# Nextomics/NextPolish2

Hardware: AMD Instinct MI355X
Metric: polished reference Mbp/s (whole node) at 30x HiFi + k21/k31; FASTA identical to oracle (higher is better)
Workload: dtype u8

## Files before the change

### nextpolish2_amd/csrc/np2_ctx.hpp

```cpp
#pragma once
#include "../../include/np2.h"
#include "np2_abi.hpp"
#include "np2_common.hpp"
#include "np2_kernels.hpp"
#include "np2_hostcpu.hpp"

#include <algorithm>
#include <atomic>
#include <chrono>
#include <cstdio>
#include <cstdlib>
#include <cstring>
#include <map>
#include <memory>
#include <exception>
#include <mutex>
#include <stdexcept>
#include <string>
#include <vector>

namespace np2h {

using namespace np2;

// ... 418 lines not shown
    uint32_t tile_cap = TILE_CAP;
};

struct np2_ctx {
    int device = 0;
    hipStream_t stream = nullptr;
    hipStream_t stream_out = nullptr;
    hipEvent_t ev_out = nullptr;
    uint8_t *out_host[2] = {nullptr, nullptr};
    size_t out_host_cap[2] = {0, 0};
    int out_slot = 0;
    bool out_pending = false;
    uint64_t out_len = 0;
    std::vector<YakTable> yaks;
    std::string err;
    bool trace = false;
    std::map<std::string, std::vector<uint8_t>> trace_items;
    Timing timing;
    std::vector<std::pair<std::string, std::pair<hipEvent_t, hipEvent_t>>> pending_events;

    PinnedBuf pin_d2h, pin_h2d;
    uint32_t *mbox_host = nullptr, *mbox_dev = nullptr;
    uint32_t mbox_seq = 0;
    bool borrowed_state = false;
    uint8_t *sink_dst = nullptr;
    uint64_t sink_cap = 0;
    uint32_t last_first_pos = 0, last_last_pos = 0;
    const uint8_t *last_dbase = nullptr;
    const uint32_t *last_dpos = nullptr;
    DevBuf<uint32_t> shard_bounds;
    uint64_t last_len = 0;
    bool reuse_identical_pass = true;
    bool h2d_inflight = false;
    bool stage_timing = false;
    DevBuf<uint8_t> tmp;
    DevBuf<uint64_t> keys_raw, keys;
    DevBuf<uint32_t> vals_raw, vals;
    DevBuf<uint32_t> npos, ncount, nminr, nbesti, node_off, run_start, run_end, n0_besti, emit, eoff;
    DevBuf<uint16_t> nbases, ndelta;
    DevBuf<int64_t> nscore;
    DevBuf<int32_t> cov, mval, smin;
    DevBuf<uint8_t> alive, cns_base, cns_cls, lq_kind, lq_nothead;
    DevBuf<uint32_t> cns_pos, lq_next, rflag, rstart, rend, ridx, raw_start, raw_end, headflag, hidx, lq_start,
        lq_end;
    DevBuf<uint32_t> pj, pcount, reg_ncand, reg_bytes, reg_soff, reg_maxlen, blk_sum, blk_coff, blk_soff, kept_read, kept_len, kept_col, cand_off, cand_order, cand_seq_off, kill_ids;
    DevBuf<uint64_t> cand_kmer;
    DevBuf<uint8_t> cand_seq;
    DevBuf<uint16_t> kscore;
    DevBuf<uint32_t> scal;
    DevBuf<uint64_t> lb_status;
    DevBuf<uint32_t> lb_ticket;
    uint32_t lb_ticket_total = 0, lb_epoch = 0;
    bool lb_dirty = false;
    static constexpr size_t LB_MAX_BLOCKS = 1u << 20;
    DevBuf<uint32_t> mlen;
    DevBuf<uint8_t> reg_lable, grp, cns_base2, rech_groups, rech_groups_tmp;
    DevBuf<uint8_t> votepack;
    DevBuf<uint8_t> votepack2;
    DevBuf<uint32_t> rl_list, rl_blob_off, rl_glen;
    DevBuf<uint2> rl_job_ol;
    DevBuf<uint32_t> rech_headjobs;
    DevBuf<uint32_t> ecount, eval, eval_s, eflag, eidx, seed_cand, keep_n, keep_list, cns_pos2, sp_idx_s,
        sp_idx_e, ap_g, ap_s, ap_e, rech, rech_joboff, job_len,
        job_off32;
    DevBuf<int32_t> ew, ap_delta, ap_shift;
    DevBuf<uint64_t> ekey, ekey_s;
    DevBuf<uint16_t> keep_ks;
    DevBuf<uint32_t> long_list;
    DevBuf<uint64_t> bt_path;
    DevBuf<uint64_t> chunk_st;
    uint32_t chunk_epoch = 0;
    DevBuf<uint32_t> tile_cur, tile_n, tile_scan, tile_scanb, tile_nn, tile_nr, tile_noff, tile_roff;
    uint32_t tile_cap = TILE_CAP;
    uint32_t bucket_cap = 0;
    DevBuf<uint2> nrec;
    DevBuf<uint8_t> votebuf;
    DevBuf<uint32_t> band, band_n, band_off, row_cnt;
    DevBuf<int64_t> run_gain, tile_gain;
    DevBuf<uint8_t> out_snap;
    DevBuf<uint8_t> run_flag;
    uint32_t deep_min = 65536;
    DevBuf<uint32_t> lq_list, hbits;
    DevBuf<uint16_t> tile_pidx;
    bool pidx_valid = false;
    DevBuf<ReadInfo> rinfo;
    DevBuf<uint32_t> lqc, lqoff;
    DevBuf<uint8_t> pflag;
    DevBuf<uint32_t> dp_list;
    DevBuf<uint16_t> pf_slots;
    DevBuf<uint32_t> pf_bad, pf_bad2;
    DevBuf<uint64_t> pf_prof;
    bool front_fused = false;
    struct Hooks {
        bool front_unfused = false, pf_prof = false, edge_sort = false;
        bool test_misspeculate = false, shard_spec_log = false, phase_profile = false, exact_grow = false, no_speculate = false;
        bool has_grow_guess = false, rech_general = false, rech_log = false;
        uint32_t grow_guess = 0;
        uint32_t rech_cap_list = 0xFFFFFFFFu, rech_cap_jobs = 0xFFFFFFFFu, rech_cap_blob = 0xFFFFFFFFu;
        bool has_pf_cap = false, has_pf_cap_big = false, has_pf_halo = false, has_pf_cov_max = false;
        uint32_t pf_cap = 0, pf_cap_big = 0, pf_halo = 0, pf_cov_max = 0;
        void read() {
            auto on = [](const char *n) { return getenv(n) != nullptr; };
            auto u32 = [](const char *n, bool &has, uint32_t &v) {
                if (const char *e = getenv(n)) has = true, v = (uint32_t)atol(e);
            };
            front_unfused = on("NP2_FRONT_UNFUSED"), pf_prof = on("NP2_PF_PROF"), edge_sort = on("NP2_EDGE_SORT");
            test_misspeculate = on("NP2_TEST_MISSPECULATE");
            shard_spec_log = on("NP2_SHARD_SPEC_LOG"), phase_profile = on("NP2_PHASE_PROFILE"), exact_grow = on("NP2_EXACT_GROW");
            no_speculate = on("NP2_NO_SPECULATE");
            rech_general = on("NP2_RECH_GENERAL");
            rech_log = on("NP2_RECH_LOG");
            if (const char *e = getenv("NP2_TEST_RECH_CAP")) {
                char *end = nullptr;
                rech_cap_list = (uint32_t)strtoul(e, &end, 10);
                if (end && *end == ',') rech_cap_jobs = (uint32_t)strtoul(end + 1, &end, 10);
                if (end && *end == ',') rech_cap_blob = (uint32_t)strtoul(end + 1, &end, 10);
            }
            u32("NP2_TEST_GROW_GUESS", has_grow_guess, grow_guess);
            u32("NP2_PF_CAP", has_pf_cap, pf_cap), u32("NP2_PF_CAP_BIG", has_pf_cap_big, pf_cap_big);
            u32("NP2_PF_HALO", has_pf_halo, pf_halo), u32("NP2_PF_COV_MAX", has_pf_cov_max, pf_cov_max);
        }
    } hooks;
    bool pf_big = getenv("NP2_PF_BIG") != nullptr;
    uint32_t front_redos = 0;
    DevBuf<uint16_t> kscore_saved;
    DevBuf<uint8_t> sstr;
    DevBuf<uint64_t> soff;
    DevBuf<uint16_t> sscore;
};


namespace np2h {


enum Scal { S_ERR = 0, S_NNODES, S_NRUNS, S_BEST, S_PATHBEGIN, S_NRAW, S_NREG, S_DUP, S_LAST0, S_LAST1, S_GAIN0,
            S_GAIN1, S_DEEP, S_NDPLIST, S_NRECH, S_NGROUPS, S_NLONG, S_NLQ, S_PF, S_M0, S_M1, S_M2, S_M3, S_NC, S_SB, S_GROW,
            S_NBAD, S_PFOUT, S_PFGAIN0, S_PFGAIN1, S_PFEND0, S_PFEND1, S_NBAD2, S_NOKEY, S_COUNT = 34 };
static_assert(S_M1 % 2 == 0 && S_LAST0 % 2 == 0 && S_GAIN0 % 2 == 0 && S_PFGAIN0 % 2 == 0 && S_PFEND0 % 2 == 0,
              "64-bit device counters live in these slot pairs");

static constexpr int NP2_MAX_YAK = 15;
static constexpr uint32_t SCAL_TOTAL = 96;
static_assert(S_COUNT + 2 * (NP2_MAX_YAK + 2) <= SCAL_TOTAL && S_COUNT < 64, "round counters behind the posted block; the mailbox holds 64 words");
static constexpr uint32_t S_RL = S_COUNT + 2 * (NP2_MAX_YAK + 2);
static_assert(S_RL + 2 + np2::RL_STATE_WORDS <= SCAL_TOTAL, "the region lists' counters fit behind the round counters");

inline double thread_cpu_ms() {
    timespec ts;
    clock_gettime(CLOCK_THREAD_CPUTIME_ID, &ts);
    return ts.tv_sec * 1e3 + ts.tv_nsec * 1e-6;
}
struct WallTimer {
    np2_ctx *cx;
    const char *name;
    double t0, c0 = 0;
    WallTimer(np2_ctx *c, const char *n);
    ~WallTimer();
};

struct EventTimer {
    np2_ctx *cx;
    hipEvent_t a = nullptr, b = nullptr;
    bool on;
    EventTimer(np2_ctx *c, const char *name, bool always = false)
        : cx(c), on((always || c->stage_timing) && !tl_recorder()) {
        if (!on) return;
// ... 239 lines not shown
```

### nextpolish2_amd/csrc/np2_final.cpp

```cpp
#include "np2_polish.hpp"

#include <algorithm>
#include <cstdio>
#include <string>
#include <vector>

using namespace np2;

namespace {

static const uint8_t LB_SUCC = 0x80, LB_RECH = 0x20;

CnsDev splice_buffers(np2_ctx *cx, const CnsDev &in, uint32_t n_slots, uint32_t grow_bound, bool to_b, uint32_t version) {
    cx->sp_idx_s.ensure(n_slots + 2);
    cx->sp_idx_e.ensure(n_slots + 2);
    cx->ap_g.ensure(n_slots + 2);
    cx->ap_s.ensure(n_slots + 2);
    cx->ap_e.ensure(n_slots + 2);
    cx->ap_delta.ensure(n_slots + 2);
    cx->ap_shift.ensure(n_slots + 2);
    cx->mlen.ensure(16);
    const uint32_t out_cap = in.M_cap + grow_bound;
    const size_t cap = (size_t)out_cap + 64;
    uint32_t *opos = to_b ? cx->cns_pos2.ensure(cap) : cx->cns_pos.ensure(cap);
    uint8_t *obase = to_b ? cx->cns_base2.ensure(cap) : cx->cns_base.ensure(cap);
    return CnsDev{opos, obase, cx->mlen.p + version, out_cap};
}
CnsDev splice_gpu(np2_ctx *cx, const CnsDev &in, uint32_t n_reg, uint8_t lable, uint32_t grow_bound, bool to_b,
                  uint32_t version) {
    hipStream_t s = cx->stream;
    EventTimer t(cx, "splice");
    const CnsDev out = splice_buffers(cx, in, n_reg, grow_bound, to_b, version);
    uint32_t *const opos = out.pos;
    uint8_t *const obase = out.base;
    const uint32_t out_cap = out.M_cap;
    uint32_t *const stuck_p = cx->scal.p + S_COUNT + 2 * version, *const nap_p = stuck_p + 1;
    launch_splice_find(s, in.pos, in.M_p, cx->lq_start.p, cx->lq_end.p, cx->reg_lable.p, lable, n_reg, cx->sp_idx_s.p,
                       cx->sp_idx_e.p, stuck_p);
    launch_splice_plan(s, next_lookback(cx, region_lb_blocks(n_reg)), cx->reg_lable.p, lable, n_reg, stuck_p,
                       cx->sp_idx_s.p, cx->sp_idx_e.p, cx->seed_cand.p, cx->cand_seq_off.p, cx->ap_g.p, cx->ap_s.p,
                       cx->ap_e.p, cx->ap_delta.p, cx->ap_shift.p, nap_p, in.M_p, cx->mlen.p + version, out_cap,
                       cx->scal.p + S_ERR);
    launch_splice_write(s, in.pos, in.base, in.M_p, in.M_cap, cx->ap_g.p, cx->ap_s.p, cx->ap_e.p, cx->ap_delta.p,
                        cx->ap_shift.p, nap_p, n_reg, cx->lq_start.p, cx->seed_cand.p, cx->cand_seq_off.p,
                        cx->cand_seq.p, opos, obase);
    return out;
}

Cns fetch_cns_dev(np2_ctx *cx, const CnsDev &c) {
    Cns r;
    const uint32_t M = d2h(cx, c.M_p, 1)[0];
    r.pos = d2h(cx, c.pos, M);
    r.base = d2h(cx, c.base, M);
    return r;
}

bool rech_by_list(const np2_ctx *cx, uint32_t n_reg) {
    return !cx->trace && !cx->hooks.rech_general && n_reg <= RL_NREG_MAX;
}
uint32_t rech_list_cap(const np2_ctx *cx) { return std::min(cx->hooks.rech_cap_list, RL_CAP_LIST); }
uint32_t *rech_list_of(np2_ctx *cx, size_t y) { return cx->rl_list.p + (y & 1) * RL_CAP_LIST; }
uint32_t *rech_list_cnt(np2_ctx *cx, size_t y) { return cx->scal.p + S_RL + (y & 1); }

CnsDev recheck_list_gpu(np2_ctx *cx, const CnsDev &in, const PassCounts &pc, int yak_idx, uint16_t min_kmer_count,
                        bool first_yak, bool last_yak, bool to_b, uint32_t version) {
    hipStream_t s = cx->stream;
    EventTimer t(cx, "recheck");
    const uint32_t ksize = cx->yaks[yak_idx].k;
    const uint32_t cap_jobs = std::min(cx->hooks.rech_cap_jobs, RL_CAP_JOBS), cap_blob = std::min(cx->hooks.rech_cap_blob, RL_CAP_BLOB);
    cx->rech.ensure(RL_CAP_LIST + 2);
    cx->rech_groups.ensure((size_t)(RL_CAP_LIST + 2) * rech_group_bytes());
    cx->rech_groups_tmp.ensure((size_t)(RL_CAP_LIST + 2) * rech_group_bytes());
    cx->rech_joboff.ensure(RL_CAP_LIST + 2);
    cx->rl_blob_off.ensure(RL_CAP_LIST + 2);
    cx->rl_glen.ensure(RL_CAP_LIST + 2);
    cx->rl_job_ol.ensure(RL_CAP_JOBS + 2);
    cx->sstr.ensure((size_t)RL_CAP_BLOB + 64);
    cx->sscore.ensure(RL_CAP_JOBS + 2);
    const CnsDev out = splice_buffers(cx, in, std::max(pc.n_reg, RL_CAP_LIST), pc.grow, to_b, version);
    uint32_t *const st = cx->scal.p + S_RL + 2, *const nap_p = cx->scal.p + S_COUNT + 2 * version + 1;
    const RechList rl{rech_list_of(cx, (size_t)yak_idx), rech_list_cnt(cx, (size_t)yak_idx), rech_list_of(cx, (size_t)yak_idx + 1),
                      rech_list_cnt(cx, (size_t)yak_idx + 1), st, cx->rech.p, cx->sp_idx_s.p, cx->sp_idx_e.p, cx->rech_groups.p, cx->rech_groups_tmp.p,
                      cx->rech_joboff.p, cx->rl_blob_off.p, cx->rl_glen.p, cx->rl_job_ol.p, cx->sstr.p,
                      rech_list_cap(cx), cap_jobs, cap_blob};
    launch_rech_prepare(s, rl, in.pos, in.base, in.M_p, cx->lq_start.p, cx->lq_end.p, cx->keep_n.p, ksize, cx->reg_maxlen.p,
                        cx->cand_off.p, cx->keep_list.p, cx->cand_seq_off.p, cx->cand_seq.p, cx->scal.p + S_ERR);
    launch_score_jobs(s, cx->yaks[yak_idx].dev(), cx->sstr.p, cx->rl_job_ol.p, st + RL_NJOBS, min_kmer_count,
                      cx->sscore.p);
    launch_rech_finish(s, rl, cx->sscore.p, cx->keep_ks.p, cx->cand_off.p, cx->keep_n.p, cx->keep_list.p, cx->cand_order.p,
                       first_yak, last_yak, cx->reg_lable.p, cx->seed_cand.p, in.pos, in.M_p, cx->lq_start.p,
                       cx->cand_seq_off.p, cx->ap_g.p, cx->ap_s.p, cx->ap_e.p, cx->ap_delta.p, cx->ap_shift.p, nap_p, cx->mlen.p + version,
                       out.M_cap, cx->scal.p + S_ERR);
    launch_splice_write(s, in.pos, in.base, in.M_p, in.M_cap, cx->ap_g.p, cx->ap_s.p, cx->ap_e.p, cx->ap_delta.p,
                        cx->ap_shift.p, nap_p, RL_CAP_LIST, cx->lq_start.p, cx->seed_cand.p, cx->cand_seq_off.p,
                        cx->cand_seq.p, out.pos, out.base);
    cx->timing.host.push_back({"rech_list", 1.0f});
    return out;
}

CnsDev recheck_gpu(np2_ctx *cx, const CnsDev &in, const PassCounts &pc, int yak_idx, uint16_t min_kmer_count,
                   bool first_yak, bool to_b, uint32_t version) {
    hipStream_t s = cx->stream;
    const uint32_t n_reg = pc.n_reg, ksize = cx->yaks[yak_idx].k;
    uint32_t n_rech = 0, n_groups = 0, n_jobs = 0;
    uint64_t blob_bound = 0;
    {
        EventTimer t(cx, "recheck");
        cx->rech.ensure(n_reg + 2);
        cx->rech_groups.ensure((size_t)(n_reg + 2) * rech_group_bytes());
        cx->rech_joboff.ensure(n_reg + 2);
        cx->rech_groups_tmp.ensure((size_t)(n_reg + 2) * rech_group_bytes());
        cx->rech_headjobs.ensure(n_reg + 2);
        launch_rech_list(s, next_lookback(cx, region_lb_blocks(n_reg)), cx->reg_lable.p, n_reg, cx->rech.p, cx->scal.p + S_NRECH,
                         (unsigned long long *)(cx->scal.p + S_M1), cx->scal.p + S_ERR);
        launch_rech_groups(s, next_lookback(cx, region_lb_blocks(n_reg)), cx->rech.p, cx->scal.p + S_NRECH, n_reg, in.pos, in.M_p,
                           cx->lq_start.p, cx->lq_end.p, cx->keep_n.p, ksize, cx->reg_maxlen.p, cx->rech_groups_tmp.p,
                           cx->rech_headjobs.p, cx->rech_groups.p,
                           cx->rech_joboff.p, cx->scal.p + S_NGROUPS,
                           cx->scal.p + S_M0, (unsigned long long *)(cx->scal.p + S_M1), cx->scal.p + S_ERR);
        std::vector<uint32_t> sc = fetch_scal(cx);
        blob_bound = (uint64_t)sc[S_M1] | ((uint64_t)sc[S_M2] << 32);
        check_region_err(sc[S_ERR]);
        n_rech = sc[S_NRECH];
        n_groups = sc[S_NGROUPS];
        n_jobs = sc[S_M0];
        if (cx->hooks.rech_log)
            fprintf(stderr, "np2 recheck, table %d: %u regions, %u RECH, %u groups, %u jobs, %llu string bytes at most\n", yak_idx, n_reg,
                    n_rech, n_groups, n_jobs, (unsigned long long)blob_bound);
    }
    if (n_rech) {
        RechPtrs rp{cx->rech_groups.p, cx->rech_joboff.p, cx->rech.p, cx->cand_off.p, cx->keep_list.p,
                    cx->cand_seq_off.p, cx->cand_seq.p, in.base, n_groups};
        if (n_jobs) {
            EventTimer t(cx, "recheck");
            cx->job_len.ensure(n_jobs + 2);
            cx->job_off32.ensure(n_jobs + 2);
            cx->soff.ensure(n_jobs + 2);
            cx->sscore.ensure(n_jobs + 2);
            cx->tmp.ensure(prim_temp_bytes((size_t)n_jobs + 2));
            launch_rech_job_len(s, rp, n_jobs, cx->job_len.p);
            exclusive_total_n(cx, cx->job_len.p, cx->job_off32.p, n_jobs);
            if (blob_bound >= 0xFFFFFFF0ull)
                blob_bound = fetch_scal(cx, cx->scal.p + S_M0, cx->job_off32.p + n_jobs)[S_M0];
            cx->sstr.ensure((size_t)blob_bound + 64);
            launch_rech_job_build(s, rp, n_jobs, cx->job_off32.p, cx->soff.p, cx->sstr.p);
            launch_score_strings(s, cx->yaks[yak_idx].dev(), cx->sstr.p, cx->soff.p, n_jobs, min_kmer_count,
                                 cx->sscore.p, true);
            launch_rech_apply(s, rp, cx->sscore.p, cx->keep_ks.p);
        }
        EventTimer t(cx, "recheck");
        launch_rech_select(s, cx->rech.p, cx->scal.p + S_NRECH, n_rech, cx->cand_off.p, cx->keep_n.p, cx->keep_list.p,
                           cx->keep_ks.p, cx->cand_order.p, first_yak, cx->reg_lable.p, cx->seed_cand.p);
    }
    CnsDev out = splice_gpu(cx, in, n_reg, LB_RECH, pc.grow, to_b, version);
    launch_rech_relabel(s, cx->reg_lable.p, n_reg);
    return out;
}

void fetch_result(np2_ctx *cx, const uint32_t *dpos, const uint8_t *dbase, const uint32_t *M_p, uint32_t M_cap, ResultOut &r,
                  uint32_t M_likely = 0xFFFFFFFFu) {
    const double t0 = now_ms();
    std::vector<uint32_t> sc;
    if (cx->sink_dst && cx->sink_cap) launch_copy_len(cx->stream, cx->sink_dst, dbase, M_p, 1, cx->sink_cap);
    if (r.want_bases || r.want_pos) {
        const uint32_t seq = ++cx->mbox_seq;
        launch_post(cx->stream, cx->scal.p, S_COUNT, cx->mbox_dev, seq, cx->scal.p + S_M0, M_p, nullptr, nullptr, nullptr, nullptr,
                    nullptr, nullptr, dpos, cx->scal.p + S_M1);
        if (r.want_bases) r.bases = (uint8_t *)pinned_pool().get((size_t)M_cap + 1);
        if (r.want_pos) r.pos = (uint32_t *)pinned_pool().get(((size_t)M_cap + 1) * 4);
        if ((r.want_bases && !r.bases) || (r.want_pos && !r.pos)) throw Np2Error(NP2_E_NOMEM, "pinned result allocation failed");
        uint32_t first = std::min(M_cap, M_likely);
        const bool exact_b = r.want_bases && op_d2h_len(cx, r.bases, dbase, M_p, 1, M_cap);
        const bool exact_p = r.want_pos && op_d2h_len(cx, r.pos, dpos, M_p, 4, (size_t)M_cap * 4);
        if (r.want_bases && !exact_b) op_d2h(cx, r.bases, dbase, first);
        if (r.want_pos && !exact_p) op_d2h(cx, r.pos, dpos, (size_t)first * 4);
// ... 156 lines not shown
```

### nextpolish2_amd/csrc/np2_graph.hip

```cpp
#include "np2_common.hpp"
#include "np2_kernels.hpp"
#include "np2_blockscan.hpp"
#include "np2_lookback.hpp"

namespace np2 {

__device__ __forceinline__ uint32_t block_excl_scan_256(uint32_t v, uint32_t *sh, uint32_t &total) {
    return block_excl_scan<OpAdd, 4>(v, sh, total);
}

__device__ uint64_t make_node_key(const np2_read_t *__restrict__ reads, const uint8_t *__restrict__ nib, uint64_t rec,
                                  uint32_t r) {
    const uint32_t col = (uint32_t)rec, t3 = (uint32_t)(rec >> 32);
    const np2_read_t rd = reads[r];
    const uint8_t *base = nib + rd.nib_off;
    const uint32_t ts = rd.aln_t_s;
    auto mk = [&](int64_t c, uint32_t t) -> AlignBase {
        if (c == -2) return ab_head(ts - 1, 0);
        if (c == -1) return ab_head(ts - 1, 1);
        const uint8_t nb = nib_at(base, (uint32_t)c);
        AlignBase a;
        a.q = nb & 7;
        a.t_pos = t;
        a.delta = 0;
        if (c > 0 && (nb & 8)) {
            uint16_t dl = 1;
            int64_t x = c - 1;
            while (x > 0 && (nib_at(base, (uint32_t)x) & 8)) {
                dl = (uint16_t)(dl + 1);
                --x;
            }
            a.delta = dl;
        }
        return a;
    };
    auto is_ins = [&](int64_t c) -> bool { return c > 0 && (nib_at(base, (uint32_t)c) & 8); };
    const int64_t c3 = col;
    const AlignBase b3 = mk(c3, t3);
    const uint32_t t2 = is_ins(c3) ? t3 : t3 - 1;
    const AlignBase b2 = mk(c3 - 1, t2);
    const uint32_t t1 = is_ins(c3 - 1) ? t2 : t2 - 1;
    const AlignBase b1 = mk(c3 - 2, t1);
    return ((uint64_t)b3.t_pos << 32) | ((uint64_t)node_bases(b1, b2, b3) << 16) | b1.delta;
}

__device__ __forceinline__ void k_tile_layout(const uint32_t np2_bid, const uint32_t np2_nb, uint32_t *__restrict__ tile_cur, uint32_t n_tiles,
                                                      uint32_t bucket_cap, uint32_t *__restrict__ tile_n,
                                                      uint32_t *__restrict__ tile_scan, uint32_t *__restrict__ tile_scanb,
                                                      const uint32_t *__restrict__ ovf_cnt, uint32_t *__restrict__ out) {
    __shared__ uint32_t sh[16];
    const uint32_t ta = block_scan_array<OpAdd>(
        n_tiles, sh, [&](uint32_t i) { return tile_cur[i]; },
        [&](uint32_t i, uint32_t pre, uint32_t v) {
            tile_scan[i] = pre;
            tile_n[i] = v;
        });
    const uint32_t tb = block_scan_array<OpAdd>(
        n_tiles, sh, [&](uint32_t i) { return min(tile_n[i], bucket_cap); },
        [&](uint32_t i, uint32_t pre, uint32_t) { tile_scanb[i] = pre; });
    const uint32_t mx = block_scan_array<OpMaxU32>(
        n_tiles, sh, [&](uint32_t i) { return tile_n[i]; }, [&](uint32_t i, uint32_t, uint32_t) { tile_cur[i] = 0; });
    if (threadIdx.x == 0) {
        tile_scan[n_tiles] = ta;
        tile_scanb[n_tiles] = tb;
        out[0] = ta;
        out[1] = mx;
        out[2] = *ovf_cnt;
    }
}

static constexpr uint32_t TLB_ITEMS = 4;
__device__ __forceinline__ void k_tile_layout_lb(const uint32_t np2_bid, const uint32_t np2_nb, Lookback lb, uint32_t n_blocks, uint32_t *__restrict__ tile_cur,
                                                        uint32_t n_tiles, uint32_t bucket_cap, uint32_t *__restrict__ tile_n,
                                                        uint32_t *__restrict__ tile_scan, uint32_t *__restrict__ tile_scanb,
                                                        const uint32_t *__restrict__ ovf_cnt, uint32_t *__restrict__ out,
                                                        uint32_t *__restrict__ err) {
    __shared__ uint32_t sh[8];
    const uint32_t bid = lb_block_id(lb, sh);
    const uint32_t i0 = (bid * 256 + threadIdx.x) * TLB_ITEMS;
    uint32_t v[TLB_ITEMS], sa = 0, sb = 0, mx = 0;
#pragma unroll
    for (uint32_t k = 0; k < TLB_ITEMS; ++k) {
        v[k] = i0 + k < n_tiles ? tile_cur[i0 + k] : 0u;
        sa += v[k];
        sb += min(v[k], bucket_cap);
        mx = max(mx, v[k]);
    }
    for (int o = 32; o > 0; o >>= 1) mx = max(mx, __shfl_xor(mx, o));
    if ((threadIdx.x & 63) == 0 && mx) atomicMax(&out[1], mx);
    uint32_t ta, tb, pa, pb;
    uint32_t ra = block_excl_scan<OpAdd, 4>(sa, sh, ta);
    uint32_t rb = block_excl_scan<OpAdd, 4>(sb, sh, tb);
    lb_exclusive2(lb, bid, ta, tb, sh, err, pa, pb);
    ra += pa, rb += pb;
#pragma unroll
    for (uint32_t k = 0; k < TLB_ITEMS; ++k)
        if (i0 + k < n_tiles) {
            tile_scan[i0 + k] = ra;
            tile_scanb[i0 + k] = rb;
            tile_n[i0 + k] = v[k];
            tile_cur[i0 + k] = 0;
            ra += v[k];
            rb += min(v[k], bucket_cap);
        }
    if (bid == n_blocks - 1 && threadIdx.x == 255) {
        tile_scan[n_tiles] = ra;
        tile_scanb[n_tiles] = rb;
        out[0] = ra;
        out[2] = *ovf_cnt;
    }
}

template <uint32_t CAP>
__device__ __forceinline__ void k_tile_sort(const uint32_t np2_bid, const uint32_t np2_nb, uint16_t *__restrict__ pidx, const np2_read_t *__restrict__ reads,
                                                   const uint8_t *__restrict__ nib, const uint32_t *__restrict__ tile_n,
                                                   uint32_t bucket_cap, uint64_t *__restrict__ keys,
                                                   uint32_t *__restrict__ vals, uint32_t *__restrict__ err,
                                                   uint32_t n_above, uint32_t n_upto) {
    __shared__ uint32_t s_klo[CAP];
    __shared__ uint32_t s_v[CAP];
    __shared__ uint16_t s_q[CAP];
    __shared__ uint16_t s_idx[CAP];
    __shared__ uint32_t s_cnt[TILE];
    __shared__ uint16_t s_off[TILE];
    __shared__ uint32_t sh[8];
    const uint32_t n = tile_n[np2_bid], tid = threadIdx.x;
    const uint64_t a = (uint64_t)np2_bid * bucket_cap;
    if (n <= n_above || n > n_upto) return;
    if (n > CAP) {
        if (tid == 0) atomicOr(err, 8u);
        return;
    }
    const uint32_t start = np2_bid << TILE_SHIFT;
    for (uint32_t i = tid; i < TILE; i += 256) s_cnt[i] = 0;
    __syncthreads();
    for (uint32_t i = tid; i < n; i += 256) {
        const uint32_t r = vals[a + i];
        const uint64_t k = make_node_key(reads, nib, keys[a + i], r);
        uint32_t q = (uint32_t)(k >> 32) - start;
        if (q >= TILE) {
            atomicOr(err, 8u);
            q = TILE - 1;
        }
        s_klo[i] = (uint32_t)k;
        s_v[i] = r;
        s_q[i] = (uint16_t)q;
        atomicAdd(&s_cnt[q], 1u);
    }
    __syncthreads();
    {
        const uint32_t q0 = tid * 4;
        const uint32_t c0 = s_cnt[q0], c1 = s_cnt[q0 + 1], c2 = s_cnt[q0 + 2], c3 = s_cnt[q0 + 3];
        uint32_t tot;
        const uint32_t l0 = block_excl_scan_256(c0 + c1 + c2 + c3, sh, tot);
        s_off[q0] = (uint16_t)l0, s_off[q0 + 1] = (uint16_t)(l0 + c0), s_off[q0 + 2] = (uint16_t)(l0 + c0 + c1), s_off[q0 + 3] = (uint16_t)(l0 + c0 + c1 + c2);
        s_cnt[q0] = 0, s_cnt[q0 + 1] = 0, s_cnt[q0 + 2] = 0, s_cnt[q0 + 3] = 0;
    }
    __syncthreads();
    for (uint32_t i = tid; i < n; i += 256) {
        const uint32_t q = s_q[i];
        s_idx[s_off[q] + atomicAdd(&s_cnt[q], 1u)] = (uint16_t)i;
    }
    if (tid < TILE / 16) pidx[(size_t)np2_bid * (TILE / 16) + tid] = s_off[tid * 16];
    __syncthreads();
    for (uint32_t d = tid; d < n; d += 256) {
        const uint32_t i = s_idx[d], q = s_q[i], b = s_off[q], m = s_cnt[q];
        const uint32_t klo = s_klo[i], v = s_v[i];
        uint32_t rank = 0;
        for (uint32_t e = b; e < b + m; ++e) {
            const uint32_t j = s_idx[e];
            const uint32_t kj = s_klo[j], vj = s_v[j];
            rank += (kj < klo || (kj == klo && vj < v)) ? 1u : 0u;
        }
        keys[a + b + rank] = ((uint64_t)(start + q) << 32) | klo;
        vals[a + b + rank] = v;
    }
}

__device__ __forceinline__ void k_gather_buckets(const uint32_t np2_bid, const uint32_t np2_nb, const np2_read_t *__restrict__ reads,
                                                        const uint8_t *__restrict__ nib,
                                                        const uint32_t *__restrict__ tile_n,
                                                        const uint32_t *__restrict__ tile_scanb, uint32_t bucket_cap,
                                                        const uint64_t *__restrict__ bkeys,
                                                        const uint32_t *__restrict__ bvals, uint64_t *__restrict__ keys,
                                                        uint32_t *__restrict__ vals) {
    const uint32_t n = min(tile_n[np2_bid], bucket_cap);
    const uint64_t a = (uint64_t)np2_bid * bucket_cap;
    const uint32_t dst = tile_scanb[np2_bid];
    for (uint32_t i = threadIdx.x; i < n; i += 256) {
        const uint32_t r = bvals[a + i];
        keys[dst + i] = make_node_key(reads, nib, bkeys[a + i], r);
        vals[dst + i] = r;
    }
}
__device__ __forceinline__ void k_gather_spill(const uint32_t np2_bid, const uint32_t np2_nb, const np2_read_t *__restrict__ reads, const uint8_t *__restrict__ nib,
                               const uint64_t *__restrict__ okeys, const uint32_t *__restrict__ ovals, uint32_t n,
                               uint64_t *__restrict__ keys, uint32_t *__restrict__ vals) {
    const uint32_t i = np2_bid * blockDim.x + threadIdx.x;
    if (i >= n) return;
    const uint32_t r = ovals[i];
    keys[i] = make_node_key(reads, nib, okeys[i], r);
    vals[i] = r;
}

__device__ __forceinline__ bool group_head(const uint64_t *__restrict__ keys, const uint32_t *__restrict__ vals,
                                           const uint8_t *__restrict__ alive, uint64_t i, uint64_t a, uint64_t b,
                                           uint32_t &cnt, uint32_t &mn) {
    const uint64_t k = keys[i];
    if (i > a && keys[i - 1] == k) return false;
    cnt = 0;
    mn = 0xFFFFFFFFu;
// ... 396 lines not shown
                const uint16_t bb = nd.bases[i], d = nd.delta[i];
                const uint32_t c = nd.count[i], m = nd.minr[i];
                const uint32_t kd = node_delta3(bb, d);
                uint32_t x = i;
                while (x > o0) {
                    const uint32_t pd = node_delta3(nd.bases[x - 1], nd.delta[x - 1]);
                    if (pd < kd || (pd == kd && nd.minr[x - 1] < m)) break;
                    nd.bases[x] = nd.bases[x - 1];
                    nd.delta[x] = nd.delta[x - 1];
                    nd.count[x] = nd.count[x - 1];
                    nd.minr[x] = nd.minr[x - 1];
                    --x;
                }
                nd.bases[x] = bb;
                nd.delta[x] = d;
                nd.count[x] = c;
                nd.minr[x] = m;
            }
            for (uint32_t i = o0; i < o1; ++i)
                nrec[i] = make_uint2((uint32_t)nd.bases[i] | ((uint32_t)nd.delta[i] << 16), nd.count[i]);
        }
    }
    uint32_t pf = 0;
#pragma unroll
    for (uint32_t j = 0; j < 4; ++j) pf |= ((cj[j] ? 1u : 0u) | (cv[j] < 2 ? 2u : 0u)) << (8 * j);
    const bool pd0 = q0 ? cnt[q0 - 1] != 0 : prevd != 0;
    const uint32_t ref4 = q0 < npos ? *reinterpret_cast<const uint16_t *>(refnib + ((start + q0) >> 1)) : 0u;
    uint32_t em[4];
    {
        long long gain = 0;
        bool pdirty = pd0;
        for (uint32_t j = 0; j < 4; ++j) {
            const bool d = cj[j] != 0;
            em[j] = d ? 0u : (((ref4 >> (4 * j)) & 7) != 4 ? 1u : 0u);
            if (q0 + j < npos) {
                if (!d && !pdirty) gain += 6LL * cv[j];
            }
            pdirty = d;
        }
        for (int o = 32; o > 0; o >>= 1) gain += __shfl_down(gain, o);
        if ((tid & 63) == 0) s_gain[tid >> 6] = gain;
        __syncthreads();
    }
    const bool s0 = c0 && !pd0, s1 = c1 && !c0, s2 = c2 && !c1, s3 = c3 && !c2;
    uint32_t r = tile_roff[np2_bid] +
                 block_excl_scan_256((uint32_t)s0 + (uint32_t)s1 + (uint32_t)s2 + (uint32_t)s3, sh, tot);
    if (s0) run_start[r++] = start + q0;
    if (s1) run_start[r++] = start + q0 + 1;
    if (s2) run_start[r++] = start + q0 + 2;
    if (s3) run_start[r++] = start + q0 + 3;
    if (q0 < npos) {
        *reinterpret_cast<uint32_t *>(pflag + start + q0) = pf;
        if (q0 + 4 <= npos) {
            *reinterpret_cast<int4 *>(cov + start + q0) = make_int4(cv[0], cv[1], cv[2], cv[3]);
            *reinterpret_cast<uint4 *>(node_off + start + q0) = make_uint4(nbase + off[0], nbase + off[1], nbase + off[2], nbase + off[3]);
            *reinterpret_cast<uint4 *>(emit + start + q0) = make_uint4(em[0], em[1], em[2], em[3]);
        } else {
            for (uint32_t j = 0; j < 4; ++j)
                if (q0 + j < npos) {
                    cov[start + q0 + j] = cv[j];
                    node_off[start + q0 + j] = nbase + off[j];
                    emit[start + q0 + j] = em[j];
                }
        }
    }
    if (np2_bid == n_tiles - 1 && tid == 255) node_off[L] = nbase + off[4];
    if (max(max(cv[0], cv[1]), max(cv[2], cv[3])) >= deep_min) atomicOr(deep_flag, 1u);
    if (tid == 0) tile_gain[np2_bid] = s_gain[0] + s_gain[1] + s_gain[2] + s_gain[3];
    if (fast) {
        for (uint32_t i = tid; i < nn; i += 256) {
            const uint32_t kk = s_nkey[i], c = s_ncnt[i];
            const uint32_t o = nbase + i;
            nd.bases[o] = (uint16_t)(kk >> 16);
            nd.delta[o] = (uint16_t)kk;
            nd.count[o] = c;
            nrec[o] = make_uint2((kk >> 16) | (kk << 16), c);
        }
    }
}

uint32_t tile_scan_blocks(uint32_t n_tiles) { return (n_tiles + 256 * TLB_ITEMS - 1) / (256 * TLB_ITEMS); }
void launch_tile_layout(hipStream_t s, uint32_t *tile_cur, uint32_t n_tiles, uint32_t bucket_cap, uint32_t *tile_n,
                        uint32_t *tile_scan, uint32_t *tile_scanb, const uint32_t *ovf_cnt, uint32_t *out,
                        const Lookback *lb, uint32_t *err) {
    if (lb)
        NP2_LAUNCH(k_tile_layout_lb, dim3(tile_scan_blocks(n_tiles)), 256, s, *lb, tile_scan_blocks(n_tiles), tile_cur, n_tiles, bucket_cap, tile_n, tile_scan, tile_scanb, ovf_cnt, out, err);
    else
        NP2_LAUNCH(k_tile_layout, dim3(1), 1024, s, tile_cur, n_tiles, bucket_cap, tile_n, tile_scan, tile_scanb, ovf_cnt, out);
}
void launch_tile_sort(hipStream_t s, uint16_t *pidx, const np2_read_t *reads, const uint8_t *nib, const uint32_t *tile_n,
                      uint32_t n_tiles, uint32_t bucket_cap, uint32_t max_tile, uint64_t *keys, uint32_t *vals,
                      uint32_t *err) {
    const uint32_t ALL = 0xFFFFFFFFu;
    if (max_tile <= 1024) {
        NP2_LAUNCH(k_tile_sort<1024>, dim3(n_tiles), 256, s, pidx, reads, nib, tile_n, bucket_cap, keys, vals, err, 0u, ALL);
    } else {
        NP2_LAUNCH(k_tile_sort<1024>, dim3(n_tiles), 256, s, pidx, reads, nib, tile_n, bucket_cap, keys, vals, err, 0u, 1024u);
        if (max_tile <= 2048 && TILE_CAP > 2048)
            NP2_LAUNCH(k_tile_sort<2048>, dim3(n_tiles), 256, s, pidx, reads, nib, tile_n, bucket_cap, keys, vals, err, 1024u, ALL);
        else
            NP2_LAUNCH(k_tile_sort<TILE_CAP>, dim3(n_tiles), 256, s, pidx, reads, nib, tile_n, bucket_cap, keys, vals, err, 1024u, ALL);
    }
}
void launch_gather_buckets(hipStream_t s, const np2_read_t *reads, const uint8_t *nib, const uint32_t *tile_n,
                           const uint32_t *tile_scanb, uint32_t n_tiles, uint32_t bucket_cap, const uint64_t *bkeys,
                           const uint32_t *bvals, uint64_t *keys, uint32_t *vals) {
    NP2_LAUNCH(k_gather_buckets, dim3(n_tiles), 256, s, reads, nib, tile_n, tile_scanb, bucket_cap, bkeys, bvals, keys, vals);
}
void launch_gather_spill(hipStream_t s, const np2_read_t *reads, const uint8_t *nib, const uint64_t *okeys,
                         const uint32_t *ovals, uint32_t n, uint64_t *keys, uint32_t *vals) {
    if (n) NP2_LAUNCH(k_gather_spill, dim3((n + 255) / 256), 256, s, reads, nib, okeys, ovals, n, keys, vals);
}
void launch_tile_count(hipStream_t s, const uint64_t *keys, const uint32_t *vals, const uint32_t *tile_n,
                       const uint32_t *tile_scan, uint32_t bucket_cap, uint32_t n_tiles, const uint8_t *alive,
                       uint32_t *tile_nn, uint32_t *tile_nr) {
    NP2_LAUNCH(k_tile_count, dim3(n_tiles), 256, s, keys, vals, TileLayout{tile_n, tile_scan, bucket_cap}, alive, tile_nn, tile_nr);
}
void launch_tile_offsets(hipStream_t s, const uint32_t *tile_nn, const uint32_t *tile_nr, uint32_t n_tiles,
                         uint32_t *tile_noff, uint32_t *tile_roff, uint32_t *n_nodes, uint32_t *n_runs, uint32_t *reset,
                         uint32_t n_reset, const Lookback *lb, uint32_t *err, const long long *tile_gain,
                         unsigned long long *gain_total) {
    if (lb)
        NP2_LAUNCH(k_tile_offsets_lb, dim3(tile_scan_blocks(n_tiles)), 256, s, *lb, tile_scan_blocks(n_tiles), tile_nn, tile_nr, n_tiles, tile_noff, tile_roff, n_nodes, n_runs, reset, n_reset, err, tile_gain, gain_total);
    else
        NP2_LAUNCH(k_tile_offsets, dim3(1), 1024, s, tile_nn, tile_nr, n_tiles, tile_noff, tile_roff, n_nodes, n_runs, reset, n_reset, tile_gain, gain_total);
}
void launch_tile_write(hipStream_t s, const uint64_t *keys, const uint32_t *vals, const uint32_t *tile_n,
                       const uint32_t *tile_scan, uint32_t bucket_cap, const uint32_t *tile_noff, const uint32_t *tile_roff,
                       uint32_t n_tiles, const uint8_t *alive, uint32_t L, NodeArrays nd, uint2 *nrec, uint32_t *node_off,
                       uint32_t *run_start, const np2_read_t *reads, const uint32_t *tile_rd_off, const uint32_t *tile_rd,
                       int32_t *cov, const uint8_t *refnib, uint32_t *emit, long long *tile_gain, uint32_t *deep_flag, uint32_t deep_min,
                       uint8_t *pflag) {
    NP2_LAUNCH(k_tile_write, dim3(n_tiles), 256, s, keys, vals, TileLayout{tile_n, tile_scan, bucket_cap}, tile_noff, tile_roff, alive, L, n_tiles, nd, nrec, node_off, run_start, reads, tile_rd_off, tile_rd, cov, refnib, emit, tile_gain, deep_flag, (int32_t)deep_min, pflag);
}

}
```

### nextpolish2_amd/csrc/np2_kernels.hip

```cpp
#include "np2_common.hpp"
#include "np2_kernels.hpp"
#include "np2_blockscan.hpp"
#include "np2_nib128.hpp"
#include "../../include/np2.h"

namespace np2 {

__device__ __forceinline__ uint8_t ref_code(const uint8_t *__restrict__ refnib, uint32_t p) {
    return (refnib[p >> 1] >> (4 * (p & 1))) & 7;
}

__device__ __forceinline__ void k_encode_ref(const uint32_t np2_bid, const uint32_t np2_nb, const uint8_t *__restrict__ read0, uint32_t L, uint8_t *__restrict__ refnib,
                             uint32_t nbytes_total, uint32_t stride, uint32_t *__restrict__ err) {
    uint32_t i = np2_bid * blockDim.x + threadIdx.x;
    if (i >= nbytes_total) return;
    uint32_t c0 = 2 * i, c1 = 2 * i + 1;
    uint8_t b = c0 < L ? read0[i] : 0;
    uint8_t hi = c0 < L ? (b >> 4) : 0, lo = c1 < L ? (b & 15) : 0;
    if ((c0 < L && c0 != 0 && (hi & 8)) || (c1 < L && (lo & 8))) atomicOr(err, 1u);
    if (c0 < L && (hi & 7) == 7) atomicOr(err, 1u);
    if (c1 < L && (lo & 7) == 7) atomicOr(err, 1u);
    refnib[i] = (uint8_t)((hi & 7) | ((lo & 7) << 4));
    const uint8_t nx = c1 + 1 < L ? (uint8_t)((read0[i + 1] >> 4) & 7) : (uint8_t)0;
    refnib[stride + i] = (uint8_t)(((hi & 7) << 4) | (lo & 7));
// ... 1131 lines not shown
            cnt = s - j + 1;
        }
    }
    pj[r] = j;
    pcount[r] = cnt;
    rinfo[r] = ReadInfo{rd.aln_t_s, rd.n_cols, (uint32_t)(rd.nib_off >> 4), (uint32_t)ck_off[r], rd.aln_t_e, j, cnt, 0u};
}


__global__ void k_yak_insert(const uint64_t *__restrict__ words, const uint64_t *__restrict__ bucket_off,
                             uint32_t n_buckets, uint64_t *__restrict__ table, uint32_t cap_log2,
                             uint32_t *__restrict__ dup_flag, uint32_t gap) {
    const uint32_t b = blockIdx.y;
    if (b >= n_buckets) return;
    const uint64_t n = bucket_off[b + 1] - bucket_off[b] - gap;
    const uint64_t capm = (1ULL << cap_log2) - 1;
    uint64_t *tb = table + ((uint64_t)b << cap_log2);
    for (uint64_t i = (uint64_t)blockIdx.x * blockDim.x + threadIdx.x; i < n; i += (uint64_t)gridDim.x * blockDim.x) {
        const uint64_t w = words[bucket_off[b] + i];
        const uint64_t key = w >> 10;
        uint64_t s = key & capm;
        for (;;) {
            const unsigned long long old = atomicCAS((unsigned long long *)&tb[s], (unsigned long long)YAK_EMPTY,
                                                     (unsigned long long)w);
            if (old == YAK_EMPTY) break;
            if ((old >> 10) == key) {
                atomicOr(dup_flag, 1u);
                break;
            }
            s = (s + 1) & capm;
        }
    }
}

__global__ void k_yak_insert_dup(const uint64_t *__restrict__ words, const uint64_t *__restrict__ bucket_off,
                                 uint32_t n_buckets, uint64_t *__restrict__ table, uint32_t cap_log2,
                                 uint32_t *__restrict__ ord, uint32_t gap) {
    const uint32_t b = blockIdx.y;
    if (b >= n_buckets) return;
    const uint64_t n = bucket_off[b + 1] - bucket_off[b] - gap;
    const uint64_t capm = (1ULL << cap_log2) - 1;
    uint64_t *tb = table + ((uint64_t)b << cap_log2);
    uint32_t *ob = ord + ((uint64_t)b << cap_log2);
    for (uint64_t i = (uint64_t)blockIdx.x * blockDim.x + threadIdx.x; i < n; i += (uint64_t)gridDim.x * blockDim.x) {
        const uint64_t w = words[bucket_off[b] + i];
        uint64_t s = (w >> 10) & capm;
        while (atomicCAS((unsigned long long *)&tb[s], (unsigned long long)YAK_EMPTY, (unsigned long long)w) != YAK_EMPTY)
            s = (s + 1) & capm;
        ob[s] = (uint32_t)i;
    }
}

__device__ __forceinline__ void k_lookup(const uint32_t np2_bid, const uint32_t np2_nb, YakDev y, const uint64_t *__restrict__ hashes, uint64_t n, uint16_t min_count,
                         uint16_t *__restrict__ out) {
    uint64_t i = (uint64_t)np2_bid * blockDim.x + threadIdx.x;
    if (i < n) out[i] = yak_get(y, hashes[i], min_count);
}

__device__ __forceinline__ uint16_t wave_score_string_any(const YakDev &y, const uint8_t *__restrict__ s, uint32_t len,
                                                          uint16_t min_count) {
    const uint32_t lane = threadIdx.x & 63;
    const uint32_t k = y.k;
    const uint64_t mask = (1ULL << (2 * (uint64_t)k)) - 1, shift = 2 * ((uint64_t)k - 1);
    uint32_t mn = 0xFFFFFFFFu;
    if (len >= k) {
        for (uint32_t st = lane; st + k <= len; st += 64) {
            uint64_t fw = 0, rv = 0;
            bool ok = true;
            for (uint32_t j = 0; j < k; ++j) {
                const uint64_t c = ascii_to_code(s[st + j]);
                if (c >= 4) {
                    ok = false;
                    break;
                }
                fw = ((fw << 2) | c) & mask;
                rv = (rv >> 2) | ((3ULL ^ c) << shift);
            }
            if (ok) mn = min(mn, (uint32_t)yak_get(y, yak_hash64(fw < rv ? fw : rv, mask), min_count));
        }
    }
    for (int o = 32; o > 0; o >>= 1) mn = min(mn, (uint32_t)__shfl_xor(mn, o));
    return mn == 0xFFFFFFFFu ? (uint16_t)0 : (uint16_t)mn;
}
__device__ __forceinline__ uint16_t wave_score_string(const YakDev &y, const uint8_t *__restrict__ s, uint32_t len,
                                                      uint16_t min_count) {
    const uint32_t lane = threadIdx.x & 63;
    const uint32_t k = y.k;
    const uint64_t mask = (1ULL << (2 * (uint64_t)k)) - 1;
    uint32_t mn = 0xFFFFFFFFu;
    if (len >= k) {
        for (uint32_t st = lane; st + k <= len; st += 64) {
            uint64_t codes = 0, bad = 0;
#pragma unroll
            for (uint32_t wd = 0; wd < 4; ++wd) {
                uint64_t x;
                __builtin_memcpy(&x, s + st + 8 * wd, 8);
                uint64_t c = ((x >> 1) ^ (x >> 2)) & 0x0303030303030303ULL;
                c = (c | (c >> 6)) & 0x000F000F000F000FULL;
                c = (c | (c >> 12)) & 0x000000FF000000FFULL;
                c = (c | (c >> 24)) & 0xFFFFULL;
                codes |= c << (16 * wd);
                uint64_t b = (x >> 3) & 0x0101010101010101ULL;
                b = (b | (b >> 7)) & 0x0003000300030003ULL;
                b = (b | (b >> 14)) & 0x0000000F0000000FULL;
                b = (b | (b >> 28)) & 0xFFULL;
                bad |= b << (8 * wd);
            }
            if ((bad & ((1ULL << k) - 1ULL)) == 0) {
                codes &= mask;
                uint64_t rb = __builtin_bitreverse64(codes);
                rb = ((rb >> 1) & 0x5555555555555555ULL) | ((rb & 0x5555555555555555ULL) << 1);
                const uint64_t fw = rb >> (64 - 2 * k), rv = ~codes & mask;
                mn = min(mn, (uint32_t)yak_get(y, yak_hash64(fw < rv ? fw : rv, mask), min_count));
            }
        }
    }
    for (int o = 32; o > 0; o >>= 1) mn = min(mn, (uint32_t)__shfl_xor(mn, o));
    return mn == 0xFFFFFFFFu ? (uint16_t)0 : (uint16_t)mn;
}

__device__ __forceinline__ void k_score_strings(const uint32_t np2_bid, const uint32_t np2_nb, YakDev y, const uint8_t *__restrict__ strs, const uint64_t *__restrict__ off,
                                uint64_t n, uint16_t min_count, uint16_t *__restrict__ out, uint32_t own_strings) {
    const uint64_t w = ((uint64_t)np2_bid * (blockDim.x >> 6)) + (uint32_t)__builtin_amdgcn_readfirstlane((int)(threadIdx.x >> 6));
    if (w >= n) return;
    const uint16_t sc = own_strings ? wave_score_string(y, strs + off[w], (uint32_t)(off[w + 1] - off[w]), min_count)
                                    : wave_score_string_any(y, strs + off[w], (uint32_t)(off[w + 1] - off[w]), min_count);
    if ((threadIdx.x & 63) == 0) out[w] = sc;
}

__device__ __forceinline__ void k_score_jobs(const uint32_t np2_bid, const uint32_t np2_nb, YakDev y, const uint8_t *__restrict__ strs, const uint2 *__restrict__ job_ol,
                                             const uint32_t *__restrict__ n_jobs_p, uint16_t min_count, uint16_t *__restrict__ out) {
    const uint32_t n = *n_jobs_p, n_waves = np2_nb * (blockDim.x >> 6);
    for (uint32_t w = np2_bid * (blockDim.x >> 6) + (uint32_t)__builtin_amdgcn_readfirstlane((int)(threadIdx.x >> 6)); w < n; w += n_waves) {
        const uint2 ol = job_ol[w];
        const uint16_t sc = wave_score_string(y, strs + ol.x, ol.y, min_count);
        if ((threadIdx.x & 63) == 0) out[w] = sc;
    }
}

__device__ __forceinline__ void k_cand_score(const uint32_t np2_bid, const uint32_t np2_nb, YakDev y, const uint32_t *__restrict__ cand_seq_off, const uint64_t *__restrict__ cand_kmer,
                             const uint32_t *__restrict__ n_cand_p, uint16_t min_count,
                             uint16_t *__restrict__ kscore, uint32_t *__restrict__ long_list,
                             uint32_t *__restrict__ n_long) {
    const uint32_t c = np2_bid * blockDim.x + threadIdx.x;
    const bool live = c < *n_cand_p;
    const uint32_t len = live ? cand_seq_off[c + 1] - cand_seq_off[c] : 0u;
    const bool is_long = live && len > y.k;
    const uint64_t m = __ballot(is_long);
    if (m) {
        const uint32_t lane = threadIdx.x & 63, lead = (uint32_t)__builtin_ctzll(m);
        uint32_t base = 0;
        if (lane == lead) base = atomicAdd(n_long, (uint32_t)__builtin_popcountll(m));
        base = __shfl(base, lead);
        if (is_long) long_list[base + (uint32_t)__builtin_popcountll(m & ((1ULL << lane) - 1ULL))] = c;
    }
    if (!live) return;
    uint16_t sc = 0;
    if (!is_long) {
        const uint64_t km = cand_kmer[c];
        if (km != INVALID_KMER) sc = yak_get(y, km, min_count);
    }
    kscore[c] = sc;
}
__device__ __forceinline__ void k_cand_score_long(const uint32_t np2_bid, const uint32_t np2_nb, YakDev y, const uint32_t *__restrict__ cand_seq_off,
                                  const uint8_t *__restrict__ cand_seq, const uint32_t *__restrict__ long_list,
                                  const uint32_t *__restrict__ n_long, uint16_t min_count,
                                  uint16_t *__restrict__ kscore) {
    const uint32_t nl = *n_long;
    for (uint32_t w = (uint32_t)__builtin_amdgcn_readfirstlane((int)((np2_bid * blockDim.x + threadIdx.x) >> 6)); w < nl; w += (np2_nb * blockDim.x) >> 6) {
        const uint32_t c = long_list[w];
        const uint16_t sc = wave_score_string(y, cand_seq + cand_seq_off[c], cand_seq_off[c + 1] - cand_seq_off[c],
                                              min_count);
        if ((threadIdx.x & 63) == 0) kscore[c] = sc;
    }
}

}

namespace np2 {
static inline dim3 grid1(uint64_t n, uint32_t bs = 256) { return dim3((unsigned)((n + bs - 1) / bs)); }

void launch_encode_ref(hipStream_t s, const uint8_t *read0, uint32_t L, uint8_t *refnib, uint32_t nbytes,
                       uint32_t stride, uint32_t *err) {
    NP2_LAUNCH(k_encode_ref, grid1(nbytes), 256, s, read0, L, refnib, nbytes, stride, err);
}
void launch_post(hipStream_t s, uint32_t *scal, uint32_t n_scal, uint32_t *mbox, uint32_t seq, uint32_t *d0,
                 const uint32_t *s0, uint32_t *d1, const uint32_t *s1, uint32_t *d2, const uint32_t *s2, uint32_t *d3,
                 const uint32_t *s3, const uint32_t *ends_of, uint32_t *ends_dst) {
    NP2_LAUNCH(k_post, dim3(1), 64, s, scal, n_scal, mbox, seq, d0, s0, d1, s1, d2, s2, d3, s3, ends_of, ends_dst);
}
void launch_fill(hipStream_t s, uint8_t *p, uint64_t bytes, uint8_t byte) {
    if (bytes) NP2_LAUNCH(k_fill, grid1((bytes + 15) / 16), 256, s, p, bytes, 0x01010101u * byte);
}
void launch_copy(hipStream_t s, uint8_t *dst, const uint8_t *src, uint64_t bytes) {
    if (bytes) NP2_LAUNCH(k_copy, grid1((bytes + 15) / 16), 256, s, dst, src, bytes);
}
void launch_copy_len(hipStream_t s, uint8_t *dst, const uint8_t *src, const uint32_t *n_dev, uint32_t elem, uint64_t cap_bytes) {
    if (cap_bytes) NP2_LAUNCH(k_copy_len, grid1((cap_bytes + 15) / 16), 256, s, dst, src, n_dev, elem, cap_bytes);
}
void launch_copy_counted(hipStream_t s, uint32_t *dst, const uint32_t *src, const uint32_t *n_dev, uint32_t cap, uint32_t words_per) {
    if (cap) NP2_LAUNCH(k_copy_counted, dim3(std::max<uint32_t>(1, std::min<uint32_t>((cap + 1023) / 1024, 2048))), 256, s, dst, src, n_dev, cap, words_per);
}
void launch_init_alive(hipStream_t s, const np2_read_t *reads, uint32_t R, uint8_t *alive) {
    NP2_LAUNCH(k_init_alive, grid1(R), 256, s, reads, R, alive);
}
void launch_kill_flagged(hipStream_t s, const uint8_t *flag, uint32_t n, uint8_t *alive) {
    if (n) NP2_LAUNCH(k_kill_flagged, grid1(n), 256, s, flag, n, alive);
}
void launch_kill_reads(hipStream_t s, const uint32_t *ids, uint32_t n, uint8_t *alive) {
    if (n) NP2_LAUNCH(k_kill_reads, grid1(n), 256, s, ids, n, alive);
}
void launch_revive_reads(hipStream_t s, const uint32_t *ids, uint32_t n, uint8_t *alive) {
    if (n) NP2_LAUNCH(k_revive_reads, grid1(n), 256, s, ids, n, alive);
}
static Graph mk_graph(const GraphPtrs &gp) { return Graph{gp.refnib, gp.node_off, gp.nd, gp.cov, gp.L, gp.nrec, gp.deep}; }

void launch_dp_short(hipStream_t s, const GraphPtrs &gp, const void *refw, const uint32_t *run_start,
                     const uint32_t *n_runs, uint32_t max_runs, uint32_t *run_end, int64_t *run_gain, uint32_t *emit,
                     uint32_t *path_begin, uint64_t *path, uint32_t *dp_list, uint32_t *n_dp_list) {
    if (max_runs)
// ... 5 lines not shown
                    const uint32_t *dp_list, const uint32_t *n_dp_list) {
    if (!max_runs) return;
    NP2_LAUNCH(k_dp_bt_oct, dim3(std::min<uint32_t>((max_runs + 7) / 8, 2048u)), 64, s, run_start, mk_graph(gp), nrec, nscore, nbesti, n0_besti, run_end, last_n0_score, run_gain, emit, path_begin, path, run_flag, dp_list, n_dp_list);
    NP2_LAUNCH(k_dp_bt_long, dim3(std::min<uint32_t>((max_runs + DP_BLOCK - 1) / DP_BLOCK, 512u)), DP_BLOCK, s, run_start, mk_graph(gp), nrec, nscore, nbesti, n0_besti, run_end, last_n0_score, run_gain, emit, path_begin, path, run_flag, dp_list, n_dp_list);
}
void launch_dp_finish(hipStream_t s, const GraphPtrs &gp, const uint32_t *run_start, const uint32_t *n_runs,
                      const int64_t *nscore, const uint32_t *nbesti, const uint32_t *n0_besti, const int64_t *last_n0_score,
                      unsigned long long *total_gain, uint32_t *blocks_done, uint32_t *best_idx, const int64_t *run_gain,
                      const long long *tile_gain, uint32_t n_tiles, uint32_t *emit, uint32_t *path_begin, uint64_t *path) {
    NP2_LAUNCH(k_dp_finish, dim3(64), 256, s, run_gain, n_runs, tile_gain, n_tiles, total_gain, blocks_done, mk_graph(gp), nscore, last_n0_score, run_start, nbesti, n0_besti, best_idx, emit, path_begin, path);
}
static inline dim3 run_grid(uint32_t bound) { return dim3(std::max<uint32_t>(1, std::min<uint32_t>((bound + 256) / 256, 4096))); }
void launch_bt_write(hipStream_t s, const GraphPtrs &gp, const uint32_t *run_start, const uint32_t *n_runs,
                     uint32_t run_bound, const uint32_t *emit, const uint32_t *eoff, const uint64_t *path,
                     uint32_t *cns_pos, uint8_t *cns_base, uint8_t *cns_cls, uint8_t *lq_nothead, uint32_t *lqc) {
    NP2_LAUNCH(k_cns_write, grid1(gp.L), 256, s, gp.refnib, gp.pflag, emit, eoff, gp.L, cns_pos, cns_base, cns_cls, lq_nothead);
    NP2_LAUNCH(k_cns_runs, run_grid(4 * (uint64_t)run_bound > 0xFFFFFFF0ull ? 0xFFFFFFF0u : 4 * run_bound), 256, s, run_start, n_runs, run_bound, gp.node_off, emit, eoff, path, cns_pos, cns_base, cns_cls, lq_nothead, lqc);
}
void launch_lq_list(hipStream_t s, const GraphPtrs &gp, const uint32_t *run_start, const uint32_t *n_runs,
                    uint32_t run_bound, const uint32_t *emit, const uint32_t *eoff, const uint64_t *path,
                    const uint32_t *lqoff, uint32_t cap, uint32_t *lq_list, uint32_t *err) {
    NP2_LAUNCH(k_lq_list, run_grid(run_bound), 256, s, run_start, n_runs, run_bound, gp.node_off, emit, eoff, path, lqoff, cap, lq_list, err);
}
void launch_default_tail(hipStream_t s, const GraphPtrs &gp, const uint32_t *best_idx, const uint32_t *M_p, uint8_t *cns_base,
                         uint8_t *cns_cls, uint32_t *lq_list, uint32_t *n_lq, uint32_t cap, uint32_t *err) {
    NP2_LAUNCH(k_default_tail, 1, 64, s, best_idx, gp.node_off, gp.pflag, gp.L, M_p, cns_base, cns_cls, lq_list, n_lq, cap, err);
}
static inline dim3 lq_grid(uint32_t cap) { return dim3(std::max<uint32_t>(1, std::min<uint32_t>((cap + 2047) / 2048, 2048))); }
void launch_lq_scan(hipStream_t s, const uint32_t *cns_pos, const uint8_t *cns_base, const uint8_t *cns_cls,
                    const uint32_t *M_p, const uint32_t *lq_list, const uint32_t *n_lq, uint32_t lq_cap, uint8_t *lq_kind,
                    uint32_t *lq_next, uint8_t *lq_nothead, uint32_t *hbits, uint32_t n_hwords, uint32_t *rstart, uint32_t *rend) {
    NP2_LAUNCH(k_lq_scan, lq_grid(std::max(lq_cap, n_hwords / 4)), 256, s, cns_pos, cns_base, cns_cls, M_p, lq_list, n_lq, lq_cap, lq_kind, lq_next, lq_nothead, hbits, n_hwords);
    NP2_LAUNCH(k_lq_region, lq_grid(lq_cap), 256, s, cns_pos, cns_base, M_p, lq_list, n_lq, lq_cap, lq_kind, lq_next, lq_nothead, hbits, rstart, rend);
}
void launch_lq_bits_count(hipStream_t s, const uint32_t *hbits, uint32_t n_words, uint32_t *wcnt) {
    NP2_LAUNCH(k_lq_bits_count, grid1((uint64_t)n_words + 1), 256, s, hbits, n_words, wcnt);
}
void launch_scatter_regions(hipStream_t s, const uint32_t *hbits, uint32_t n_words, const uint32_t *woff,
                            const uint32_t *rstart, const uint32_t *rend, uint32_t *raw_start, uint32_t *raw_end,
                            uint32_t *n_raw) {
    NP2_LAUNCH(k_scatter_regions, grid1(std::max<uint32_t>(n_words, 1)), 256, s, hbits, n_words, woff, rstart, rend, raw_start, raw_end, n_raw);
}
void launch_lq_merge_flag(hipStream_t s, const uint32_t *raw_start, const uint32_t *raw_end, const uint32_t *n_raw,
                          uint32_t *headflag) {
    NP2_LAUNCH(k_lq_merge_flag, dim3(256), 256, s, raw_start, raw_end, n_raw, headflag);
}
void launch_lq_merge_scan(hipStream_t s, const uint32_t *raw_start, const uint32_t *raw_end, const uint32_t *n_raw, uint32_t n_host,
                          uint32_t *headflag, uint32_t *hidx) {
    NP2_LAUNCH(k_lq_merge_scan, dim3(1), 1024, s, raw_start, raw_end, n_raw, n_host, headflag, hidx);
}
void launch_lq_merge_write(hipStream_t s, const uint32_t *raw_start, const uint32_t *raw_end, const uint32_t *n_raw,
                           const uint32_t *headflag, const uint32_t *hidx, uint32_t *lq_start, uint32_t *lq_end,
                           uint32_t *n_reg) {
    NP2_LAUNCH(k_lq_merge_write, dim3(256), 256, s, raw_start, raw_end, n_raw, headflag, hidx, lq_start, lq_end, n_reg);
}
void launch_read_m(hipStream_t s, const np2_read_t *reads, uint32_t R, const uint8_t *alive, const uint32_t *lq_start,
                   uint32_t n_reg, int32_t *mval) {
    NP2_LAUNCH(k_read_m, grid1(R), 256, s, reads, R, alive, lq_start, n_reg, mval);
}
void launch_pair_count(hipStream_t s, const np2_read_t *reads, uint32_t R, const uint8_t *alive,
                       const uint32_t *lq_start, const uint32_t *lq_end, uint32_t n_reg, const int32_t *smin,
                       uint32_t *pj, uint32_t *pcount, const uint64_t *ck_off, ReadInfo *rinfo) {
    NP2_LAUNCH(k_pair_count, grid1(R), 256, s, reads, R, alive, lq_start, lq_end, n_reg, smin, pj, pcount, ck_off, rinfo);
}
void launch_yak_insert(hipStream_t s, const uint64_t *words, const uint64_t *bucket_off, uint32_t n_buckets,
                       uint64_t max_bucket, uint64_t *table, uint32_t cap_log2, uint32_t *dup_flag, uint32_t gap) {
    uint32_t gx = (uint32_t)((max_bucket + 255) / 256);
    if (gx == 0) gx = 1;
    if (gx > 64) gx = 64;
    hipLaunchKernelGGL(k_yak_insert, dim3(gx, n_buckets), dim3(256), 0, s, words, bucket_off, n_buckets, table,
                       cap_log2, dup_flag, gap);
}
void launch_yak_insert_dup(hipStream_t s, const uint64_t *words, const uint64_t *bucket_off, uint32_t n_buckets,
                           uint64_t max_bucket, uint64_t *table, uint32_t cap_log2, uint32_t *ord, uint32_t gap) {
    uint32_t gx = (uint32_t)((max_bucket + 255) / 256);
    gx = std::min<uint32_t>(64, std::max<uint32_t>(1, gx));
    hipLaunchKernelGGL(k_yak_insert_dup, dim3(gx, n_buckets), dim3(256), 0, s, words, bucket_off, n_buckets, table,
                       cap_log2, ord, gap);
}
void launch_lookup(hipStream_t s, const YakDev &y, const uint64_t *hashes, uint64_t n, uint16_t min_count,
                   uint16_t *out) {
    if (n) NP2_LAUNCH(k_lookup, grid1(n), 256, s, y, hashes, n, min_count, out);
}
void launch_score_jobs(hipStream_t s, const YakDev &y, const uint8_t *strs, const uint2 *job_ol, const uint32_t *n_jobs_p,
                       uint16_t min_count, uint16_t *out) {
    NP2_LAUNCH(k_score_jobs, dim3(16), 256, s, y, strs, job_ol, n_jobs_p, min_count, out);
}
void launch_score_strings(hipStream_t s, const YakDev &y, const uint8_t *strs, const uint64_t *off, uint64_t n,
                          uint16_t min_count, uint16_t *out, bool own_strings) {
    if (n) NP2_LAUNCH(k_score_strings, grid1(n * 64), 256, s, y, strs, off, n, min_count, out, own_strings ? 1u : 0u);
}
void launch_cand_score(hipStream_t s, const YakDev &y, const uint32_t *cand_seq_off, const uint8_t *cand_seq,
                       const uint64_t *cand_kmer, const uint32_t *n_cand_p, uint32_t cand_cap, uint16_t min_count,
                       uint16_t *kscore, uint32_t *long_list, uint32_t *n_long) {
    if (!cand_cap) return;
    NP2_LAUNCH(k_cand_score, grid1(cand_cap), 256, s, y, cand_seq_off, cand_kmer, n_cand_p, min_count, kscore, long_list, n_long);
    NP2_LAUNCH(k_cand_score_long, dim3(std::max<uint32_t>(16, std::min<uint32_t>(1024, cand_cap / 4096))), 256, s, y, cand_seq_off, cand_seq, long_list, n_long, min_count, kscore);
}
}
```

### nextpolish2_amd/csrc/np2_kernels.hpp

```cpp
#pragma once
#include <cstddef>
#include <cstdint>
#include <hip/hip_runtime.h>
#include "../../include/np2.h"
#include "np2_lookback.hpp"
#include "np2_launch.hpp"
#include "np2_vote_band.hpp"

namespace np2 {

static constexpr uint32_t TILE_SHIFT = 10;
static constexpr uint32_t TILE = 1u << TILE_SHIFT;
static constexpr uint32_t TILE_CAP = 4096;

static constexpr uint32_t DENSE_COLS = 4096;
struct ChunkDesc {
    uint64_t nib_off;
    uint64_t ckbase;
    uint32_t read, ts;
    uint32_t c0, ncols;
    uint32_t first_chunk;
    uint32_t aln_t_e, nck;
    uint32_t pad0;
    uint32_t pad[4];
};

struct NodeArrays {
    uint32_t *pos;
    uint16_t *bases;
    uint16_t *delta;
    uint32_t *count;
    uint32_t *minr;
};
struct GraphPtrs {
    const uint8_t *refnib;
    const uint32_t *node_off;
    NodeArrays nd;
    const int32_t *cov;
    uint32_t L;
    const uint2 *nrec;
    const uint32_t *deep;
    const uint8_t *pflag;
};
struct __attribute__((aligned(16))) ReadInfo {
    uint32_t aln_t_s, n_cols;
    uint32_t nib16;
    uint32_t ck_off;
    uint32_t aln_t_e;
    uint32_t pj, pcount;
    uint32_t pad;
};
struct CandPtrs {
    const np2_read_t *reads;
    const uint8_t *nib;
    const uint64_t *ck_off;
    const uint32_t *ckpt;
    const uint32_t *lq_start;
    const uint32_t *lq_end;
    const uint32_t *pj;
    const uint32_t *pcount;
    const uint8_t *alive;
    const ReadInfo *rinfo;
    const uint32_t *tile_rd_off;
    const uint32_t *tile_rd;
    uint32_t n_tiles;
    uint32_t ksize;
    const uint64_t *rec_key;
    const uint32_t *rec_read;
    const uint32_t *tile_n;
    const uint16_t *rec_pidx;
    uint32_t bucket_cap;
    const uint32_t *refnib;
    uint32_t L;
};
struct YakDev {
    const uint64_t *table;
    uint32_t cap_log2;
    uint32_t k;
    const uint32_t *ord;
};
static constexpr uint64_t YAK_EMPTY = ~0ULL;
#if defined(__HIPCC__)
__device__ __forceinline__ uint16_t yak_get(const YakDev &y, uint64_t x, uint16_t min_count) {
    const uint64_t capm = (1ULL << y.cap_log2) - 1;
    const uint64_t *tb = y.table + ((x & 1023) << y.cap_log2);
    const uint64_t key = x >> 10;
    uint64_t s = key & capm;
    if (y.ord) {
        const uint32_t *ob = y.ord + ((x & 1023) << y.cap_log2);
        uint16_t c = 0;
        int64_t at = -1;
        for (;;) {
            const uint64_t w = tb[s];
            if (w == YAK_EMPTY) return c;
            if ((w >> 10) == key && (uint16_t)(w & 1023) >= min_count && (int64_t)ob[s] > at) at = ob[s], c = (uint16_t)(w & 1023);
            s = (s + 1) & capm;
        }
    }
    for (;;) {
        const uint64_t w = tb[s];
        if (w == YAK_EMPTY) return 0;
        if ((w >> 10) == key) {
            const uint16_t c = (uint16_t)(w & 1023);
            return c >= min_count ? c : 0;
        }
        s = (s + 1) & capm;
    }
}
#endif

void launch_encode_ref(hipStream_t s, const uint8_t *read0, uint32_t L, uint8_t *refnib, uint32_t nbytes, uint32_t stride, uint32_t *err);
void launch_chunk_counts(hipStream_t s, const ChunkDesc *descs, uint32_t n_chunks, const uint8_t *nib, uint64_t *chunk_st, uint32_t epoch);
void launch_diff_reads(hipStream_t s, const ChunkDesc *descs, uint32_t n_chunks, const uint8_t *nib, const uint64_t *refw,
                       const uint8_t *refnib, const uint8_t *refeo, uint32_t eo_stride, uint32_t L, uint64_t *keys, uint32_t *vals, uint32_t *tile_cur,
                       uint32_t n_tiles, uint32_t bucket_cap, uint64_t ovf_base, uint32_t ovf_cap, uint32_t *ovf_cnt,
                       uint32_t *ckpt, uint64_t *chunk_st, uint32_t epoch, uint32_t *err);
void launch_post(hipStream_t s, uint32_t *scal, uint32_t n_scal, uint32_t *mbox, uint32_t seq, uint32_t *d0 = nullptr,
                 const uint32_t *s0 = nullptr, uint32_t *d1 = nullptr, const uint32_t *s1 = nullptr, uint32_t *d2 = nullptr,
                 const uint32_t *s2 = nullptr, uint32_t *d3 = nullptr, const uint32_t *s3 = nullptr,
                 const uint32_t *ends_of = nullptr, uint32_t *ends_dst = nullptr);
void launch_fill(hipStream_t s, uint8_t *p, uint64_t bytes, uint8_t byte);
void launch_copy(hipStream_t s, uint8_t *dst, const uint8_t *src, uint64_t bytes);
void launch_copy_len(hipStream_t s, uint8_t *dst, const uint8_t *src, const uint32_t *n_dev, uint32_t elem, uint64_t cap_bytes);
void launch_copy_counted(hipStream_t s, uint32_t *dst, const uint32_t *src, const uint32_t *n_dev, uint32_t cap, uint32_t words_per = 1);
void launch_init_alive(hipStream_t s, const np2_read_t *reads, uint32_t R, uint8_t *alive);
void launch_kill_reads(hipStream_t s, const uint32_t *ids, uint32_t n, uint8_t *alive);
void launch_revive_reads(hipStream_t s, const uint32_t *ids, uint32_t n, uint8_t *alive);
void launch_kill_flagged(hipStream_t s, const uint8_t *flag, uint32_t n, uint8_t *alive);
void launch_dp_short(hipStream_t s, const GraphPtrs &gp, const void *refw, const uint32_t *run_start,
                     const uint32_t *n_runs, uint32_t max_runs, uint32_t *run_end, int64_t *run_gain, uint32_t *emit,
                     uint32_t *path_begin, uint64_t *path, uint32_t *dp_list, uint32_t *n_dp_list);
void launch_dp_long(hipStream_t s, const GraphPtrs &gp, const uint32_t *run_start, uint32_t max_runs, const uint2 *nrec,
                    int64_t *nscore, uint32_t *nbesti, uint32_t *n0_besti, uint32_t *run_end, int64_t *last_n0_score,
                    int64_t *run_gain, uint32_t *emit, uint32_t *path_begin, uint64_t *path, uint8_t *run_flag,
                    const uint32_t *dp_list, const uint32_t *n_dp_list);
void launch_dp_finish(hipStream_t s, const GraphPtrs &gp, const uint32_t *run_start, const uint32_t *n_runs,
                      const int64_t *nscore, const uint32_t *nbesti, const uint32_t *n0_besti, const int64_t *last_n0_score,
                      unsigned long long *total_gain, uint32_t *blocks_done, uint32_t *best_idx, const int64_t *run_gain,
                      const long long *tile_gain, uint32_t n_tiles, uint32_t *emit, uint32_t *path_begin, uint64_t *path);
void launch_bt_write(hipStream_t s, const GraphPtrs &gp, const uint32_t *run_start, const uint32_t *n_runs,
                     uint32_t run_bound, const uint32_t *emit, const uint32_t *eoff, const uint64_t *path,
                     uint32_t *cns_pos, uint8_t *cns_base, uint8_t *cns_cls, uint8_t *lq_nothead, uint32_t *lqc);
void launch_lq_list(hipStream_t s, const GraphPtrs &gp, const uint32_t *run_start, const uint32_t *n_runs,
                    uint32_t run_bound, const uint32_t *emit, const uint32_t *eoff, const uint64_t *path,
                    const uint32_t *lqoff, uint32_t cap, uint32_t *lq_list, uint32_t *err);
void launch_default_tail(hipStream_t s, const GraphPtrs &gp, const uint32_t *best_idx, const uint32_t *M_p, uint8_t *cns_base,
                         uint8_t *cns_cls, uint32_t *lq_list, uint32_t *n_lq, uint32_t cap, uint32_t *err);
void launch_lq_scan(hipStream_t s, const uint32_t *cns_pos, const uint8_t *cns_base, const uint8_t *cns_cls,
                    const uint32_t *M_p, const uint32_t *lq_list, const uint32_t *n_lq, uint32_t lq_cap, uint8_t *lq_kind,
                    uint32_t *lq_next, uint8_t *lq_nothead, uint32_t *hbits, uint32_t n_hwords, uint32_t *rstart, uint32_t *rend);
void launch_lq_merge_scan_lb(hipStream_t s, const Lookback &lb, const uint32_t *raw_start, const uint32_t *raw_end, const uint32_t *n_raw,
                             uint32_t n_host, uint32_t *headflag, uint32_t *hidx, uint32_t *err);
uint32_t lq_merge_lb_blocks();
void launch_lq_merge_scan(hipStream_t s, const uint32_t *raw_start, const uint32_t *raw_end, const uint32_t *n_raw, uint32_t n_host,
                          uint32_t *headflag, uint32_t *hidx);
void launch_scan_lb_popc(hipStream_t s, const Lookback &lb, const uint32_t *bits, uint32_t *out, uint32_t n_words, uint32_t *err);
void launch_lq_bits_count(hipStream_t s, const uint32_t *hbits, uint32_t n_words, uint32_t *wcnt);
void launch_scatter_regions(hipStream_t s, const uint32_t *hbits, uint32_t n_words, const uint32_t *woff,
                            const uint32_t *rstart, const uint32_t *rend, uint32_t *raw_start, uint32_t *raw_end,
                            uint32_t *n_raw);
void launch_lq_merge_flag(hipStream_t s, const uint32_t *raw_start, const uint32_t *raw_end, const uint32_t *n_raw,
                          uint32_t *headflag);
void launch_lq_merge_write(hipStream_t s, const uint32_t *raw_start, const uint32_t *raw_end, const uint32_t *n_raw,
                           const uint32_t *headflag, const uint32_t *hidx, uint32_t *lq_start, uint32_t *lq_end,
                           uint32_t *n_reg);
void launch_read_m(hipStream_t s, const np2_read_t *reads, uint32_t R, const uint8_t *alive, const uint32_t *lq_start,
                   uint32_t n_reg, int32_t *mval);
void launch_yak_insert(hipStream_t s, const uint64_t *words, const uint64_t *bucket_off, uint32_t n_buckets,
                       uint64_t max_bucket, uint64_t *table, uint32_t cap_log2, uint32_t *dup_flag, uint32_t gap = 0);
void launch_yak_insert_dup(hipStream_t s, const uint64_t *words, const uint64_t *bucket_off, uint32_t n_buckets,
                           uint64_t max_bucket, uint64_t *table, uint32_t cap_log2, uint32_t *ord, uint32_t gap = 0);
void launch_lookup(hipStream_t s, const YakDev &y, const uint64_t *hashes, uint64_t n, uint16_t min_count, uint16_t *out);
void launch_score_strings(hipStream_t s, const YakDev &y, const uint8_t *strs, const uint64_t *off, uint64_t n,
                          uint16_t min_count, uint16_t *out, bool own_strings);
void launch_score_jobs(hipStream_t s, const YakDev &y, const uint8_t *strs, const uint2 *job_ol, const uint32_t *n_jobs_p,
                       uint16_t min_count, uint16_t *out);
void launch_cand_score(hipStream_t s, const YakDev &y, const uint32_t *cand_seq_off, const uint8_t *cand_seq,
                       const uint64_t *cand_kmer, const uint32_t *n_cand_p, uint32_t cand_cap, uint16_t min_count,
                       uint16_t *kscore, uint32_t *long_list, uint32_t *n_long);


void launch_pair_count(hipStream_t s, const np2_read_t *reads, uint32_t R, const uint8_t *alive,
                       const uint32_t *lq_start, const uint32_t *lq_end, uint32_t n_reg, const int32_t *smin,
                       uint32_t *pj, uint32_t *pcount, const uint64_t *ck_off, ReadInfo *rinfo);
void launch_scan_lb_excl(hipStream_t s, const Lookback &lb, const uint32_t *in, uint32_t *out, uint32_t n, bool write_end,
                          uint32_t *err);
uint32_t scan_lb_blocks(uint64_t n);
void launch_scan_small_excl(hipStream_t s, const uint32_t *in, uint32_t *out, uint32_t n, const uint32_t *n_dev,
                            uint32_t *total_out, bool write_end);
void launch_scan_small_incl(hipStream_t s, const int32_t *in, int32_t *out, uint32_t n, const uint32_t *n_dev);
void launch_scan_small_min(hipStream_t s, const int32_t *in, int32_t *out, uint32_t n, const uint32_t *n_dev);
void launch_region_measure(hipStream_t s, const CandPtrs &c, uint32_t n_reg, uint32_t *kept_read, uint32_t *kept_len,
                           uint32_t *kept_col, uint32_t *reg_ncand, uint32_t *reg_bytes, uint32_t *reg_maxlen,
                           uint32_t *blk_sum);
uint32_t cand_offsets_blocks(uint32_t n_reg);
void launch_cand_offsets(hipStream_t s, const uint32_t *blk_sum, uint32_t n_reg, uint32_t *blk_coff, uint32_t *blk_soff,
                         uint32_t *cand_off, uint32_t *reg_soff, uint32_t *n_cand, uint32_t *n_bytes, uint32_t *grow,
                         const Lookback *lb = nullptr, uint32_t *err = nullptr);
void launch_region_write(hipStream_t s, const CandPtrs &c, uint32_t n_reg, const uint32_t *kept_read,
                         const uint32_t *kept_len, const uint32_t *kept_col, const uint32_t *reg_ncand,
                         const uint32_t *reg_bytes, const uint32_t *blk_coff, const uint32_t *blk_soff, uint32_t *cand_off,
                         uint32_t *reg_soff, uint32_t cand_cap, uint32_t seq_cap, uint32_t *cand_order, uint64_t *cand_kmer,
                         uint32_t *cand_seq_off, uint8_t *cand_seq);

uint32_t tile_scan_blocks(uint32_t n_tiles);
void launch_tile_layout(hipStream_t s, uint32_t *tile_cur, uint32_t n_tiles, uint32_t bucket_cap, uint32_t *tile_n,
                        uint32_t *tile_scan, uint32_t *tile_scanb, const uint32_t *ovf_cnt, uint32_t *out,
                        const Lookback *lb = nullptr, uint32_t *err = nullptr);
void launch_tile_sort(hipStream_t s, uint16_t *pidx, const np2_read_t *reads, const uint8_t *nib, const uint32_t *tile_n,
                      uint32_t n_tiles, uint32_t bucket_cap, uint32_t max_tile, uint64_t *keys, uint32_t *vals,
                      uint32_t *err);
void launch_gather_buckets(hipStream_t s, const np2_read_t *reads, const uint8_t *nib, const uint32_t *tile_n,
                           const uint32_t *tile_scanb, uint32_t n_tiles, uint32_t bucket_cap, const uint64_t *bkeys,
                           const uint32_t *bvals, uint64_t *keys, uint32_t *vals);
void launch_gather_spill(hipStream_t s, const np2_read_t *reads, const uint8_t *nib, const uint64_t *okeys,
                         const uint32_t *ovals, uint32_t n, uint64_t *keys, uint32_t *vals);
void launch_tile_count(hipStream_t s, const uint64_t *keys, const uint32_t *vals, const uint32_t *tile_n,
                       const uint32_t *tile_scan, uint32_t bucket_cap, uint32_t n_tiles, const uint8_t *alive,
                       uint32_t *tile_nn, uint32_t *tile_nr);
void launch_tile_offsets(hipStream_t s, const uint32_t *tile_nn, const uint32_t *tile_nr, uint32_t n_tiles,
                         uint32_t *tile_noff, uint32_t *tile_roff, uint32_t *n_nodes, uint32_t *n_runs, uint32_t *reset,
                         uint32_t n_reset, const Lookback *lb = nullptr, uint32_t *err = nullptr,
                         const long long *tile_gain = nullptr, unsigned long long *gain_total = nullptr);
void launch_tile_write(hipStream_t s, const uint64_t *keys, const uint32_t *vals, const uint32_t *tile_n,
                       const uint32_t *tile_scan, uint32_t bucket_cap, const uint32_t *tile_noff, const uint32_t *tile_roff,
                       uint32_t n_tiles, const uint8_t *alive, uint32_t L, NodeArrays nd, uint2 *nrec, uint32_t *node_off,
                       uint32_t *run_start, const np2_read_t *reads, const uint32_t *tile_rd_off, const uint32_t *tile_rd,
                       int32_t *cov, const uint8_t *refnib, uint32_t *emit, long long *tile_gain, uint32_t *deep_flag, uint32_t deep_min,
                       uint8_t *pflag);

static constexpr uint32_t PF_CAP = 960;
static constexpr uint32_t PF_HALO = 64;
static constexpr uint32_t PF_CAP_MID = 2048;
static constexpr uint32_t PF_CAP_BIG = 3584;
static constexpr uint32_t PF_COV_MAX = 8192;
static constexpr uint32_t PF_REDO = 1u;
static constexpr uint32_t PF_NEED_BIG = 2u;
struct PfTile {
    const uint64_t *keys;
    const uint32_t *vals;
    const uint32_t *tile_n, *tile_scan;
    const uint16_t *pidx;
    const uint8_t *alive;
    const np2_read_t *reads;
    const uint32_t *tile_rd_off, *tile_rd;
    const uint8_t *refnib;
    uint16_t *slots;
    uint32_t *tile_cnt, *tile_lq;
    long long *tile_gain;
    uint32_t *flags, *n_bad, *bad_list, *n_bad2, *bad_list2;
    long long *end_rel;
    unsigned long long *gain_total;
    unsigned long long *prof;
    uint32_t L, n_tiles, bucket_cap;
    uint32_t cap_lim, cap_lim_big, halo_lim, cov_max;
    uint32_t big_enabled;
};
uint64_t pf_slot_entries(uint32_t n_tiles, uint64_t T);
void launch_pf_tile(hipStream_t s, const PfTile &a);
void launch_pf_compact(hipStream_t s, uint32_t n_tiles, const uint16_t *slots, const uint32_t *tile_scan, const uint32_t *tile_cnt,
                       const uint32_t *tile_coff, const uint32_t *tile_lqoff, uint32_t *cns_pos, uint8_t *cns_base,
                       uint8_t *cns_cls, uint8_t *lq_nothead, uint32_t *lq_list, uint32_t lq_cap, uint32_t *err, uint32_t *flags,
                       uint32_t *flags_out, uint32_t *n_bad, uint32_t *n_bad2);

struct RegionTables {
    const uint32_t *cand_off;
    const uint32_t *order;
    uint16_t *kscore;
    const uint32_t *seq_off;
    const uint8_t *seq;
    uint32_t n_reg;
};
struct RechPtrs {
    const void *groups;
    const uint32_t *job_off;
    const uint32_t *rech;
    const uint32_t *cand_off;
    const uint32_t *keep_list;
    const uint32_t *seq_off;
    const uint8_t *seq;
    const uint8_t *cns_base;
    uint32_t n_groups;
};
void launch_vote_phase(hipStream_t s, const RegionTables &rt, bool asref, bool use_all, const uint32_t *lq_start,
                       uint32_t own_lo, uint32_t own_hi, uint8_t *reg_lable, uint8_t *grp, uint32_t *ecount, int32_t *ref_w,
                       uint8_t *ref_seen, uint8_t *bad, uint32_t *first_reg, uint32_t *err);
void launch_vote_counts(hipStream_t s, const uint32_t *first_reg, const uint8_t *bad, uint32_t R, uint32_t *out);
void launch_edges_write(hipStream_t s, const RegionTables &rt, const uint8_t *reg_lable, const uint8_t *grp,
                        const uint32_t *ecount, const uint32_t *eoff, uint64_t *ekey, uint32_t *eval);
static_assert(EDGE_BAND == 4 * 64, "the band kernels move a read's row as one uint4 per lane of a wavefront");
void launch_edges_row(hipStream_t s, const RegionTables &rt, const uint8_t *grp, const uint32_t *ecount, const uint32_t *pj,
                      const uint32_t *pcount, const uint8_t *alive, uint32_t R, uint32_t *band, uint32_t *row_n, uint32_t *ovf);
void launch_band_emit(hipStream_t s, const uint32_t *band, uint32_t R, const uint32_t *row_off, uint64_t *ukey, uint32_t *uw,
                      uint32_t *n_out, uint64_t key_add = 0);
void launch_vote_rows_count(hipStream_t s, const uint32_t *band, const uint32_t *row_n, const uint8_t *bad, bool use_all, uint32_t R,
                            uint32_t *cnt, uint32_t *nokey);
void launch_vote_rows_emit(hipStream_t s, const uint32_t *band, const uint32_t *row_n, const uint8_t *bad, bool use_all,
                           const uint32_t *first_reg, uint32_t R, const uint32_t *off, void *edges, uint32_t *n_out, uint32_t *nokey);
void launch_edge_reduce(hipStream_t s, const uint64_t *ekey, const uint32_t *eval, uint32_t n, uint32_t *flag, uint32_t *wout);
void launch_edge_compact(hipStream_t s, const uint64_t *ekey, const uint32_t *flag, const uint32_t *idx, const uint32_t *wout,
                         uint32_t n, uint64_t *ukey, uint32_t *uw, uint32_t *n_out);
void launch_seed(hipStream_t s, const RegionTables &rt, int32_t max_indel_len, uint8_t *reg_lable, uint32_t *seed_cand,
                 uint32_t *keep_n, uint32_t *keep_list, uint16_t *keep_ks, uint32_t *err, uint32_t *rl_list = nullptr,
                 uint32_t *rl_cnt = nullptr, uint32_t rl_cap = 0);
uint32_t region_lb_blocks(uint32_t n_reg);
void launch_splice_find(hipStream_t s, const uint32_t *cns_pos, const uint32_t *M_p, const uint32_t *lq_start,
                        const uint32_t *lq_end, const uint8_t *reg_lable, uint8_t lable, uint32_t n_reg, uint32_t *idx_s,
                        uint32_t *idx_e, uint32_t *stuck);
void launch_splice_plan(hipStream_t s, const Lookback &lb, const uint8_t *reg_lable, uint8_t lable, uint32_t n_reg,
                        const uint32_t *stuck, const uint32_t *idx_s, const uint32_t *idx_e, const uint32_t *seed_cand,
                        const uint32_t *seq_off, uint32_t *ap_g, uint32_t *ap_s, uint32_t *ap_e, int32_t *ap_delta,
                        int32_t *ap_shift_incl, uint32_t *n_ap, const uint32_t *M_in, uint32_t *M_out, uint32_t out_cap , uint32_t *err);
void launch_splice_write(hipStream_t s, const uint32_t *in_pos, const uint8_t *in_base, const uint32_t *M_p, uint32_t M_cap,
                         const uint32_t *ap_g, const uint32_t *ap_s, const uint32_t *ap_e, const int32_t *ap_delta,
                         const int32_t *ap_shift_incl, const uint32_t *n_ap, uint32_t max_ap, const uint32_t *lq_start,
                         const uint32_t *seed_cand, const uint32_t *seq_off, const uint8_t *seq, uint32_t *out_pos,
                         uint8_t *out_base);
void launch_shard_bounds(hipStream_t s, const uint32_t *cns_pos, const uint32_t *M_p, const uint32_t *t, uint32_t *out);
void launch_rech_list(hipStream_t s, const Lookback &lb, const uint8_t *reg_lable, uint32_t n_reg, uint32_t *rech,
                      uint32_t *n_rech, unsigned long long *blob_bound, uint32_t *err);
void launch_rech_groups(hipStream_t s, const Lookback &lb, const uint32_t *rech, const uint32_t *n_rech_p, uint32_t max_rech,
                        const uint32_t *cns_pos, const uint32_t *M_p, const uint32_t *lq_start, const uint32_t *lq_end,
                        const uint32_t *keep_n, uint32_t ksize, const uint32_t *reg_maxlen, void *tmp_groups,
                        uint32_t *head_jobs, void *groups, uint32_t *job_off, uint32_t *n_groups, uint32_t *n_jobs,
                        unsigned long long *blob_bound, uint32_t *err);
size_t rech_group_bytes();
void launch_rech_job_len(hipStream_t s, const RechPtrs &p, uint32_t n_jobs, uint32_t *len);
void launch_rech_job_build(hipStream_t s, const RechPtrs &p, uint32_t n_jobs, const uint32_t *soff32, uint64_t *soff64,
                           uint8_t *blob);
void launch_rech_apply(hipStream_t s, const RechPtrs &p, const uint16_t *score, uint16_t *keep_ks);
void launch_rech_select(hipStream_t s, const uint32_t *rech, const uint32_t *n_rech_p, uint32_t max_rech,
                        const uint32_t *cand_off, const uint32_t *keep_n, const uint32_t *keep_list, const uint16_t *keep_ks,
                        const uint32_t *order, bool first_yak, uint8_t *reg_lable, uint32_t *seed_cand);
void launch_rech_relabel(hipStream_t s, uint8_t *reg_lable, uint32_t n_reg);
static constexpr uint32_t RL_CAP_LIST = 1024;
static constexpr uint32_t RL_CAP_JOBS = 2048;
static constexpr uint32_t RL_CAP_BLOB = 1u << 20;
static constexpr uint32_t RL_NREG_MAX = 400000;
enum : uint32_t { RL_N = 0, RL_NGROUPS, RL_NJOBS, RL_OFF, RL_STATE_WORDS };
struct RechList {
    const uint32_t *list_in;
    uint32_t *cnt_in;
    uint32_t *list_out, *cnt_out;
    uint32_t *st;
    uint32_t *rech;
    uint32_t *pos_lo, *pos_ub;
    void *groups, *tmp_groups;
    uint32_t *job_off, *blob_off, *glen;
    uint2 *job_ol;
    uint8_t *blob;
    uint32_t cap_list, cap_jobs, cap_blob;
};
void launch_rech_prepare(hipStream_t s, const RechList &a, const uint32_t *cns_pos, const uint8_t *cns_base, const uint32_t *M_p,
                         const uint32_t *lq_start, const uint32_t *lq_end, const uint32_t *keep_n, uint32_t ksize,
                         const uint32_t *reg_maxlen, const uint32_t *cand_off, const uint32_t *keep_list,
                         const uint32_t *seq_off, const uint8_t *seq, uint32_t *err);
void launch_rech_finish(hipStream_t s, const RechList &a, const uint16_t *score, uint16_t *keep_ks, const uint32_t *cand_off,
                        const uint32_t *keep_n, const uint32_t *keep_list, const uint32_t *order, bool first_yak,
                        bool last_round, uint8_t *reg_lable, uint32_t *seed_cand, const uint32_t *cns_pos,
                        const uint32_t *M_in, const uint32_t *lq_start, const uint32_t *seq_off,
                        uint32_t *ap_g, uint32_t *ap_s, uint32_t *ap_e, int32_t *ap_delta, int32_t *ap_shift_incl,
                        uint32_t *n_ap, uint32_t *M_out, uint32_t out_cap, uint32_t *err);

struct FrontOp {
    uint32_t col0, q0, t0;
    uint32_t len_type;
};
struct FrontRec {
    uint32_t pos, n_ops;
    uint64_t op_off;
    uint64_t seq_off;
    uint64_t out_off;
    uint32_t n_cols;
    uint32_t pad;
};
struct FrontOut {
    uint32_t aln_t_s, aln_t_e, n_cols, pad;
};
void launch_columnarise(hipStream_t s, const FrontRec *recs, uint32_t n_recs, const FrontOp *ops, const uint8_t *ref,
                        const uint8_t *seq4, uint8_t *nib, FrontOut *out);
void launch_pack_ref(hipStream_t s, const uint8_t *ref, uint32_t L, uint8_t *dst);

size_t prim_temp_bytes(size_t n);
int prim_sort_pairs_u64_u32(hipStream_t s, void *tmp, size_t tmp_bytes, const uint64_t *kin, uint64_t *kout,
                            const uint32_t *vin, uint32_t *vout, size_t n, unsigned end_bit);
int prim_exclusive_sum_u32(hipStream_t s, void *tmp, size_t tmp_bytes, const uint32_t *in, uint32_t *out, size_t n);
int prim_exclusive_sum_u32_u64(hipStream_t s, void *tmp, size_t tmp_bytes, const uint32_t *in, uint64_t *out, size_t n);
int prim_inclusive_sum_i32(hipStream_t s, void *tmp, size_t tmp_bytes, const int32_t *in, int32_t *out, size_t n);
int prim_inclusive_min_i32(hipStream_t s, void *tmp, size_t tmp_bytes, const int32_t *in, int32_t *out, size_t n);

}
```

### nextpolish2_amd/csrc/np2_polish.cpp

```cpp
#include "np2_polish.hpp"

#include <algorithm>
#include <cstdio>
#include <cstdlib>
#include <cstring>
#include <functional>
#include <future>
#include <memory>
#include <string>
#include <vector>

using namespace np2;

namespace np2h {
void check_region_err(uint32_t e) {
    if (e & 4u) throw Np2Error(NP2_E_REFPANIC, "reference would panic: seq2 order is equal to 0");
    if (e & 8u) throw Np2Error(NP2_E_REFPANIC, "reference would panic: index out of bounds: lqseq.seqs[max1_p]");
    if (e & 16u) throw Np2Error(NP2_E_REFPANIC, "reference would panic: the first lqseq is not ref.");
    if (e & 32u) throw Np2Error(NP2_E_REFPANIC, "reference would panic: lqseq.seqs[0] after retain_sort_seqs");
    if (e & 64u) throw Np2Error(NP2_E_REFPANIC, "reference would panic: consensus index out of bounds in reupdate");
    if (e & 128u) throw Np2Error(NP2_E_NOMEM, "cartesian product of chained LQ regions is too large");
    if (e & LB_ERR) throw Np2Error(NP2_E_DEVICE, "device-wide scan timed out waiting for a predecessor block");
    if (e & (GROW_ERR | RECH_CAP_ERR)) throw GrowRetry((e & GROW_ERR) != 0, (e & RECH_CAP_ERR) != 0);
    if (e & LQ_LIST_ERR) throw Np2Error(NP2_E_DEVICE, "internal: more low-quality bases than their list was sized for");
}

void trace_cns(np2_ctx *cx, int pass, const std::string &tag, const Cns &c) {
    trace_put(cx, pass, tag + ".pos", c.pos);
    trace_put(cx, pass, tag + ".base", c.base);
}

void trace_region_tables(np2_ctx *cx, int pass, const std::string &tag, const PassCounts &pc, bool kept_view) {
    if (!cx->trace) return;
    const uint32_t n_reg = pc.n_reg;
    auto start = d2h(cx, cx->lq_start.p, n_reg), end = d2h(cx, cx->lq_end.p, n_reg);
    auto coff = d2h(cx, cx->cand_off.p, (size_t)n_reg + 1);
    auto order = d2h(cx, cx->cand_order.p, pc.NC);
    auto ks = d2h(cx, cx->kscore.p, pc.NC);
    auto soff = d2h(cx, cx->cand_seq_off.p, (size_t)pc.NC + 1);
    auto pool = d2h(cx, cx->cand_seq.p, pc.SB);
    std::vector<uint8_t> lable(n_reg, 0);
    std::vector<uint32_t> seedc, keepn, keepl;
    std::vector<uint16_t> keepks;
    if (tag != "cand") lable = d2h(cx, cx->reg_lable.p, n_reg);
    if (kept_view) {
        seedc = d2h(cx, cx->seed_cand.p, n_reg);
        keepn = d2h(cx, cx->keep_n.p, n_reg);
        keepl = d2h(cx, cx->keep_list.p, pc.NC);
        keepks = d2h(cx, cx->keep_ks.p, pc.NC);
    }
    std::vector<uint32_t> o_coff(1, 0), o_order, o_soff(1, 0), sudo_off(1, 0);
    std::vector<uint16_t> o_ks;
    std::vector<uint8_t> o_seq, sudo;
    for (uint32_t g = 0; g < n_reg; ++g) {
        if (kept_view) {
            const uint32_t c = seedc[g];
            if (c != 0xFFFFFFFFu) sudo.insert(sudo.end(), pool.begin() + soff[c], pool.begin() + soff[c + 1]);
            for (uint32_t t = 0; t < keepn[g]; ++t) {
                const uint32_t ci = keepl[coff[g] + t];
                o_order.push_back(order[ci]);
                o_ks.push_back(keepks[coff[g] + t]);
                o_seq.insert(o_seq.end(), pool.begin() + soff[ci], pool.begin() + soff[ci + 1]);
                o_soff.push_back((uint32_t)o_seq.size());
            }
        } else {
            for (uint32_t ci = coff[g]; ci < coff[g + 1]; ++ci) {
                o_order.push_back(order[ci]);
                o_ks.push_back(ks[ci]);
                o_seq.insert(o_seq.end(), pool.begin() + soff[ci], pool.begin() + soff[ci + 1]);
                o_soff.push_back((uint32_t)o_seq.size());
            }
        }
        sudo_off.push_back((uint32_t)sudo.size());
        o_coff.push_back((uint32_t)o_order.size());
    }
    trace_put(cx, pass, tag + ".start", start);
    trace_put(cx, pass, tag + ".end", end);
    trace_put(cx, pass, tag + ".lable", lable);
    trace_put(cx, pass, tag + ".sudo_off", sudo_off);
    trace_put(cx, pass, tag + ".sudo", sudo);
    trace_put(cx, pass, tag + ".cand_off", o_coff);
    trace_put(cx, pass, tag + ".order", o_order);
    trace_put(cx, pass, tag + ".kscore", o_ks);
    trace_put(cx, pass, tag + ".seq_off", o_soff);
    trace_put(cx, pass, tag + ".seq", o_seq);
    if (tag == "cand") trace_put(cx, pass, "cand.kmer", d2h(cx, cx->cand_kmer.p, pc.NC));
}

}

namespace {

void run_diff(np2_ctx *cx, np2_contig *c, uint32_t &T) {
    hipStream_t s = cx->stream;
    const uint32_t L = c->L, R = c->R, NCH = c->n_chunks;
    const uint32_t n_tiles = (L + TILE - 1) >> TILE_SHIFT;
    const uint32_t bcap = std::min(cx->tile_cap, c->tile_cap);
    const uint64_t buckets = (uint64_t)n_tiles * bcap;
    uint64_t ovf_cap = std::max<uint64_t>(c->n_cols / 256 + 65536, 1u << 18);
    cx->tmp.ensure(prim_temp_bytes(std::max<size_t>((size_t)NCH + 2, (size_t)L + 2)));
    cx->tile_n.ensure(n_tiles + 2);
    cx->tile_scan.ensure(n_tiles + 2);
    cx->tile_scanb.ensure(n_tiles + 2);
    cx->tile_nn.ensure(n_tiles + 2);
    cx->tile_nr.ensure(n_tiles + 2);
    cx->tile_noff.ensure(n_tiles + 2);
    cx->tile_roff.ensure(n_tiles + 2);
    cx->tile_gain.ensure(n_tiles + 2);
    if (cx->tile_cur.cap < (size_t)n_tiles + 2) {
        cx->tile_cur.ensure(n_tiles + 2);
        zero32(cx, cx->tile_cur.p, cx->tile_cur.cap);
    }
    if (cx->chunk_st.cap < (size_t)NCH + 2) {
        cx->chunk_st.ensure(NCH + 2);
        zero32(cx, cx->chunk_st.p, cx->chunk_st.cap, 8);
    }
    static const bool precount_env = getenv("NP2_DENSE_PRECOUNT") != nullptr;
    bool precount = precount_env;
    for (int attempt = 0; attempt < 4; ++attempt) {
        if (ovf_cap >= 0xFFFFFFF0ull) throw Np2Error(NP2_E_NOMEM, "too many exception nodes");
        cx->keys_raw.ensure(buckets + ovf_cap + 1);
        cx->vals_raw.ensure(buckets + ovf_cap + 1);
        zero32(cx, cx->scal.p, SCAL_TOTAL);
        if (++cx->chunk_epoch == 0) ++cx->chunk_epoch;
        if (precount) launch_chunk_counts(s, c->descs.p, NCH, c->nib.p, cx->chunk_st.p, cx->chunk_epoch);
        {
            EventTimer t(cx, "diff_reads", true);
            launch_diff_reads(s, c->descs.p, NCH, c->nib.p, (const uint64_t *)c->refnib.p, c->refnib.p, c->refnib.p + c->ref_stride, c->ref_stride, L,
                              cx->keys_raw.p, cx->vals_raw.p, cx->tile_cur.p, n_tiles, bcap, buckets, (uint32_t)ovf_cap,
                              cx->scal.p + S_M3, c->ckpt.p, cx->chunk_st.p, cx->chunk_epoch, cx->scal.p + S_ERR);
        }
        {
            EventTimer t(cx, "sort_exceptions");
            const bool wide = n_tiles >= 2048;
            Lookback lb{};
            if (wide) lb = next_lookback(cx, tile_scan_blocks(n_tiles));
            launch_tile_layout(s, cx->tile_cur.p, n_tiles, bcap, cx->tile_n.p, cx->tile_scan.p, cx->tile_scanb.p,
                               cx->scal.p + S_M3, cx->scal.p + S_M0, wide ? &lb : nullptr, cx->scal.p + S_ERR);
        }
        std::vector<uint32_t> sc = fetch_scal(cx);
        static const bool test_fail = getenv("NP2_TEST_DENSE_LB_FAIL") != nullptr;
        if (test_fail && attempt == 0 && !precount) sc[S_ERR] |= LB_ERR;
        if ((sc[S_ERR] & LB_ERR) && !precount) {
            precount = true;
            continue;
        }
        if (sc[S_ERR] & ~2u) check_region_err(sc[S_ERR] & ~2u);
        if (sc[S_ERR] & 2u)
            throw Np2Error(NP2_E_ARG, "packed read inconsistent with its descriptor (n_cols / aln_t_e / terminator)");
        if (sc[S_M2] > ovf_cap) {
            ovf_cap = (uint64_t)sc[S_M2] * 5 / 4 + 65536;
            continue;
        }
        T = sc[S_M0];
        if (T >= 0xFFFFFFF0u) throw Np2Error(NP2_E_NOMEM, "too many exception nodes");
        cx->tmp.ensure(prim_temp_bytes(std::max<size_t>({(size_t)T + 1, (size_t)L + 2, (size_t)R + 1})));
        EventTimer t(cx, "sort_exceptions");
        if (sc[S_M2] == 0) {
            cx->tile_pidx.ensure((size_t)n_tiles * (TILE / 16) + 64);
            launch_tile_sort(s, cx->tile_pidx.p, c->reads.p, c->nib.p, cx->tile_n.p, n_tiles, bcap, sc[S_M1], cx->keys_raw.p,
                             cx->vals_raw.p, cx->scal.p + S_ERR);
            cx->bucket_cap = bcap;
            cx->pidx_valid = true;
        } else {
            cx->keys.ensure((size_t)T + 1);
            cx->vals.ensure((size_t)T + 1);
            const uint32_t nb = T - sc[S_M2];
            launch_gather_buckets(s, c->reads.p, c->nib.p, cx->tile_n.p, cx->tile_scanb.p, n_tiles, bcap, cx->keys_raw.p,
                                  cx->vals_raw.p, cx->keys.p, cx->vals.p);
            launch_gather_spill(s, c->reads.p, c->nib.p, cx->keys_raw.p + buckets, cx->vals_raw.p + buckets, sc[S_M2],
                                cx->keys.p + nb, cx->vals.p + nb);
            unsigned pos_bits = 1;
            while ((1ull << pos_bits) < (uint64_t)L + 1) ++pos_bits;
            prim_op(cx, [=](hipStream_t st) {
                if (prim_sort_pairs_u64_u32(st, cx->tmp.p, cx->tmp.cap, cx->keys.p, cx->keys_raw.p, cx->vals.p, cx->vals_raw.p,
                                            T, 32 + pos_bits))
                    throw Np2Error(NP2_E_DEVICE, "rocprim radix_sort_pairs failed");
            });
            cx->bucket_cap = 0;
            cx->pidx_valid = false;
        }
        return;
    }
    throw Np2Error(NP2_E_NOMEM, "exception buffer kept overflowing");
}

void build_graph(np2_ctx *cx, np2_contig *c, uint32_t T, uint32_t &n_nodes, uint32_t &n_runs) {
    hipStream_t s = cx->stream;
    const uint32_t L = c->L;
    const uint32_t n_tiles = (L + TILE - 1) >> TILE_SHIFT;
    EventTimer t(cx, "build_graph");
    cx->npos.ensure(T + 1);
    cx->nbases.ensure(T + 1);
    cx->ndelta.ensure(T + 1);
    cx->ncount.ensure(T + 1);
    cx->nminr.ensure(T + 1);
    cx->nscore.ensure(T + 1);
    cx->nbesti.ensure(T + 1);
    cx->nrec.ensure((size_t)T + 32);
    cx->node_off.ensure(L + 16);
    cx->cov.ensure(L + 16);
    cx->pflag.ensure((size_t)L + TILE + 16);
    cx->run_start.ensure(L + 2);
    cx->run_end.ensure(L + 2);
    cx->emit.ensure(L + 2);
    NodeArrays nd{cx->npos.p, cx->nbases.p, cx->ndelta.p, cx->ncount.p, cx->nminr.p};
    launch_tile_count(s, cx->keys_raw.p, cx->vals_raw.p, cx->tile_n.p, cx->tile_scan.p, cx->bucket_cap, n_tiles,
                      cx->alive.p, cx->tile_nn.p, cx->tile_nr.p);
    {
        const bool wide = n_tiles >= 2048;
        Lookback lb{};
        if (wide) lb = next_lookback(cx, tile_scan_blocks(n_tiles));
        launch_tile_offsets(s, cx->tile_nn.p, cx->tile_nr.p, n_tiles, cx->tile_noff.p, cx->tile_roff.p,
                            cx->scal.p + S_NNODES, cx->scal.p + S_NRUNS, cx->scal.p + S_BEST, S_NLQ + 1 - S_BEST,
                            wide ? &lb : nullptr, cx->scal.p + S_ERR);
    }
    launch_tile_write(s, cx->keys_raw.p, cx->vals_raw.p, cx->tile_n.p, cx->tile_scan.p, cx->bucket_cap, cx->tile_noff.p,
                      cx->tile_roff.p, n_tiles, cx->alive.p, L, nd, cx->nrec.p, cx->node_off.p, cx->run_start.p,
                      c->reads.p, c->tile_rd_off.p, c->tile_rd.p, cx->cov.p, c->refnib.p, cx->emit.p,
                      (long long *)cx->tile_gain.p, cx->scal.p + S_DEEP , cx->deep_min,
                      cx->pflag.p);
    n_runs = std::min<uint32_t>(T, L);
    n_nodes = T;
    if (cx->trace) n_nodes = d2h(cx, cx->scal.p + S_NNODES, 1)[0];
}

GraphPtrs graph_ptrs(np2_ctx *cx, np2_contig *c) {
    NodeArrays nd{cx->npos.p, cx->nbases.p, cx->ndelta.p, cx->ncount.p, cx->nminr.p};
    return GraphPtrs{c->refnib.p, cx->node_off.p, nd, cx->cov.p, c->L, cx->nrec.p, cx->scal.p + S_DEEP, cx->pflag.p};
}

void trace_graph(np2_ctx *cx, np2_contig *c, int pass, uint32_t n_nodes) {
    if (!cx->trace) return;
    const uint32_t L = c->L;
    auto off = d2h(cx, cx->node_off.p, (size_t)L + 1);
    auto nb = d2h(cx, cx->nbases.p, n_nodes);
    auto ndl = d2h(cx, cx->ndelta.p, n_nodes);
    auto nc = d2h(cx, cx->ncount.p, n_nodes);
    auto cov = d2h(cx, cx->cov.p, (size_t)L);
    auto rn = d2h(cx, c->refnib.p, (size_t)(L + 1) / 2);
    auto code = [&](uint32_t p) -> unsigned { return (rn[p >> 1] >> (4 * (p & 1))) & 7; };
    std::vector<uint32_t> goff(L + 1, 0), gcount;
    std::vector<uint16_t> gbases, gdelta;
    for (uint32_t p = 0; p < L; ++p) {
// ... 554 lines not shown
```

### nextpolish2_amd/csrc/np2_regions.hip

```cpp
#include "np2_common.hpp"
#include "np2_kernels.hpp"
#include "np2_blockscan.hpp"
#include "np2_lookback.hpp"

namespace np2 {

static constexpr uint8_t LB_TEMP = 0x01, LB_SUCC = 0x80, LB_HETE = 0x40, LB_RECH = 0x20;

__device__ __forceinline__ uint32_t min_support(uint32_t n) { return n >= 9 ? 3u : (n >= 6 ? 2u : 1u); }

struct SubWave {
    uint32_t base;
    bool half;
    __device__ __forceinline__ uint64_t ballot(bool p) const {
        const uint64_t b = __ballot(p);
        return half ? (b >> base) & 0xFFFFFFFFull : b;
    }
    template <class T> __device__ __forceinline__ T shfl(T v, uint32_t j) const { return __shfl(v, (int)(base + j)); }
};

struct WaveStats {
    uint64_t eqmask;
    uint32_t stat;
    uint32_t c;
// ... 586 lines not shown
    cns_span(cns_pos, M, st, en, lo, ub);
    return splice_range(cns_pos, M, st, lo, ub, s, e);
}
__device__ __forceinline__ void splice_plan_total(uint32_t m_in, uint32_t dsum, uint32_t cnt, uint32_t out_cap,
                                                  uint32_t *__restrict__ n_ap, uint32_t *__restrict__ M_out,
                                                  uint32_t *__restrict__ err) {
    const uint32_t m_out = m_in + dsum;
    if (m_out > out_cap) {
        atomicOr(err, GROW_ERR);
        *n_ap = 0;
        *M_out = m_in;
    } else {
        *n_ap = cnt;
        *M_out = m_out;
    }
}
__device__ __forceinline__ void k_splice_find(const uint32_t np2_bid, const uint32_t np2_nb, const uint32_t *__restrict__ cns_pos, const uint32_t *__restrict__ M_p,
                              const uint32_t *__restrict__ lq_start,
                              const uint32_t *__restrict__ lq_end, const uint8_t *__restrict__ reg_lable,
                              uint8_t lable, uint32_t n_reg, uint32_t *__restrict__ idx_s, uint32_t *__restrict__ idx_e,
                              uint32_t *__restrict__ stuck) {
    uint32_t g = np2_bid * blockDim.x + threadIdx.x;
    if (g >= n_reg || !(reg_lable[g] & lable)) return;
    uint32_t s, e;
    const bool found = splice_find_region(cns_pos, *M_p, lq_start[g], lq_end[g], s, e);
    idx_s[g] = s;
    idx_e[g] = e;
    if (!found) atomicMax(stuck, g + 1);
}
static constexpr uint32_t LB_REG_ITEMS = 4;
__device__ __forceinline__ void k_splice_plan(const uint32_t np2_bid, const uint32_t np2_nb, Lookback lb, uint32_t n_blocks, const uint8_t *__restrict__ reg_lable,
                                                     uint8_t lable, uint32_t n_reg, const uint32_t *__restrict__ stuck,
                                                     const uint32_t *__restrict__ idx_s, const uint32_t *__restrict__ idx_e,
                                                     const uint32_t *__restrict__ seed_cand,
                                                     const uint32_t *__restrict__ seq_off, uint32_t *__restrict__ ap_g,
                                                     uint32_t *__restrict__ ap_s, uint32_t *__restrict__ ap_e,
                                                     int32_t *__restrict__ ap_delta, int32_t *__restrict__ ap_shift_incl,
                                                     uint32_t *__restrict__ n_ap, const uint32_t *__restrict__ M_in,
                                                     uint32_t *__restrict__ M_out, uint32_t out_cap, uint32_t *__restrict__ err) {
    __shared__ uint32_t sh[8];
    const uint32_t bid = lb_block_id(lb, sh);
    uint32_t flag[LB_REG_ITEMS], g[LB_REG_ITEMS], s[LB_REG_ITEMS], e[LB_REG_ITEMS];
    int32_t delta[LB_REG_ITEMS];
    uint32_t fsum = 0;
    int32_t dsum_t = 0;
#pragma unroll
    for (uint32_t k = 0; k < LB_REG_ITEMS; ++k) {
        const uint32_t rr = (bid * 256 + threadIdx.x) * LB_REG_ITEMS + k;
        flag[k] = 0, g[k] = 0, s[k] = 0, e[k] = 0, delta[k] = 0;
        if (rr < n_reg) {
            g[k] = n_reg - 1 - rr;
            flag[k] = ((reg_lable[g[k]] & lable) && g[k] + 1 > *stuck) ? 1u : 0u;
            if (flag[k]) {
                const uint32_t c = seed_cand[g[k]];
                s[k] = idx_s[g[k]], e[k] = idx_e[g[k]];
                delta[k] = (int32_t)(seq_off[c + 1] - seq_off[c]) - (int32_t)(e[k] - s[k]);
            }
        }
        fsum += flag[k];
        dsum_t += delta[k];
    }
    uint32_t cnt, dsum;
    uint32_t lo = block_excl_scan<OpAdd, 4>(fsum, sh, cnt);
    uint32_t ld = block_excl_scan<OpAdd, 4>((uint32_t)dsum_t, sh, dsum);
    uint32_t pre_c, pre_d;
    lb_exclusive2(lb, bid, cnt, dsum, sh, err, pre_c, pre_d);
#pragma unroll
    for (uint32_t k = 0; k < LB_REG_ITEMS; ++k) {
        if (flag[k]) {
            const uint32_t o = pre_c + lo;
            ap_g[o] = g[k];
            ap_s[o] = s[k];
            ap_e[o] = e[k];
            ap_delta[o] = delta[k];
            ap_shift_incl[o] = (int32_t)(pre_d + ld) + delta[k];
        }
        lo += flag[k];
        ld += (uint32_t)delta[k];
    }
    if (bid == n_blocks - 1 && threadIdx.x == 0) splice_plan_total(*M_in, pre_d + dsum, pre_c + cnt, out_cap, n_ap, M_out, err);
}
static constexpr uint32_t SPLICE_SPAN = 2048;
static constexpr uint32_t SPLICE_LDS_SLOTS = 256;
__device__ __forceinline__ void k_splice_bases(const uint32_t np2_bid, const uint32_t np2_nb, const uint32_t *__restrict__ in_pos,
                                                      const uint8_t *__restrict__ in_base,
                                                      const uint32_t *__restrict__ M_p,
                                                      const uint32_t *__restrict__ ap_s, const uint32_t *__restrict__ ap_e,
                                                      const int32_t *__restrict__ ap_shift_incl,
                                                      const uint32_t *__restrict__ n_ap_p, uint32_t *__restrict__ out_pos,
                                                      uint8_t *__restrict__ out_base) {
    __shared__ uint32_t s_lo[2];
    __shared__ uint32_t s_s[SPLICE_LDS_SLOTS], s_e[SPLICE_LDS_SLOTS];
    __shared__ int32_t s_sh[SPLICE_LDS_SLOTS];
    const uint32_t i0 = np2_bid * SPLICE_SPAN;
    const uint32_t n_ap = *n_ap_p, M = *M_p;
    if (i0 >= M) return;
    uint32_t pv[SPLICE_SPAN / 256];
    uint8_t bv[SPLICE_SPAN / 256];
#pragma unroll
    for (uint32_t k = 0; k < SPLICE_SPAN / 256; ++k) {
        const uint32_t i = min(i0 + k * 256 + threadIdx.x, M - 1);
        pv[k] = in_pos[i], bv[k] = in_base[i];
    }
    if (threadIdx.x < 2)
        s_lo[threadIdx.x] = upper_bound_u32(ap_s, n_ap, threadIdx.x == 0 ? i0 : min(M - 1, i0 + SPLICE_SPAN - 1));
    __syncthreads();
    const uint32_t blo = s_lo[0], bhi = s_lo[1], b0 = blo ? blo - 1 : 0u;
    const bool staged = bhi - b0 <= SPLICE_LDS_SLOTS;
    if (staged && b0 + threadIdx.x < bhi) {
        s_s[threadIdx.x] = ap_s[b0 + threadIdx.x];
        s_e[threadIdx.x] = ap_e[b0 + threadIdx.x];
        s_sh[threadIdx.x] = ap_shift_incl[b0 + threadIdx.x];
    }
    __syncthreads();
#pragma unroll
    for (uint32_t k = 0; k < SPLICE_SPAN / 256; ++k) {
        const uint32_t i = i0 + k * 256 + threadIdx.x;
        if (i >= M) break;
        uint32_t lo = blo, hi = bhi;
        int64_t o = i;
        if (staged) {
            while (lo < hi) {
                const uint32_t mid = (lo + hi) >> 1;
                if (s_s[mid - b0] <= i) lo = mid + 1; else hi = mid;
            }
            if (lo > 0) {
                if (i < s_e[lo - 1 - b0]) continue;
                o += s_sh[lo - 1 - b0];
            }
        } else {
            while (lo < hi) {
                const uint32_t mid = (lo + hi) >> 1;
                if (ap_s[mid] <= i) lo = mid + 1; else hi = mid;
            }
            if (lo > 0) {
                const uint32_t sl = lo - 1;
                if (i < ap_e[sl]) continue;
                o += ap_shift_incl[sl];
            }
        }
        out_pos[o] = pv[k];
        out_base[o] = bv[k];
    }
}
__device__ __forceinline__ void k_splice_seeds(const uint32_t np2_bid, const uint32_t np2_nb, const uint32_t *__restrict__ ap_g, const uint32_t *__restrict__ ap_s,
                               const int32_t *__restrict__ ap_delta, const int32_t *__restrict__ ap_shift_incl,
                               const uint32_t *__restrict__ n_ap_p, const uint32_t *__restrict__ lq_start,
                               const uint32_t *__restrict__ seed_cand, const uint32_t *__restrict__ seq_off,
                               const uint8_t *__restrict__ seq, uint32_t *__restrict__ out_pos,
                               uint8_t *__restrict__ out_base) {
    const uint32_t sl = (np2_bid * blockDim.x + threadIdx.x) >> 3, q = threadIdx.x & 7u;
    if (sl >= *n_ap_p) return;
    const uint32_t g = ap_g[sl], c = seed_cand[g];
    const uint32_t so = seq_off[c], len = seq_off[c + 1] - so;
    const int64_t o = (int64_t)ap_s[sl] + (ap_shift_incl[sl] - ap_delta[sl]);
    const uint32_t p = lq_start[g];
    for (uint32_t t = q; t < len; t += 8) {
        out_pos[o + t] = p;
        out_base[o + t] = seq[so + t];
    }
}

__device__ __forceinline__ void k_shard_bounds(const uint32_t np2_bid, const uint32_t np2_nb, const uint32_t *__restrict__ cns_pos, const uint32_t *__restrict__ M_p,
                                               uint32_t t0, uint32_t t1, uint32_t t2, uint32_t t3, uint32_t t4, uint32_t t5,
                                               uint32_t *__restrict__ out) {
    __shared__ uint32_t s_i[6];
    const uint32_t M = *M_p;
    const uint32_t t[6] = {t0, t1, t2, t3, t4, t5};
    if (threadIdx.x < 6) {
        uint32_t tv = t[0];
#pragma unroll
        for (uint32_t k = 1; k < 6; ++k) tv = threadIdx.x == k ? t[k] : tv;
        const uint32_t i = lower_bound_u32(cns_pos, M, tv);
        out[threadIdx.x] = i;
        s_i[threadIdx.x] = i;
    }
    __syncthreads();
    if (threadIdx.x == 0) {
        const uint32_t a = s_i[1], b = s_i[4];
        out[6] = b > a ? cns_pos[a] : 0u;
        out[7] = b > a ? cns_pos[b - 1] : 0u;
    }
}

__device__ __forceinline__ void k_rech_list(const uint32_t np2_bid, const uint32_t np2_nb, Lookback lb, uint32_t n_blocks, const uint8_t *__restrict__ reg_lable,
                                                   uint32_t n_reg, uint32_t *__restrict__ rech, uint32_t *__restrict__ n_rech,
                                                   unsigned long long *__restrict__ blob_bound, uint32_t *__restrict__ err) {
    __shared__ uint32_t sh[8];
    if (np2_bid == 0 && threadIdx.x == 0) *blob_bound = 0;
    const uint32_t bid = lb_block_id(lb, sh);
    uint32_t flag[LB_REG_ITEMS], fsum = 0;
#pragma unroll
    for (uint32_t k = 0; k < LB_REG_ITEMS; ++k) {
        const uint32_t rr = (bid * 256 + threadIdx.x) * LB_REG_ITEMS + k;
        flag[k] = (rr < n_reg && (reg_lable[n_reg - 1 - rr] & LB_RECH)) ? 1u : 0u;
        fsum += flag[k];
    }
    uint32_t cnt, pre, dummy;
    uint32_t lo = block_excl_scan<OpAdd, 4>(fsum, sh, cnt);
    lb_exclusive2(lb, bid, cnt, 0u, sh, err, pre, dummy);
#pragma unroll
    for (uint32_t k = 0; k < LB_REG_ITEMS; ++k) {
        if (flag[k]) rech[pre + lo] = n_reg - 1 - ((bid * 256 + threadIdx.x) * LB_REG_ITEMS + k);
        lo += flag[k];
    }
    if (bid == n_blocks - 1 && threadIdx.x == 0) *n_rech = pre + cnt;
}

struct RechGroup {
    uint32_t first, n;
    uint32_t sl, el, sr, er;
    uint32_t bs[5], be[5];
    uint32_t lens[6];
    uint32_t njobs;
};

__device__ __forceinline__ bool rech_chained(const uint32_t *rech, const uint32_t *__restrict__ lq_start,
                                             const uint32_t *__restrict__ lq_end, uint32_t ksize, uint32_t x) {
    return lq_start[rech[x]] < lq_end[rech[x - 1]] + ksize;
}
__device__ __forceinline__ bool rech_is_head(const uint32_t *rech, const uint32_t *__restrict__ lq_start,
                                             const uint32_t *__restrict__ lq_end, uint32_t ksize, uint32_t e) {
    uint32_t back = 0, x = e;
    while (x > 0 && rech_chained(rech, lq_start, lq_end, ksize, x)) {
        --x;
        ++back;
    }
    return back % 6 == 0;
}
struct RechSearch {
    const uint32_t *rech, *cns_pos, *lq_start, *lq_end;
    uint32_t M;
    __device__ __forceinline__ uint32_t lo(uint32_t x) const { return lower_bound_u32(cns_pos, M, lq_start[rech[x]]); }
    __device__ __forceinline__ uint32_t ub(uint32_t x) const { return upper_bound_u32(cns_pos, M, lq_end[rech[x]]); }
};
struct RechFound {
    const uint32_t *s_lo, *s_ub;
    __device__ __forceinline__ uint32_t lo(uint32_t x) const { return s_lo[x]; }
    __device__ __forceinline__ uint32_t ub(uint32_t x) const { return s_ub[x]; }
};
template <class Where>
__device__ __forceinline__ RechGroup rech_group_build(uint32_t e, uint32_t n_rech, const uint32_t *rech, const Where &where,
                                                      uint32_t M, const uint32_t *__restrict__ lq_start,
// ... 177 lines not shown
                                 uint8_t *__restrict__ blob) {
    uint32_t j = np2_bid * blockDim.x + threadIdx.x;
    if (j < n_jobs) rech_string<true>(cx, j, blob + soff[j]);
}
__device__ __forceinline__ void k_u32_to_u64_off(const uint32_t np2_bid, const uint32_t np2_nb, const uint32_t *__restrict__ in, uint32_t n, uint64_t *__restrict__ out) {
    uint32_t i = np2_bid * blockDim.x + threadIdx.x;
    if (i < n) out[i] = in[i];
}

__device__ __forceinline__ void rech_apply_group(const RechCtx &cx, uint32_t gi, const uint16_t *__restrict__ score,
                                                 uint16_t *__restrict__ keep_ks) {
    const RechGroup &G = cx.groups[gi];
    const uint32_t j0 = cx.job_off[gi];
    if (G.n == 1) {
        const uint32_t g = cx.rech[G.first];
        for (uint32_t t = 0; t < G.lens[0]; ++t) keep_ks[cx.cand_off[g] + t] = score[j0 + t];
        return;
    }
    for (uint32_t x = 0; x < G.n; ++x) {
        const uint32_t g = cx.rech[G.first + x];
        for (uint32_t t = 0; t < G.lens[x]; ++t) keep_ks[cx.cand_off[g] + t] = 0;
    }
    for (uint32_t j = 0; j < G.njobs; ++j) {
        const uint16_t ks = score[j0 + j];
        if (!ks) continue;
        uint32_t rem = j;
        for (uint32_t x = G.n; x-- > 0;) {
            const uint32_t p = rem % G.lens[x];
            rem /= G.lens[x];
            keep_ks[cx.cand_off[cx.rech[G.first + x]] + p] = ks;
        }
    }
}
__device__ __forceinline__ void k_rech_apply(const uint32_t np2_bid, const uint32_t np2_nb, RechCtx cx, const uint16_t *__restrict__ score, uint16_t *__restrict__ keep_ks) {
    uint32_t gi = np2_bid * blockDim.x + threadIdx.x;
    if (gi < cx.n_groups) rech_apply_group(cx, gi, score, keep_ks);
}

__device__ __forceinline__ void rech_select_region(uint32_t g, const uint32_t *__restrict__ cand_off,
                                                   const uint32_t *__restrict__ keep_n, const uint32_t *__restrict__ keep_list,
                                                   const uint16_t *__restrict__ keep_ks, const uint32_t *__restrict__ order,
                                                   uint32_t first_yak, uint8_t *__restrict__ reg_lable,
                                                   uint32_t *__restrict__ seed_cand) {
    const uint32_t c0 = cand_off[g], n = keep_n[g];
    uint32_t c = 0, valid = 0;
    for (uint32_t p = 0; p < n; ++p)
        if (keep_ks[c0 + p] != 0) {
            if (c == 0 || order[keep_list[c0 + p]] == 0) c = p + 1;
            ++valid;
        }
    if (valid > 1) reg_lable[g] |= LB_TEMP;
    if (c != 0) {
        seed_cand[g] = keep_list[c0 + c - 1];
    } else if (first_yak) {
        uint32_t i = 0;
        for (uint32_t p = 0; p < n; ++p)
            if (order[keep_list[c0 + p]] == 0) {
                i = p;
                break;
            }
        seed_cand[g] = keep_list[c0 + i];
    }
}
__device__ __forceinline__ void k_rech_select(const uint32_t np2_bid, const uint32_t np2_nb, const uint32_t *__restrict__ rech, const uint32_t *__restrict__ n_rech_p,
                              const uint32_t *__restrict__ cand_off, const uint32_t *__restrict__ keep_n,
                              const uint32_t *__restrict__ keep_list, const uint16_t *__restrict__ keep_ks,
                              const uint32_t *__restrict__ order, uint32_t first_yak, uint8_t *__restrict__ reg_lable,
                              uint32_t *__restrict__ seed_cand) {
    uint32_t e = np2_bid * blockDim.x + threadIdx.x;
    if (e >= *n_rech_p) return;
    rech_select_region(rech[e], cand_off, keep_n, keep_list, keep_ks, order, first_yak, reg_lable, seed_cand);
}
__device__ __forceinline__ uint8_t rech_relabel(uint8_t l) {
    return (l & LB_TEMP) ? (uint8_t)(l ^ LB_TEMP) : (uint8_t)(l ^ LB_RECH);
}
__device__ __forceinline__ void k_rech_relabel(const uint32_t np2_bid, const uint32_t np2_nb, uint8_t *__restrict__ reg_lable, uint32_t n_reg) {
    uint32_t g = np2_bid * blockDim.x + threadIdx.x;
    if (g >= n_reg) return;
    const uint8_t l = reg_lable[g];
    if (l & LB_RECH) reg_lable[g] = rech_relabel(l);
}

static constexpr uint32_t RL_ITEMS = 4;
static_assert(RL_CAP_LIST == 256 * RL_ITEMS, "a thread of the list kernels owns RL_ITEMS consecutive entries");
static_assert((uint64_t)RL_CAP_LIST * (RL_CAP_JOBS + 1) < (1ull << 32) && (uint64_t)RL_CAP_LIST * (RL_CAP_BLOB + 1) < (1ull << 32),
              "clamped per-group sums stay inside 32 bits");

__device__ __forceinline__ RechCtx rl_ctx(const RechList &a, const uint32_t *rech, const uint32_t *__restrict__ cand_off,
                                          const uint32_t *__restrict__ keep_list, const uint32_t *__restrict__ seq_off,
                                          const uint8_t *__restrict__ seq, const uint8_t *__restrict__ cns_base, uint32_t n_groups) {
    return RechCtx{(const RechGroup *)a.groups, a.job_off, rech, cand_off, keep_list, seq_off, seq, cns_base, n_groups};
}
__device__ __forceinline__ void rl_round_off(const RechList &a, uint32_t cap_err, uint32_t *__restrict__ err) {
    a.st[RL_N] = 0, a.st[RL_NGROUPS] = 0, a.st[RL_NJOBS] = 0, a.st[RL_OFF] = 1;
    if (cap_err) atomicOr(err, RECH_CAP_ERR);
}

__device__ __forceinline__ void k_rech_prepare(const uint32_t np2_bid, const uint32_t np2_nb, RechList a,
                                               const uint32_t *__restrict__ cns_pos, const uint8_t *__restrict__ cns_base,
                                               const uint32_t *__restrict__ M_p, const uint32_t *__restrict__ lq_start,
                                               const uint32_t *__restrict__ lq_end, const uint32_t *__restrict__ keep_n,
                                               uint32_t ksize, const uint32_t *__restrict__ reg_maxlen,
                                               const uint32_t *__restrict__ cand_off, const uint32_t *__restrict__ keep_list,
                                               const uint32_t *__restrict__ seq_off, const uint8_t *__restrict__ seq,
                                               uint32_t *__restrict__ err) {
    __shared__ uint32_t s_raw[RL_CAP_LIST], s_rech[RL_CAP_LIST], s_lo[RL_CAP_LIST], s_ub[RL_CAP_LIST], sh[8], s_hdr[2];
    const uint32_t tid = threadIdx.x;
    if (tid == 0) s_hdr[0] = *err, s_hdr[1] = *a.cnt_in;
    __syncthreads();
    const uint32_t n = s_hdr[1], cap_list = min(a.cap_list, RL_CAP_LIST);
    if (s_hdr[0] != 0 || n > cap_list) {
        if (tid == 0) rl_round_off(a, s_hdr[0] == 0, err);
        return;
    }
    for (uint32_t i = tid; i < n; i += 256) s_raw[i] = a.list_in[i];
    __syncthreads();
    for (uint32_t i = tid; i < n; i += 256) {
        const uint32_t v = s_raw[i];
        uint32_t rank = 0;
        for (uint32_t j = 0; j < n; ++j) rank += s_raw[j] > v ? 1u : 0u;
        s_rech[rank] = v;
        a.rech[rank] = v;
    }
    __syncthreads();
    const uint32_t M = *M_p;
    for (uint32_t i = tid; i < n; i += 256) {
        const uint32_t g = s_rech[i];
        uint32_t lo, ub;
        cns_span(cns_pos, M, lq_start[g], lq_end[g], lo, ub);
        s_lo[i] = lo, s_ub[i] = ub;
        a.pos_lo[i] = lo, a.pos_ub[i] = ub;
    }
    __syncthreads();
    RechGroup *const groups = (RechGroup *)a.groups, *const tmp_groups = (RechGroup *)a.tmp_groups;
    uint32_t head[RL_ITEMS], jobs[RL_ITEMS], bytes[RL_ITEMS], glen[RL_ITEMS], hs = 0, js = 0, bsum = 0;
#pragma unroll
    for (uint32_t k = 0; k < RL_ITEMS; ++k) {
        const uint32_t e = tid * RL_ITEMS + k;
        head[k] = (e < n && rech_is_head(s_rech, lq_start, lq_end, ksize, e)) ? 1u : 0u;
        jobs[k] = 0, bytes[k] = 0, glen[k] = 0;
        if (head[k]) {
            uint64_t len;
            const RechGroup G = rech_group_build(e, n, s_rech, RechFound{s_lo, s_ub}, M, lq_start, lq_end, keep_n, ksize, reg_maxlen, err, len);
            tmp_groups[e] = G;
            jobs[k] = min(G.njobs, a.cap_jobs + 1u);
            glen[k] = (uint32_t)min(len, (uint64_t)a.cap_blob + 1u);
            bytes[k] = (uint32_t)min((uint64_t)G.njobs * len, (uint64_t)a.cap_blob + 1u);
        }
        hs += head[k], js += jobs[k], bsum += bytes[k];
    }
    uint32_t nh, nj, nb;
    uint32_t lh = block_excl_scan<OpAdd, 4>(hs, sh, nh);
    uint32_t lj = block_excl_scan<OpAdd, 4>(js, sh, nj);
    uint32_t lbt = block_excl_scan<OpAdd, 4>(bsum, sh, nb);
    if (nj > min(a.cap_jobs, RL_CAP_JOBS) || nb > min(a.cap_blob, RL_CAP_BLOB)) {
        if (tid == 0) rl_round_off(a, 1u, err);
        return;
    }
#pragma unroll
    for (uint32_t k = 0; k < RL_ITEMS; ++k) {
        if (!head[k]) continue;
        groups[lh] = tmp_groups[tid * RL_ITEMS + k];
        a.job_off[lh] = lj;
        a.blob_off[lh] = lbt;
        a.glen[lh] = glen[k];
        ++lh, lj += jobs[k], lbt += bytes[k];
    }
    if (tid == 0) {
        a.job_off[nh] = nj;
        a.st[RL_N] = n, a.st[RL_NGROUPS] = nh, a.st[RL_NJOBS] = nj, a.st[RL_OFF] = 0;
    }
    __threadfence_block();
    __syncthreads();
    const RechCtx cx = rl_ctx(a, s_rech, cand_off, keep_list, seq_off, seq, cns_base, nh);
    for (uint32_t j = tid >> 4; j < nj; j += 16) {
        const uint32_t gi = job_group(cx, j), rem = j - a.job_off[gi];
        const uint32_t off = a.blob_off[gi] + rem * a.glen[gi];
        uint32_t len = rech_group_string<false>(cx, gi, rem, nullptr);
        if (len <= a.glen[gi]) {
            rech_group_string<true>(cx, gi, rem, a.blob + off, tid & 15u, 16u);
        } else {
            if ((tid & 15u) == 0) atomicOr(err, RECH_CAP_ERR);
            len = 0;
        }
        if ((tid & 15u) == 0) a.job_ol[j] = make_uint2(off, len);
    }
}

__device__ __forceinline__ void k_rech_finish(const uint32_t np2_bid, const uint32_t np2_nb, RechList a,
                                              const uint16_t *__restrict__ score, uint16_t *__restrict__ keep_ks,
                                              const uint32_t *__restrict__ cand_off, const uint32_t *__restrict__ keep_n,
                                              const uint32_t *__restrict__ keep_list, const uint32_t *__restrict__ order,
                                              uint32_t first_yak, uint32_t last_round, uint8_t *__restrict__ reg_lable,
                                              uint32_t *__restrict__ seed_cand, const uint32_t *__restrict__ cns_pos,
                                              const uint32_t *__restrict__ M_in, const uint32_t *__restrict__ lq_start,
                                              const uint32_t *__restrict__ seq_off,
                                              uint32_t *__restrict__ ap_g, uint32_t *__restrict__ ap_s,
                                              uint32_t *__restrict__ ap_e, int32_t *__restrict__ ap_delta,
                                              int32_t *__restrict__ ap_shift_incl, uint32_t *__restrict__ n_ap,
                                              uint32_t *__restrict__ M_out, uint32_t out_cap, uint32_t *__restrict__ err) {
    __shared__ uint32_t sh[8], s_hdr[4], s_stuck;
    const uint32_t tid = threadIdx.x;
    if (tid == 0) s_hdr[0] = *err, s_hdr[1] = a.st[RL_N], s_hdr[2] = a.st[RL_NGROUPS], s_hdr[3] = a.st[RL_OFF], s_stuck = 0;
    __syncthreads();
    if (s_hdr[0] != 0 || s_hdr[3] != 0) {
        if (tid == 0) *n_ap = 0, *M_out = *M_in, *a.cnt_in = 0, *a.cnt_out = 0;
        return;
    }
    const uint32_t n = s_hdr[1], n_groups = s_hdr[2], M = *M_in;
    const RechCtx cx = rl_ctx(a, a.rech, cand_off, keep_list, seq_off, nullptr, nullptr, n_groups);
    for (uint32_t gi = tid; gi < n_groups; gi += 256) rech_apply_group(cx, gi, score, keep_ks);
    __threadfence_block();
    __syncthreads();
    uint32_t g[RL_ITEMS], s[RL_ITEMS], e[RL_ITEMS];
#pragma unroll
    for (uint32_t k = 0; k < RL_ITEMS; ++k) {
        const uint32_t x = tid * RL_ITEMS + k;
        g[k] = 0, s[k] = 0, e[k] = 0;
        if (x >= n) continue;
        g[k] = a.rech[x];
        rech_select_region(g[k], cand_off, keep_n, keep_list, keep_ks, order, first_yak, reg_lable, seed_cand);
        if (!splice_range(cns_pos, M, lq_start[g[k]], a.pos_lo[x], a.pos_ub[x], s[k], e[k])) atomicMax(&s_stuck, g[k] + 1);
    }
    __syncthreads();
    const uint32_t stuck = s_stuck;
    uint32_t flag[RL_ITEMS], fsum = 0;
    int32_t delta[RL_ITEMS], dsum_t = 0;
#pragma unroll
    for (uint32_t k = 0; k < RL_ITEMS; ++k) {
        flag[k] = (tid * RL_ITEMS + k < n && g[k] + 1 > stuck) ? 1u : 0u;
        delta[k] = 0;
        if (flag[k]) {
            const uint32_t c = seed_cand[g[k]];
            delta[k] = (int32_t)(seq_off[c + 1] - seq_off[c]) - (int32_t)(e[k] - s[k]);
        }
        fsum += flag[k], dsum_t += delta[k];
    }
    uint32_t cnt, dsum;
    uint32_t lo = block_excl_scan<OpAdd, 4>(fsum, sh, cnt);
    uint32_t ld = block_excl_scan<OpAdd, 4>((uint32_t)dsum_t, sh, dsum);
#pragma unroll
    for (uint32_t k = 0; k < RL_ITEMS; ++k) {
        if (flag[k]) {
            ap_g[lo] = g[k];
            ap_s[lo] = s[k];
            ap_e[lo] = e[k];
            ap_delta[lo] = delta[k];
            ap_shift_incl[lo] = (int32_t)ld + delta[k];
        }
        lo += flag[k];
        ld += (uint32_t)delta[k];
    }
    if (tid == 0) splice_plan_total(M, dsum, cnt, out_cap, n_ap, M_out, err);
    uint32_t keep[RL_ITEMS], ksum = 0;
#pragma unroll
    for (uint32_t k = 0; k < RL_ITEMS; ++k) {
        keep[k] = 0;
        if (tid * RL_ITEMS + k < n) {
            const uint8_t l = rech_relabel(reg_lable[g[k]]);
            reg_lable[g[k]] = l;
            keep[k] = (l & LB_RECH) ? 1u : 0u;
        }
        ksum += keep[k];
    }
    uint32_t n_keep;
    uint32_t lk = block_excl_scan<OpAdd, 4>(ksum, sh, n_keep);
#pragma unroll
    for (uint32_t k = 0; k < RL_ITEMS; ++k) {
        if (keep[k]) a.list_out[lk] = g[k];
        lk += keep[k];
    }
    if (tid == 0) *a.cnt_in = 0, *a.cnt_out = last_round ? 0u : n_keep;
}

__device__ __forceinline__ void k_vote_counts(const uint32_t np2_bid, const uint32_t np2_nb, const uint32_t *__restrict__ first_reg, const uint8_t *__restrict__ bad,
                                                      uint32_t R, uint32_t *__restrict__ out) {
    __shared__ uint32_t sk[16], sb[16];
    uint32_t nk = 0, nb = 0;
    for (uint32_t r = threadIdx.x; r < R; r += 1024) {
        nk += first_reg[r] != 0xFFFFFFFFu ? 1u : 0u;
        nb += bad[r] ? 1u : 0u;
    }
    for (int o = 32; o > 0; o >>= 1) {
        nk += __shfl_xor(nk, o);
        nb += __shfl_xor(nb, o);
    }
    if ((threadIdx.x & 63) == 0) {
        sk[threadIdx.x >> 6] = nk;
        sb[threadIdx.x >> 6] = nb;
    }
    __syncthreads();
    if (threadIdx.x == 0) {
        uint32_t a = 0, b = 0;
        for (int i = 0; i < 16; ++i) {
            a += sk[i];
            b += sb[i];
        }
        out[0] = a;
        out[1] = b;
    }
}

static inline dim3 g1(uint64_t n, uint32_t bs = 256) { return dim3((unsigned)((n + bs - 1) / bs)); }

void launch_vote_phase(hipStream_t s, const RegionTables &rt, bool asref, bool use_all, const uint32_t *lq_start,
                       uint32_t own_lo, uint32_t own_hi, uint8_t *reg_lable, uint8_t *grp, uint32_t *ecount, int32_t *ref_w,
                       uint8_t *ref_seen, uint8_t *bad, uint32_t *first_reg, uint32_t *err) {
    if (rt.n_reg)
        NP2_LAUNCH(k_vote_phase, g1((uint64_t)((rt.n_reg + 1) / 2) * 64), 256, s, rt, asref ? 1u : 0u, use_all ? 1u : 0u, lq_start, own_lo, own_hi, reg_lable, grp, ecount, ref_w, ref_seen, bad, first_reg, err);
}
void launch_vote_counts(hipStream_t s, const uint32_t *first_reg, const uint8_t *bad, uint32_t R, uint32_t *out) {
    NP2_LAUNCH(k_vote_counts, dim3(1), 1024, s, first_reg, bad, R, out);
}
void launch_edges_write(hipStream_t s, const RegionTables &rt, const uint8_t *reg_lable, const uint8_t *grp,
                        const uint32_t *ecount, const uint32_t *eoff, uint64_t *ekey, uint32_t *eval) {
    if (rt.n_reg)
        NP2_LAUNCH(k_edges_write, g1((uint64_t)rt.n_reg * 64), 256, s, rt, reg_lable, grp, ecount, eoff, ekey, eval);
}
void launch_edges_row(hipStream_t s, const RegionTables &rt, const uint8_t *grp, const uint32_t *ecount, const uint32_t *pj,
                      const uint32_t *pcount, const uint8_t *alive, uint32_t R, uint32_t *band, uint32_t *row_n, uint32_t *ovf) {
    if (R) NP2_LAUNCH(k_edges_row, g1((uint64_t)R * 64), 256, s, rt, grp, ecount, pj, pcount, alive, R, band, row_n, ovf);
}
void launch_vote_rows_count(hipStream_t s, const uint32_t *band, const uint32_t *row_n, const uint8_t *bad, bool use_all, uint32_t R,
                            uint32_t *cnt, uint32_t *nokey) {
    if (R) NP2_LAUNCH(k_vote_rows_count, g1((uint64_t)R * 64), 256, s, band, row_n, bad, use_all ? 1u : 0u, R, cnt, nokey);
}
void launch_vote_rows_emit(hipStream_t s, const uint32_t *band, const uint32_t *row_n, const uint8_t *bad, bool use_all,
                           const uint32_t *first_reg, uint32_t R, const uint32_t *off, void *edges, uint32_t *n_out, uint32_t *nokey) {
    if (R) NP2_LAUNCH(k_vote_rows_emit, g1((uint64_t)R * 64), 256, s, band, row_n, bad, use_all ? 1u : 0u, first_reg, R, off, (uint2 *)edges, n_out, nokey);
}
void launch_band_emit(hipStream_t s, const uint32_t *band, uint32_t R, const uint32_t *row_off, uint64_t *ukey, uint32_t *uw,
                      uint32_t *n_out, uint64_t key_add) {
    if (R) NP2_LAUNCH(k_band_emit, g1((uint64_t)R * 64), 256, s, band, R, row_off, ukey, uw, n_out, key_add);
}
void launch_edge_reduce(hipStream_t s, const uint64_t *ekey, const uint32_t *eval, uint32_t n, uint32_t *flag,
                        uint32_t *wout) {
    if (n) NP2_LAUNCH(k_edge_reduce, g1(n), 256, s, ekey, eval, n, flag, wout);
}
void launch_edge_compact(hipStream_t s, const uint64_t *ekey, const uint32_t *flag, const uint32_t *idx,
                         const uint32_t *wout, uint32_t n, uint64_t *ukey, uint32_t *uw, uint32_t *n_out) {
    if (n) NP2_LAUNCH(k_edge_compact, g1(n), 256, s, ekey, flag, idx, wout, n, ukey, uw, n_out);
}
void launch_seed(hipStream_t s, const RegionTables &rt, int32_t max_indel_len, uint8_t *reg_lable, uint32_t *seed_cand,
                 uint32_t *keep_n, uint32_t *keep_list, uint16_t *keep_ks, uint32_t *err, uint32_t *rl_list, uint32_t *rl_cnt,
                 uint32_t rl_cap) {
    if (rt.n_reg)
        NP2_LAUNCH(k_seed, g1((uint64_t)((rt.n_reg + 1) / 2) * 64), 256, s, rt, max_indel_len, reg_lable, seed_cand, keep_n, keep_list, keep_ks, err, rl_list, rl_cnt, rl_cap);
}
uint32_t region_lb_blocks(uint32_t n_reg) { return (n_reg + 256 * LB_REG_ITEMS - 1) / (256 * LB_REG_ITEMS); }
void launch_splice_find(hipStream_t s, const uint32_t *cns_pos, const uint32_t *M_p, const uint32_t *lq_start,
                        const uint32_t *lq_end, const uint8_t *reg_lable, uint8_t lable, uint32_t n_reg,
                        uint32_t *idx_s, uint32_t *idx_e, uint32_t *stuck) {
    NP2_LAUNCH(k_splice_find, g1(n_reg), 256, s, cns_pos, M_p, lq_start, lq_end, reg_lable, lable, n_reg, idx_s, idx_e, stuck);
}
void launch_splice_plan(hipStream_t s, const Lookback &lb, const uint8_t *reg_lable, uint8_t lable, uint32_t n_reg,
                        const uint32_t *stuck, const uint32_t *idx_s, const uint32_t *idx_e, const uint32_t *seed_cand,
                        const uint32_t *seq_off, uint32_t *ap_g, uint32_t *ap_s, uint32_t *ap_e, int32_t *ap_delta,
                        int32_t *ap_shift_incl, uint32_t *n_ap, const uint32_t *M_in, uint32_t *M_out, uint32_t out_cap, uint32_t *err) {
    const uint32_t nb = region_lb_blocks(n_reg);
    NP2_LAUNCH(k_splice_plan, dim3(nb), 256, s, lb, nb, reg_lable, lable, n_reg, stuck, idx_s, idx_e, seed_cand, seq_off, ap_g, ap_s, ap_e, ap_delta, ap_shift_incl, n_ap, M_in, M_out, out_cap, err);
}
void launch_splice_write(hipStream_t s, const uint32_t *in_pos, const uint8_t *in_base, const uint32_t *M_p, uint32_t M_cap,
                         const uint32_t *ap_g, const uint32_t *ap_s, const uint32_t *ap_e, const int32_t *ap_delta,
                         const int32_t *ap_shift_incl, const uint32_t *n_ap, uint32_t max_ap, const uint32_t *lq_start,
                         const uint32_t *seed_cand, const uint32_t *seq_off, const uint8_t *seq, uint32_t *out_pos,
                         uint8_t *out_base) {
    NP2_LAUNCH(k_splice_bases, dim3((M_cap + SPLICE_SPAN - 1) / SPLICE_SPAN), 256, s, in_pos, in_base, M_p, ap_s, ap_e, ap_shift_incl, n_ap, out_pos, out_base);
    if (max_ap)
        NP2_LAUNCH(k_splice_seeds, g1((uint64_t)max_ap * 8, 256), 256, s, ap_g, ap_s, ap_delta, ap_shift_incl, n_ap, lq_start, seed_cand, seq_off, seq, out_pos, out_base);
}
void launch_shard_bounds(hipStream_t s, const uint32_t *cns_pos, const uint32_t *M_p, const uint32_t *t, uint32_t *out) {
    NP2_LAUNCH(k_shard_bounds, dim3(1), 64, s, cns_pos, M_p, t[0], t[1], t[2], t[3], t[4], t[5], out);
}
void launch_rech_list(hipStream_t s, const Lookback &lb, const uint8_t *reg_lable, uint32_t n_reg, uint32_t *rech,
                      uint32_t *n_rech, unsigned long long *blob_bound, uint32_t *err) {
    const uint32_t nb = region_lb_blocks(n_reg);
    NP2_LAUNCH(k_rech_list, dim3(nb), 256, s, lb, nb, reg_lable, n_reg, rech, n_rech, blob_bound, err);
}
void launch_rech_groups(hipStream_t s, const Lookback &lb, const uint32_t *rech, const uint32_t *n_rech_p, uint32_t max_rech,
                        const uint32_t *cns_pos, const uint32_t *M_p, const uint32_t *lq_start, const uint32_t *lq_end,
                        const uint32_t *keep_n, uint32_t ksize, const uint32_t *reg_maxlen, void *tmp_groups,
                        uint32_t *head_jobs, void *groups, uint32_t *job_off, uint32_t *n_groups, uint32_t *n_jobs,
                        unsigned long long *blob_bound, uint32_t *err) {
    NP2_LAUNCH(k_rech_groups, dim3((max_rech + 255) / 256), 256, s, rech, n_rech_p, cns_pos, M_p, lq_start, lq_end, keep_n, ksize, reg_maxlen, (RechGroup *)tmp_groups, head_jobs, blob_bound, err);
    const uint32_t nb = region_lb_blocks(max_rech);
    NP2_LAUNCH(k_rech_compact, dim3(nb), 256, s, lb, nb, n_rech_p, head_jobs, (const RechGroup *)tmp_groups, (RechGroup *)groups, job_off, n_groups, n_jobs, err);
}
size_t rech_group_bytes() { return sizeof(RechGroup); }
static RechCtx mk_rech(const RechPtrs &p) {
    return RechCtx{(const RechGroup *)p.groups, p.job_off, p.rech, p.cand_off, p.keep_list, p.seq_off, p.seq,
                   p.cns_base, p.n_groups};
}
void launch_rech_job_len(hipStream_t s, const RechPtrs &p, uint32_t n_jobs, uint32_t *len) {
    if (n_jobs) NP2_LAUNCH(k_rech_job_len, g1(n_jobs, 64), 64, s, mk_rech(p), n_jobs, len);
}
void launch_rech_job_build(hipStream_t s, const RechPtrs &p, uint32_t n_jobs, const uint32_t *soff32, uint64_t *soff64,
                           uint8_t *blob) {
    if (!n_jobs) return;
    NP2_LAUNCH(k_u32_to_u64_off, g1(n_jobs + 1), 256, s, soff32, n_jobs + 1, soff64);
    NP2_LAUNCH(k_rech_job_build, g1(n_jobs, 64), 64, s, mk_rech(p), n_jobs, soff64, blob);
}
void launch_rech_apply(hipStream_t s, const RechPtrs &p, const uint16_t *score, uint16_t *keep_ks) {
    if (p.n_groups) NP2_LAUNCH(k_rech_apply, g1(p.n_groups, 64), 64, s, mk_rech(p), score, keep_ks);
}
void launch_rech_select(hipStream_t s, const uint32_t *rech, const uint32_t *n_rech_p, uint32_t max_rech,
                        const uint32_t *cand_off, const uint32_t *keep_n, const uint32_t *keep_list,
                        const uint16_t *keep_ks, const uint32_t *order, bool first_yak, uint8_t *reg_lable,
                        uint32_t *seed_cand) {
    if (max_rech)
        NP2_LAUNCH(k_rech_select, g1(max_rech, 64), 64, s, rech, n_rech_p, cand_off, keep_n, keep_list, keep_ks, order, first_yak ? 1u : 0u, reg_lable, seed_cand);
}
void launch_rech_relabel(hipStream_t s, uint8_t *reg_lable, uint32_t n_reg) {
    NP2_LAUNCH(k_rech_relabel, g1(n_reg), 256, s, reg_lable, n_reg);
}
void launch_rech_prepare(hipStream_t s, const RechList &a, const uint32_t *cns_pos, const uint8_t *cns_base, const uint32_t *M_p,
                         const uint32_t *lq_start, const uint32_t *lq_end, const uint32_t *keep_n, uint32_t ksize,
                         const uint32_t *reg_maxlen, const uint32_t *cand_off, const uint32_t *keep_list,
                         const uint32_t *seq_off, const uint8_t *seq, uint32_t *err) {
    NP2_LAUNCH(k_rech_prepare, dim3(1), 256, s, a, cns_pos, cns_base, M_p, lq_start, lq_end, keep_n, ksize, reg_maxlen, cand_off, keep_list, seq_off, seq, err);
}
void launch_rech_finish(hipStream_t s, const RechList &a, const uint16_t *score, uint16_t *keep_ks, const uint32_t *cand_off,
                        const uint32_t *keep_n, const uint32_t *keep_list, const uint32_t *order, bool first_yak,
                        bool last_round, uint8_t *reg_lable, uint32_t *seed_cand, const uint32_t *cns_pos,
                        const uint32_t *M_in, const uint32_t *lq_start, const uint32_t *seq_off,
                        uint32_t *ap_g, uint32_t *ap_s, uint32_t *ap_e, int32_t *ap_delta, int32_t *ap_shift_incl,
                        uint32_t *n_ap, uint32_t *M_out, uint32_t out_cap, uint32_t *err) {
    NP2_LAUNCH(k_rech_finish, dim3(1), 256, s, a, score, keep_ks, cand_off, keep_n, keep_list, order, first_yak ? 1u : 0u, last_round ? 1u : 0u, reg_lable, seed_cand, cns_pos, M_in, lq_start, seq_off, ap_g, ap_s, ap_e, ap_delta, ap_shift_incl, n_ap, M_out, out_cap, err);
}

}
```

Baseline: 4488.

## Fuse recheck round kernels, merge splice launches, and add register-resident tile sort

The list-based recheck's prepare, k-mer scoring and finish kernels become one single-block kernel that keeps per-round state in shared memory. The two splice-write kernels become one launch, and tile sort gains a register-staged fast path for tiles up to 2048 entries, flagging overfull tiles as heavy for the larger-capacity kernel. The goal is fewer launches and less global-memory round-tripping, at the cost of scoring all jobs inside a single workgroup, which can serialise large job counts.

```diff
diff --git a/nextpolish2_amd/csrc/np2_ctx.hpp b/nextpolish2_amd/csrc/np2_ctx.hpp
--- a/nextpolish2_amd/csrc/np2_ctx.hpp
+++ b/nextpolish2_amd/csrc/np2_ctx.hpp
@@ -524,6 +524,7 @@
     uint32_t deep_min = 65536;
     DevBuf<uint32_t> lq_list, hbits;
     DevBuf<uint16_t> tile_pidx;
+    DevBuf<uint8_t> tile_heavy;
     bool pidx_valid = false;
     DevBuf<ReadInfo> rinfo;
     DevBuf<uint32_t> lqc, lqoff;
diff --git a/nextpolish2_amd/csrc/np2_final.cpp b/nextpolish2_amd/csrc/np2_final.cpp
--- a/nextpolish2_amd/csrc/np2_final.cpp
+++ b/nextpolish2_amd/csrc/np2_final.cpp
@@ -68,10 +68,8 @@
     EventTimer t(cx, "recheck");
     const uint32_t ksize = cx->yaks[yak_idx].k;
     const uint32_t cap_jobs = std::min(cx->hooks.rech_cap_jobs, RL_CAP_JOBS), cap_blob = std::min(cx->hooks.rech_cap_blob, RL_CAP_BLOB);
-    cx->rech.ensure(RL_CAP_LIST + 2);
     cx->rech_groups.ensure((size_t)(RL_CAP_LIST + 2) * rech_group_bytes());
     cx->rech_groups_tmp.ensure((size_t)(RL_CAP_LIST + 2) * rech_group_bytes());
-    cx->rech_joboff.ensure(RL_CAP_LIST + 2);
     cx->rl_blob_off.ensure(RL_CAP_LIST + 2);
     cx->rl_glen.ensure(RL_CAP_LIST + 2);
     cx->rl_job_ol.ensure(RL_CAP_JOBS + 2);
@@ -80,17 +78,14 @@
     const CnsDev out = splice_buffers(cx, in, std::max(pc.n_reg, RL_CAP_LIST), pc.grow, to_b, version);
     uint32_t *const st = cx->scal.p + S_RL + 2, *const nap_p = cx->scal.p + S_COUNT + 2 * version + 1;
     const RechList rl{rech_list_of(cx, (size_t)yak_idx), rech_list_cnt(cx, (size_t)yak_idx), rech_list_of(cx, (size_t)yak_idx + 1),
-                      rech_list_cnt(cx, (size_t)yak_idx + 1), st, cx->rech.p, cx->sp_idx_s.p, cx->sp_idx_e.p, cx->rech_groups.p, cx->rech_groups_tmp.p,
-                      cx->rech_joboff.p, cx->rl_blob_off.p, cx->rl_glen.p, cx->rl_job_ol.p, cx->sstr.p,
+                      rech_list_cnt(cx, (size_t)yak_idx + 1), st, cx->rech_groups.p, cx->rech_groups_tmp.p,
+                      cx->rl_blob_off.p, cx->rl_glen.p, cx->rl_job_ol.p, cx->sstr.p,
                       rech_list_cap(cx), cap_jobs, cap_blob};
-    launch_rech_prepare(s, rl, in.pos, in.base, in.M_p, cx->lq_start.p, cx->lq_end.p, cx->keep_n.p, ksize, cx->reg_maxlen.p,
-                        cx->cand_off.p, cx->keep_list.p, cx->cand_seq_off.p, cx->cand_seq.p, cx->scal.p + S_ERR);
-    launch_score_jobs(s, cx->yaks[yak_idx].dev(), cx->sstr.p, cx->rl_job_ol.p, st + RL_NJOBS, min_kmer_count,
-                      cx->sscore.p);
-    launch_rech_finish(s, rl, cx->sscore.p, cx->keep_ks.p, cx->cand_off.p, cx->keep_n.p, cx->keep_list.p, cx->cand_order.p,
-                       first_yak, last_yak, cx->reg_lable.p, cx->seed_cand.p, in.pos, in.M_p, cx->lq_start.p,
-                       cx->cand_seq_off.p, cx->ap_g.p, cx->ap_s.p, cx->ap_e.p, cx->ap_delta.p, cx->ap_shift.p, nap_p, cx->mlen.p + version,
-                       out.M_cap, cx->scal.p + S_ERR);
+    launch_rech_round(s, rl, cx->yaks[yak_idx].dev(), min_kmer_count, cx->sscore.p, in.pos, in.base, in.M_p, cx->lq_start.p,
+                      cx->lq_end.p, cx->keep_n.p, ksize, cx->reg_maxlen.p, cx->cand_off.p, cx->keep_list.p, cx->cand_seq_off.p,
+                      cx->cand_seq.p, cx->keep_ks.p, cx->cand_order.p, first_yak, last_yak, cx->reg_lable.p, cx->seed_cand.p,
+                      cx->ap_g.p, cx->ap_s.p, cx->ap_e.p, cx->ap_delta.p, cx->ap_shift.p, nap_p, cx->mlen.p + version,
+                      out.M_cap, cx->scal.p + S_ERR);
     launch_splice_write(s, in.pos, in.base, in.M_p, in.M_cap, cx->ap_g.p, cx->ap_s.p, cx->ap_e.p, cx->ap_delta.p,
                         cx->ap_shift.p, nap_p, RL_CAP_LIST, cx->lq_start.p, cx->seed_cand.p, cx->cand_seq_off.p,
                         cx->cand_seq.p, out.pos, out.base);
diff --git a/nextpolish2_amd/csrc/np2_graph.hip b/nextpolish2_amd/csrc/np2_graph.hip
--- a/nextpolish2_amd/csrc/np2_graph.hip
+++ b/nextpolish2_amd/csrc/np2_graph.hip
@@ -47,7 +47,8 @@
 __device__ __forceinline__ void k_tile_layout(const uint32_t np2_bid, const uint32_t np2_nb, uint32_t *__restrict__ tile_cur, uint32_t n_tiles,
                                                       uint32_t bucket_cap, uint32_t *__restrict__ tile_n,
                                                       uint32_t *__restrict__ tile_scan, uint32_t *__restrict__ tile_scanb,
-                                                      const uint32_t *__restrict__ ovf_cnt, uint32_t *__restrict__ out) {
+                                                      const uint32_t *__restrict__ ovf_cnt, uint32_t *__restrict__ out,
+                                                      uint8_t *__restrict__ heavy) {
     __shared__ uint32_t sh[16];
     const uint32_t ta = block_scan_array<OpAdd>(
         n_tiles, sh, [&](uint32_t i) { return tile_cur[i]; },
@@ -59,7 +60,11 @@
         n_tiles, sh, [&](uint32_t i) { return min(tile_n[i], bucket_cap); },
         [&](uint32_t i, uint32_t pre, uint32_t) { tile_scanb[i] = pre; });
     const uint32_t mx = block_scan_array<OpMaxU32>(
-        n_tiles, sh, [&](uint32_t i) { return tile_n[i]; }, [&](uint32_t i, uint32_t, uint32_t) { tile_cur[i] = 0; });
+        n_tiles, sh, [&](uint32_t i) { return tile_n[i]; },
+        [&](uint32_t i, uint32_t, uint32_t) {
+            tile_cur[i] = 0;
+            if (heavy) heavy[i] = 0;
+        });
     if (threadIdx.x == 0) {
         tile_scan[n_tiles] = ta;
         tile_scanb[n_tiles] = tb;
@@ -74,7 +79,7 @@
                                                         uint32_t n_tiles, uint32_t bucket_cap, uint32_t *__restrict__ tile_n,
                                                         uint32_t *__restrict__ tile_scan, uint32_t *__restrict__ tile_scanb,
                                                         const uint32_t *__restrict__ ovf_cnt, uint32_t *__restrict__ out,
-                                                        uint32_t *__restrict__ err) {
+                                                        uint32_t *__restrict__ err, uint8_t *__restrict__ heavy) {
     __shared__ uint32_t sh[8];
     const uint32_t bid = lb_block_id(lb, sh);
     const uint32_t i0 = (bid * 256 + threadIdx.x) * TLB_ITEMS;
@@ -100,6 +105,7 @@
             tile_scanb[i0 + k] = rb;
             tile_n[i0 + k] = v[k];
             tile_cur[i0 + k] = 0;
+            if (heavy) heavy[i0 + k] = 0;
             ra += v[k];
             rb += min(v[k], bucket_cap);
         }
@@ -111,12 +117,108 @@
     }
 }
 
+static constexpr uint32_t TS_REGS = 8;
 template <uint32_t CAP>
 __device__ __forceinline__ void k_tile_sort(const uint32_t np2_bid, const uint32_t np2_nb, uint16_t *__restrict__ pidx, const np2_read_t *__restrict__ reads,
                                                    const uint8_t *__restrict__ nib, const uint32_t *__restrict__ tile_n,
                                                    uint32_t bucket_cap, uint64_t *__restrict__ keys,
                                                    uint32_t *__restrict__ vals, uint32_t *__restrict__ err,
-                                                   uint32_t n_above, uint32_t n_upto) {
+                                                   uint8_t *__restrict__ heavy);
+template <>
+__device__ __forceinline__ void k_tile_sort<1024>(const uint32_t np2_bid, const uint32_t np2_nb, uint16_t *__restrict__ pidx, const np2_read_t *__restrict__ reads,
+                                                         const uint8_t *__restrict__ nib, const uint32_t *__restrict__ tile_n,
+                                                         uint32_t bucket_cap, uint64_t *__restrict__ keys,
+                                                         uint32_t *__restrict__ vals, uint32_t *__restrict__ err,
+                                                         uint8_t *__restrict__ heavy) {
+    constexpr uint32_t CAP = 1024;
+    __shared__ uint32_t s_klo[CAP];
+    __shared__ uint32_t s_v[CAP];
+    __shared__ uint16_t s_q[CAP];
+    __shared__ uint32_t s_cnt[TILE];
+    __shared__ uint16_t s_off[TILE + 2];
+    __shared__ uint32_t sh[8];
+    const uint32_t n = tile_n[np2_bid], tid = threadIdx.x;
+    const uint64_t a = (uint64_t)np2_bid * bucket_cap;
+    if (n == 0 || n > TS_REGS * 256) return;
+    const uint32_t start = np2_bid << TILE_SHIFT;
+    for (uint32_t i = tid; i < TILE; i += 256) s_cnt[i] = 0;
+    __syncthreads();
+    uint32_t r_klo[TS_REGS], r_v[TS_REGS], r_q[TS_REGS];
+#pragma unroll
+    for (uint32_t k = 0; k < TS_REGS; ++k) {
+        const uint32_t i = tid + k * 256;
+        r_klo[k] = 0, r_v[k] = 0, r_q[k] = 0xFFFFFFFFu;
+        if (i < n) {
+            const uint32_t r = vals[a + i];
+            const uint64_t key = make_node_key(reads, nib, keys[a + i], r);
+            uint32_t q = (uint32_t)(key >> 32) - start;
+            if (q >= TILE) {
+                atomicOr(err, 8u);
+                q = TILE - 1;
+            }
+            r_klo[k] = (uint32_t)key, r_v[k] = r, r_q[k] = q;
+            atomicAdd(&s_cnt[q], 1u);
+        }
+    }
+    __syncthreads();
+    uint32_t one_pos_too_many;
+    {
+        const uint32_t q0 = tid * 4;
+        const uint32_t c0 = s_cnt[q0], c1 = s_cnt[q0 + 1], c2 = s_cnt[q0 + 2], c3 = s_cnt[q0 + 3];
+        uint32_t tot;
+        const uint32_t l0 = block_excl_scan_256(c0 + c1 + c2 + c3, sh, tot);
+        s_off[q0] = (uint16_t)l0, s_off[q0 + 1] = (uint16_t)(l0 + c0), s_off[q0 + 2] = (uint16_t)(l0 + c0 + c1), s_off[q0 + 3] = (uint16_t)(l0 + c0 + c1 + c2);
+        if (tid == 0) s_off[TILE] = (uint16_t)n;
+        s_cnt[q0] = 0, s_cnt[q0 + 1] = 0, s_cnt[q0 + 2] = 0, s_cnt[q0 + 3] = 0;
+        one_pos_too_many = __syncthreads_or((c0 > CAP || c1 > CAP || c2 > CAP || c3 > CAP) ? 1 : 0);
+    }
+    if (one_pos_too_many) {
+        if (tid == 0) heavy[np2_bid] = 1;
+        return;
+    }
+    if (tid < TILE / 16) pidx[(size_t)np2_bid * (TILE / 16) + tid] = s_off[tid * 16];
+    for (uint32_t qa = 0, qb; qa < TILE; qa = qb) {
+        const uint32_t base = s_off[qa];
+        if (base >= n) break;
+        qb = TILE;
+        if (n - base > CAP) {
+            uint32_t lo = qa + 1, hi = TILE - 1;
+            while (lo < hi) {
+                const uint32_t mid = (lo + hi + 1) >> 1;
+                if (s_off[mid] - base <= CAP) lo = mid; else hi = mid - 1;
+            }
+            qb = lo;
+        }
+        const uint32_t m = s_off[qb] - base;
+#pragma unroll
+        for (uint32_t k = 0; k < TS_REGS; ++k) {
+            const uint32_t q = r_q[k];
+            if (q >= qa && q < qb) {
+                const uint32_t d = s_off[q] - base + atomicAdd(&s_cnt[q], 1u);
+                s_klo[d] = r_klo[k], s_v[d] = r_v[k], s_q[d] = (uint16_t)q;
+            }
+        }
+        __syncthreads();
+        for (uint32_t d = tid; d < m; d += 256) {
+            const uint32_t q = s_q[d], b = s_off[q] - base, c = s_cnt[q];
+            const uint32_t klo = s_klo[d], v = s_v[d];
+            uint32_t rank = 0;
+            for (uint32_t e = b; e < b + c; ++e) {
+                const uint32_t kj = s_klo[e], vj = s_v[e];
+                rank += (kj < klo || (kj == klo && vj < v)) ? 1u : 0u;
+            }
+            keys[a + base + b + rank] = ((uint64_t)(start + q) << 32) | klo;
+            vals[a + base + b + rank] = v;
+        }
+        __syncthreads();
+    }
+}
+template <uint32_t CAP>
+__device__ __forceinline__ void k_tile_sort(const uint32_t np2_bid, const uint32_t np2_nb, uint16_t *__restrict__ pidx, const np2_read_t *__restrict__ reads,
+                                                   const uint8_t *__restrict__ nib, const uint32_t *__restrict__ tile_n,
+                                                   uint32_t bucket_cap, uint64_t *__restrict__ keys,
+                                                   uint32_t *__restrict__ vals, uint32_t *__restrict__ err,
+                                                   uint8_t *__restrict__ heavy) {
     __shared__ uint32_t s_klo[CAP];
     __shared__ uint32_t s_v[CAP];
     __shared__ uint16_t s_q[CAP];
@@ -126,7 +228,7 @@
     __shared__ uint32_t sh[8];
     const uint32_t n = tile_n[np2_bid], tid = threadIdx.x;
     const uint64_t a = (uint64_t)np2_bid * bucket_cap;
-    if (n <= n_above || n > n_upto) return;
+    if (n <= TS_REGS * 256 && !heavy[np2_bid]) return;
     if (n > CAP) {
         if (tid == 0) atomicOr(err, 8u);
         return;
@@ -689,25 +791,21 @@
 uint32_t tile_scan_blocks(uint32_t n_tiles) { return (n_tiles + 256 * TLB_ITEMS - 1) / (256 * TLB_ITEMS); }
 void launch_tile_layout(hipStream_t s, uint32_t *tile_cur, uint32_t n_tiles, uint32_t bucket_cap, uint32_t *tile_n,
                         uint32_t *tile_scan, uint32_t *tile_scanb, const uint32_t *ovf_cnt, uint32_t *out,
-                        const Lookback *lb, uint32_t *err) {
+                        const Lookback *lb, uint32_t *err, uint8_t *heavy) {
     if (lb)
-        NP2_LAUNCH(k_tile_layout_lb, dim3(tile_scan_blocks(n_tiles)), 256, s, *lb, tile_scan_blocks(n_tiles), tile_cur, n_tiles, bucket_cap, tile_n, tile_scan, tile_scanb, ovf_cnt, out, err);
+        NP2_LAUNCH(k_tile_layout_lb, dim3(tile_scan_blocks(n_tiles)), 256, s, *lb, tile_scan_blocks(n_tiles), tile_cur, n_tiles, bucket_cap, tile_n, tile_scan, tile_scanb, ovf_cnt, out, err, heavy);
     else
-        NP2_LAUNCH(k_tile_layout, dim3(1), 1024, s, tile_cur, n_tiles, bucket_cap, tile_n, tile_scan, tile_scanb, ovf_cnt, out);
+        NP2_LAUNCH(k_tile_layout, dim3(1), 1024, s, tile_cur, n_tiles, bucket_cap, tile_n, tile_scan, tile_scanb, ovf_cnt, out, heavy);
 }
 void launch_tile_sort(hipStream_t s, uint16_t *pidx, const np2_read_t *reads, const uint8_t *nib, const uint32_t *tile_n,
                       uint32_t n_tiles, uint32_t bucket_cap, uint32_t max_tile, uint64_t *keys, uint32_t *vals,
-                      uint32_t *err) {
-    const uint32_t ALL = 0xFFFFFFFFu;
-    if (max_tile <= 1024) {
-        NP2_LAUNCH(k_tile_sort<1024>, dim3(n_tiles), 256, s, pidx, reads, nib, tile_n, bucket_cap, keys, vals, err, 0u, ALL);
-    } else {
-        NP2_LAUNCH(k_tile_sort<1024>, dim3(n_tiles), 256, s, pidx, reads, nib, tile_n, bucket_cap, keys, vals, err, 0u, 1024u);
-        if (max_tile <= 2048 && TILE_CAP > 2048)
-            NP2_LAUNCH(k_tile_sort<2048>, dim3(n_tiles), 256, s, pidx, reads, nib, tile_n, bucket_cap, keys, vals, err, 1024u, ALL);
-        else
-            NP2_LAUNCH(k_tile_sort<TILE_CAP>, dim3(n_tiles), 256, s, pidx, reads, nib, tile_n, bucket_cap, keys, vals, err, 1024u, ALL);
-    }
+                      uint32_t *err, uint8_t *heavy) {
+    NP2_LAUNCH(k_tile_sort<1024>, dim3(n_tiles), 256, s, pidx, reads, nib, tile_n, bucket_cap, keys, vals, err, heavy);
+    if (max_tile <= 1024) return;
+    if (max_tile <= 2048 && TILE_CAP > 2048)
+        NP2_LAUNCH(k_tile_sort<2048>, dim3(n_tiles), 256, s, pidx, reads, nib, tile_n, bucket_cap, keys, vals, err, heavy);
+    else
+        NP2_LAUNCH(k_tile_sort<TILE_CAP>, dim3(n_tiles), 256, s, pidx, reads, nib, tile_n, bucket_cap, keys, vals, err, heavy);
 }
 void launch_gather_buckets(hipStream_t s, const np2_read_t *reads, const uint8_t *nib, const uint32_t *tile_n,
                            const uint32_t *tile_scanb, uint32_t n_tiles, uint32_t bucket_cap, const uint64_t *bkeys,
diff --git a/nextpolish2_amd/csrc/np2_kernels.hip b/nextpolish2_amd/csrc/np2_kernels.hip
--- a/nextpolish2_amd/csrc/np2_kernels.hip
+++ b/nextpolish2_amd/csrc/np2_kernels.hip
@@ -1237,42 +1237,6 @@
     for (int o = 32; o > 0; o >>= 1) mn = min(mn, (uint32_t)__shfl_xor(mn, o));
     return mn == 0xFFFFFFFFu ? (uint16_t)0 : (uint16_t)mn;
 }
-__device__ __forceinline__ uint16_t wave_score_string(const YakDev &y, const uint8_t *__restrict__ s, uint32_t len,
-                                                      uint16_t min_count) {
-    const uint32_t lane = threadIdx.x & 63;
-    const uint32_t k = y.k;
-    const uint64_t mask = (1ULL << (2 * (uint64_t)k)) - 1;
-    uint32_t mn = 0xFFFFFFFFu;
-    if (len >= k) {
-        for (uint32_t st = lane; st + k <= len; st += 64) {
-            uint64_t codes = 0, bad = 0;
-#pragma unroll
-            for (uint32_t wd = 0; wd < 4; ++wd) {
-                uint64_t x;
-                __builtin_memcpy(&x, s + st + 8 * wd, 8);
-                uint64_t c = ((x >> 1) ^ (x >> 2)) & 0x0303030303030303ULL;
-                c = (c | (c >> 6)) & 0x000F000F000F000FULL;
-                c = (c | (c >> 12)) & 0x000000FF000000FFULL;
-                c = (c | (c >> 24)) & 0xFFFFULL;
-                codes |= c << (16 * wd);
-                uint64_t b = (x >> 3) & 0x0101010101010101ULL;
-                b = (b | (b >> 7)) & 0x0003000300030003ULL;
-                b = (b | (b >> 14)) & 0x0000000F0000000FULL;
-                b = (b | (b >> 28)) & 0xFFULL;
-                bad |= b << (8 * wd);
-            }
-            if ((bad & ((1ULL << k) - 1ULL)) == 0) {
-                codes &= mask;
-                uint64_t rb = __builtin_bitreverse64(codes);
-                rb = ((rb >> 1) & 0x5555555555555555ULL) | ((rb & 0x5555555555555555ULL) << 1);
-                const uint64_t fw = rb >> (64 - 2 * k), rv = ~codes & mask;
-                mn = min(mn, (uint32_t)yak_get(y, yak_hash64(fw < rv ? fw : rv, mask), min_count));
-            }
-        }
-    }
-    for (int o = 32; o > 0; o >>= 1) mn = min(mn, (uint32_t)__shfl_xor(mn, o));
-    return mn == 0xFFFFFFFFu ? (uint16_t)0 : (uint16_t)mn;
-}
 
 __device__ __forceinline__ void k_score_strings(const uint32_t np2_bid, const uint32_t np2_nb, YakDev y, const uint8_t *__restrict__ strs, const uint64_t *__restrict__ off,
                                 uint64_t n, uint16_t min_count, uint16_t *__restrict__ out, uint32_t own_strings) {
@@ -1281,16 +1245,6 @@
     const uint16_t sc = own_strings ? wave_score_string(y, strs + off[w], (uint32_t)(off[w + 1] - off[w]), min_count)
                                     : wave_score_string_any(y, strs + off[w], (uint32_t)(off[w + 1] - off[w]), min_count);
     if ((threadIdx.x & 63) == 0) out[w] = sc;
-}
-
-__device__ __forceinline__ void k_score_jobs(const uint32_t np2_bid, const uint32_t np2_nb, YakDev y, const uint8_t *__restrict__ strs, const uint2 *__restrict__ job_ol,
-                                             const uint32_t *__restrict__ n_jobs_p, uint16_t min_count, uint16_t *__restrict__ out) {
-    const uint32_t n = *n_jobs_p, n_waves = np2_nb * (blockDim.x >> 6);
-    for (uint32_t w = np2_bid * (blockDim.x >> 6) + (uint32_t)__builtin_amdgcn_readfirstlane((int)(threadIdx.x >> 6)); w < n; w += n_waves) {
-        const uint2 ol = job_ol[w];
-        const uint16_t sc = wave_score_string(y, strs + ol.x, ol.y, min_count);
-        if ((threadIdx.x & 63) == 0) out[w] = sc;
-    }
 }
 
 __device__ __forceinline__ void k_cand_score(const uint32_t np2_bid, const uint32_t np2_nb, YakDev y, const uint32_t *__restrict__ cand_seq_off, const uint64_t *__restrict__ cand_kmer,
@@ -1462,10 +1416,6 @@
                    uint16_t *out) {
     if (n) NP2_LAUNCH(k_lookup, grid1(n), 256, s, y, hashes, n, min_count, out);
 }
-void launch_score_jobs(hipStream_t s, const YakDev &y, const uint8_t *strs, const uint2 *job_ol, const uint32_t *n_jobs_p,
-                       uint16_t min_count, uint16_t *out) {
-    NP2_LAUNCH(k_score_jobs, dim3(16), 256, s, y, strs, job_ol, n_jobs_p, min_count, out);
-}
 void launch_score_strings(hipStream_t s, const YakDev &y, const uint8_t *strs, const uint64_t *off, uint64_t n,
                           uint16_t min_count, uint16_t *out, bool own_strings) {
     if (n) NP2_LAUNCH(k_score_strings, grid1(n * 64), 256, s, y, strs, off, n, min_count, out, own_strings ? 1u : 0u);
diff --git a/nextpolish2_amd/csrc/np2_kernels.hpp b/nextpolish2_amd/csrc/np2_kernels.hpp
--- a/nextpolish2_amd/csrc/np2_kernels.hpp
+++ b/nextpolish2_amd/csrc/np2_kernels.hpp
@@ -3,6 +3,7 @@
 #include <cstdint>
 #include <hip/hip_runtime.h>
 #include "../../include/np2.h"
+#include "np2_common.hpp"
 #include "np2_lookback.hpp"
 #include "np2_launch.hpp"
 #include "np2_vote_band.hpp"
@@ -106,6 +107,42 @@
         }
         s = (s + 1) & capm;
     }
+}
+__device__ __forceinline__ uint16_t wave_score_string(const YakDev &y, const uint8_t *__restrict__ s, uint32_t len,
+                                                      uint16_t min_count) {
+    const uint32_t lane = threadIdx.x & 63;
+    const uint32_t k = y.k;
+    const uint64_t mask = (1ULL << (2 * (uint64_t)k)) - 1;
+    uint32_t mn = 0xFFFFFFFFu;
+    if (len >= k) {
+        for (uint32_t st = lane; st + k <= len; st += 64) {
+            uint64_t codes = 0, bad = 0;
+#pragma unroll
+            for (uint32_t wd = 0; wd < 4; ++wd) {
+                uint64_t x;
+                __builtin_memcpy(&x, s + st + 8 * wd, 8);
+                uint64_t c = ((x >> 1) ^ (x >> 2)) & 0x0303030303030303ULL;
+                c = (c | (c >> 6)) & 0x000F000F000F000FULL;
+                c = (c | (c >> 12)) & 0x000000FF000000FFULL;
+                c = (c | (c >> 24)) & 0xFFFFULL;
+                codes |= c << (16 * wd);
+                uint64_t b = (x >> 3) & 0x0101010101010101ULL;
+                b = (b | (b >> 7)) & 0x0003000300030003ULL;
+                b = (b | (b >> 14)) & 0x0000000F0000000FULL;
+                b = (b | (b >> 28)) & 0xFFULL;
+                bad |= b << (8 * wd);
+            }
+            if ((bad & ((1ULL << k) - 1ULL)) == 0) {
+                codes &= mask;
+                uint64_t rb = __builtin_bitreverse64(codes);
+                rb = ((rb >> 1) & 0x5555555555555555ULL) | ((rb & 0x5555555555555555ULL) << 1);
+                const uint64_t fw = rb >> (64 - 2 * k), rv = ~codes & mask;
+                mn = min(mn, (uint32_t)yak_get(y, yak_hash64(fw < rv ? fw : rv, mask), min_count));
+            }
+        }
+    }
+    for (int o = 32; o > 0; o >>= 1) mn = min(mn, (uint32_t)__shfl_xor(mn, o));
+    return mn == 0xFFFFFFFFu ? (uint16_t)0 : (uint16_t)mn;
 }
 #endif
 
@@ -173,8 +210,6 @@
 void launch_lookup(hipStream_t s, const YakDev &y, const uint64_t *hashes, uint64_t n, uint16_t min_count, uint16_t *out);
 void launch_score_strings(hipStream_t s, const YakDev &y, const uint8_t *strs, const uint64_t *off, uint64_t n,
                           uint16_t min_count, uint16_t *out, bool own_strings);
-void launch_score_jobs(hipStream_t s, const YakDev &y, const uint8_t *strs, const uint2 *job_ol, const uint32_t *n_jobs_p,
-                       uint16_t min_count, uint16_t *out);
 void launch_cand_score(hipStream_t s, const YakDev &y, const uint32_t *cand_seq_off, const uint8_t *cand_seq,
                        const uint64_t *cand_kmer, const uint32_t *n_cand_p, uint32_t cand_cap, uint16_t min_count,
                        uint16_t *kscore, uint32_t *long_list, uint32_t *n_long);
@@ -206,10 +241,10 @@
 uint32_t tile_scan_blocks(uint32_t n_tiles);
 void launch_tile_layout(hipStream_t s, uint32_t *tile_cur, uint32_t n_tiles, uint32_t bucket_cap, uint32_t *tile_n,
                         uint32_t *tile_scan, uint32_t *tile_scanb, const uint32_t *ovf_cnt, uint32_t *out,
-                        const Lookback *lb = nullptr, uint32_t *err = nullptr);
+                        const Lookback *lb = nullptr, uint32_t *err = nullptr, uint8_t *heavy = nullptr);
 void launch_tile_sort(hipStream_t s, uint16_t *pidx, const np2_read_t *reads, const uint8_t *nib, const uint32_t *tile_n,
                       uint32_t n_tiles, uint32_t bucket_cap, uint32_t max_tile, uint64_t *keys, uint32_t *vals,
-                      uint32_t *err);
+                      uint32_t *err, uint8_t *heavy);
 void launch_gather_buckets(hipStream_t s, const np2_read_t *reads, const uint8_t *nib, const uint32_t *tile_n,
                            const uint32_t *tile_scanb, uint32_t n_tiles, uint32_t bucket_cap, const uint64_t *bkeys,
                            const uint32_t *bvals, uint64_t *keys, uint32_t *vals);
@@ -343,24 +378,19 @@
     uint32_t *cnt_in;
     uint32_t *list_out, *cnt_out;
     uint32_t *st;
-    uint32_t *rech;
-    uint32_t *pos_lo, *pos_ub;
     void *groups, *tmp_groups;
-    uint32_t *job_off, *blob_off, *glen;
+    uint32_t *blob_off, *glen;
     uint2 *job_ol;
     uint8_t *blob;
     uint32_t cap_list, cap_jobs, cap_blob;
 };
-void launch_rech_prepare(hipStream_t s, const RechList &a, const uint32_t *cns_pos, const uint8_t *cns_base, const uint32_t *M_p,
-                         const uint32_t *lq_start, const uint32_t *lq_end, const uint32_t *keep_n, uint32_t ksize,
-                         const uint32_t *reg_maxlen, const uint32_t *cand_off, const uint32_t *keep_list,
-                         const uint32_t *seq_off, const uint8_t *seq, uint32_t *err);
-void launch_rech_finish(hipStream_t s, const RechList &a, const uint16_t *score, uint16_t *keep_ks, const uint32_t *cand_off,
-                        const uint32_t *keep_n, const uint32_t *keep_list, const uint32_t *order, bool first_yak,
-                        bool last_round, uint8_t *reg_lable, uint32_t *seed_cand, const uint32_t *cns_pos,
-                        const uint32_t *M_in, const uint32_t *lq_start, const uint32_t *seq_off,
-                        uint32_t *ap_g, uint32_t *ap_s, uint32_t *ap_e, int32_t *ap_delta, int32_t *ap_shift_incl,
-                        uint32_t *n_ap, uint32_t *M_out, uint32_t out_cap, uint32_t *err);
+void launch_rech_round(hipStream_t s, const RechList &a, const YakDev &y, uint16_t min_count, uint16_t *score,
+                       const uint32_t *cns_pos, const uint8_t *cns_base, const uint32_t *M_in, const uint32_t *lq_start,
+                       const uint32_t *lq_end, const uint32_t *keep_n, uint32_t ksize, const uint32_t *reg_maxlen,
+                       const uint32_t *cand_off, const uint32_t *keep_list, const uint32_t *seq_off, const uint8_t *seq,
+                       uint16_t *keep_ks, const uint32_t *order, bool first_yak, bool last_round, uint8_t *reg_lable,
+                       uint32_t *seed_cand, uint32_t *ap_g, uint32_t *ap_s, uint32_t *ap_e, int32_t *ap_delta,
+                       int32_t *ap_shift_incl, uint32_t *n_ap, uint32_t *M_out, uint32_t out_cap, uint32_t *err);
 
 struct FrontOp {
     uint32_t col0, q0, t0;
diff --git a/nextpolish2_amd/csrc/np2_polish.cpp b/nextpolish2_amd/csrc/np2_polish.cpp
--- a/nextpolish2_amd/csrc/np2_polish.cpp
+++ b/nextpolish2_amd/csrc/np2_polish.cpp
@@ -100,6 +100,7 @@
     uint64_t ovf_cap = std::max<uint64_t>(c->n_cols / 256 + 65536, 1u << 18);
     cx->tmp.ensure(prim_temp_bytes(std::max<size_t>((size_t)NCH + 2, (size_t)L + 2)));
     cx->tile_n.ensure(n_tiles + 2);
+    cx->tile_heavy.ensure(n_tiles + 2);
     cx->tile_scan.ensure(n_tiles + 2);
     cx->tile_scanb.ensure(n_tiles + 2);
     cx->tile_nn.ensure(n_tiles + 2);
@@ -136,7 +137,7 @@
             Lookback lb{};
             if (wide) lb = next_lookback(cx, tile_scan_blocks(n_tiles));
             launch_tile_layout(s, cx->tile_cur.p, n_tiles, bcap, cx->tile_n.p, cx->tile_scan.p, cx->tile_scanb.p,
-                               cx->scal.p + S_M3, cx->scal.p + S_M0, wide ? &lb : nullptr, cx->scal.p + S_ERR);
+                               cx->scal.p + S_M3, cx->scal.p + S_M0, wide ? &lb : nullptr, cx->scal.p + S_ERR, cx->tile_heavy.p);
         }
         std::vector<uint32_t> sc = fetch_scal(cx);
         static const bool test_fail = getenv("NP2_TEST_DENSE_LB_FAIL") != nullptr;
@@ -159,7 +160,7 @@
         if (sc[S_M2] == 0) {
             cx->tile_pidx.ensure((size_t)n_tiles * (TILE / 16) + 64);
             launch_tile_sort(s, cx->tile_pidx.p, c->reads.p, c->nib.p, cx->tile_n.p, n_tiles, bcap, sc[S_M1], cx->keys_raw.p,
-                             cx->vals_raw.p, cx->scal.p + S_ERR);
+                             cx->vals_raw.p, cx->scal.p + S_ERR, cx->tile_heavy.p);
             cx->bucket_cap = bcap;
             cx->pidx_valid = true;
         } else {
diff --git a/nextpolish2_amd/csrc/np2_regions.hip b/nextpolish2_amd/csrc/np2_regions.hip
--- a/nextpolish2_amd/csrc/np2_regions.hip
+++ b/nextpolish2_amd/csrc/np2_regions.hip
@@ -692,7 +692,7 @@
 }
 static constexpr uint32_t SPLICE_SPAN = 2048;
 static constexpr uint32_t SPLICE_LDS_SLOTS = 256;
-__device__ __forceinline__ void k_splice_bases(const uint32_t np2_bid, const uint32_t np2_nb, const uint32_t *__restrict__ in_pos,
+__device__ __forceinline__ void splice_bases_block(const uint32_t np2_bid, const uint32_t *__restrict__ in_pos,
                                                       const uint8_t *__restrict__ in_base,
                                                       const uint32_t *__restrict__ M_p,
                                                       const uint32_t *__restrict__ ap_s, const uint32_t *__restrict__ ap_e,
@@ -753,7 +753,7 @@
         out_base[o] = bv[k];
     }
 }
-__device__ __forceinline__ void k_splice_seeds(const uint32_t np2_bid, const uint32_t np2_nb, const uint32_t *__restrict__ ap_g, const uint32_t *__restrict__ ap_s,
+__device__ __forceinline__ void splice_seeds_block(const uint32_t np2_bid, const uint32_t *__restrict__ ap_g, const uint32_t *__restrict__ ap_s,
                                const int32_t *__restrict__ ap_delta, const int32_t *__restrict__ ap_shift_incl,
                                const uint32_t *__restrict__ n_ap_p, const uint32_t *__restrict__ lq_start,
                                const uint32_t *__restrict__ seed_cand, const uint32_t *__restrict__ seq_off,
@@ -769,6 +769,20 @@
         out_pos[o + t] = p;
         out_base[o + t] = seq[so + t];
     }
+}
+__device__ __forceinline__ void k_splice_write(const uint32_t np2_bid, const uint32_t np2_nb, uint32_t n_bases_blocks,
+                                               const uint32_t *__restrict__ in_pos, const uint8_t *__restrict__ in_base,
+                                               const uint32_t *__restrict__ M_p, const uint32_t *__restrict__ ap_g,
+                                               const uint32_t *__restrict__ ap_s, const uint32_t *__restrict__ ap_e,
+                                               const int32_t *__restrict__ ap_delta, const int32_t *__restrict__ ap_shift_incl,
+                                               const uint32_t *__restrict__ n_ap_p, const uint32_t *__restrict__ lq_start,
+                                               const uint32_t *__restrict__ seed_cand, const uint32_t *__restrict__ seq_off,
+                                               const uint8_t *__restrict__ seq, uint32_t *__restrict__ out_pos,
+                                               uint8_t *__restrict__ out_base) {
+    if (np2_bid < n_bases_blocks)
+        splice_bases_block(np2_bid, in_pos, in_base, M_p, ap_s, ap_e, ap_shift_incl, n_ap_p, out_pos, out_base);
+    else
+        splice_seeds_block(np2_bid - n_bases_blocks, ap_g, ap_s, ap_delta, ap_shift_incl, n_ap_p, lq_start, seed_cand, seq_off, seq, out_pos, out_base);
 }
 
 __device__ __forceinline__ void k_shard_bounds(const uint32_t np2_bid, const uint32_t np2_nb, const uint32_t *__restrict__ cns_pos, const uint32_t *__restrict__ M_p,
@@ -1112,54 +1126,71 @@
 }
 
 static constexpr uint32_t RL_ITEMS = 4;
-static_assert(RL_CAP_LIST == 256 * RL_ITEMS, "a thread of the list kernels owns RL_ITEMS consecutive entries");
+static_assert(RL_CAP_LIST == 256 * RL_ITEMS, "a thread of the list phases owns RL_ITEMS consecutive entries");
+static constexpr uint32_t RR_THREADS = 1024, RR_WAVES = RR_THREADS / 64;
 static_assert((uint64_t)RL_CAP_LIST * (RL_CAP_JOBS + 1) < (1ull << 32) && (uint64_t)RL_CAP_LIST * (RL_CAP_BLOB + 1) < (1ull << 32),
               "clamped per-group sums stay inside 32 bits");
 
-__device__ __forceinline__ RechCtx rl_ctx(const RechList &a, const uint32_t *rech, const uint32_t *__restrict__ cand_off,
-                                          const uint32_t *__restrict__ keep_list, const uint32_t *__restrict__ seq_off,
-                                          const uint8_t *__restrict__ seq, const uint8_t *__restrict__ cns_base, uint32_t n_groups) {
-    return RechCtx{(const RechGroup *)a.groups, a.job_off, rech, cand_off, keep_list, seq_off, seq, cns_base, n_groups};
-}
-__device__ __forceinline__ void rl_round_off(const RechList &a, uint32_t cap_err, uint32_t *__restrict__ err) {
+__device__ __forceinline__ void rl_round_off(const RechList &a, uint32_t cap_err, const uint32_t *__restrict__ M_in,
+                                             uint32_t *__restrict__ n_ap, uint32_t *__restrict__ M_out, uint32_t *err) {
     a.st[RL_N] = 0, a.st[RL_NGROUPS] = 0, a.st[RL_NJOBS] = 0, a.st[RL_OFF] = 1;
     if (cap_err) atomicOr(err, RECH_CAP_ERR);
-}
-
-__device__ __forceinline__ void k_rech_prepare(const uint32_t np2_bid, const uint32_t np2_nb, RechList a,
-                                               const uint32_t *__restrict__ cns_pos, const uint8_t *__restrict__ cns_base,
-                                               const uint32_t *__restrict__ M_p, const uint32_t *__restrict__ lq_start,
-                                               const uint32_t *__restrict__ lq_end, const uint32_t *__restrict__ keep_n,
-                                               uint32_t ksize, const uint32_t *__restrict__ reg_maxlen,
-                                               const uint32_t *__restrict__ cand_off, const uint32_t *__restrict__ keep_list,
-                                               const uint32_t *__restrict__ seq_off, const uint8_t *__restrict__ seq,
-                                               uint32_t *__restrict__ err) {
-    __shared__ uint32_t s_raw[RL_CAP_LIST], s_rech[RL_CAP_LIST], s_lo[RL_CAP_LIST], s_ub[RL_CAP_LIST], sh[8], s_hdr[2];
+    *n_ap = 0, *M_out = *M_in, *a.cnt_in = 0, *a.cnt_out = 0;
+}
+static constexpr uint32_t RL_NEAR = 2048;
+__device__ __forceinline__ void cns_span_near(const uint32_t *__restrict__ cns_pos, uint32_t M, uint32_t st, uint32_t en,
+                                              uint32_t &lo, uint32_t &ub) {
+    if (M == 0) {
+        lo = ub = 0;
+        return;
+    }
+    const uint32_t c = min(st, M), wl = c > RL_NEAR ? c - RL_NEAR : 0u, wh = (uint32_t)min((uint64_t)M, (uint64_t)c + RL_NEAR);
+    const uint32_t before = cns_pos[wl ? wl - 1 : 0u], behind = cns_pos[min(wh, M - 1)];
+    const bool inside = (wl == 0 || before < st) && (wh == M || behind >= st);
+    lo = inside ? bound16_u32<false>(cns_pos, wh, st, wl) : lower_bound_u32(cns_pos, M, st);
+    const uint32_t near = (uint32_t)min((uint64_t)M, (uint64_t)lo + (en - st) + 65u);
+    ub = (near == M || cns_pos[near - 1] > en) ? bound16_u32<true>(cns_pos, near, en, lo) : upper_bound_u32(cns_pos, M, en);
+}
+
+__device__ __forceinline__ void k_rech_round(const uint32_t np2_bid, const uint32_t np2_nb, RechList a, YakDev y, uint32_t min_count,
+                                             uint16_t *score, const uint32_t *__restrict__ cns_pos,
+                                             const uint8_t *__restrict__ cns_base, const uint32_t *__restrict__ M_in,
+                                             const uint32_t *__restrict__ lq_start, const uint32_t *__restrict__ lq_end,
+                                             const uint32_t *__restrict__ keep_n, uint32_t ksize,
+                                             const uint32_t *__restrict__ reg_maxlen, const uint32_t *__restrict__ cand_off,
+                                             const uint32_t *__restrict__ keep_list, const uint32_t *__restrict__ seq_off,
+                                             const uint8_t *__restrict__ seq, uint16_t *keep_ks,
+                                             const uint32_t *__restrict__ order, uint32_t first_yak, uint32_t last_round,
+                                             uint8_t *reg_lable, uint32_t *seed_cand, uint32_t *__restrict__ ap_g,
+                                             uint32_t *__restrict__ ap_s, uint32_t *__restrict__ ap_e,
+                                             int32_t *__restrict__ ap_delta, int32_t *__restrict__ ap_shift_incl,
+                                             uint32_t *__restrict__ n_ap, uint32_t *__restrict__ M_out, uint32_t out_cap,
+                                             uint32_t *err) {
+    __shared__ uint32_t s_joff[RL_CAP_LIST + 1], s_rech[RL_CAP_LIST], s_lo[RL_CAP_LIST], s_ub[RL_CAP_LIST], sh[RR_WAVES], s_hdr[2], s_stuck;
+    uint32_t *const s_raw = s_joff;
     const uint32_t tid = threadIdx.x;
-    if (tid == 0) s_hdr[0] = *err, s_hdr[1] = *a.cnt_in;
+    if (tid == 0) s_hdr[0] = *err, s_hdr[1] = *a.cnt_in, s_stuck = 0;
     __syncthreads();
     const uint32_t n = s_hdr[1], cap_list = min(a.cap_list, RL_CAP_LIST);
     if (s_hdr[0] != 0 || n > cap_list) {
-        if (tid == 0) rl_round_off(a, s_hdr[0] == 0, err);
+        if (tid == 0) rl_round_off(a, s_hdr[0] == 0, M_in, n_ap, M_out, err);
         return;
     }
-    for (uint32_t i = tid; i < n; i += 256) s_raw[i] = a.list_in[i];
+    for (uint32_t i = tid; i < n; i += RR_THREADS) s_raw[i] = a.list_in[i];
     __syncthreads();
-    for (uint32_t i = tid; i < n; i += 256) {
+    for (uint32_t i = tid; i < n; i += RR_THREADS) {
         const uint32_t v = s_raw[i];
         uint32_t rank = 0;
         for (uint32_t j = 0; j < n; ++j) rank += s_raw[j] > v ? 1u : 0u;
         s_rech[rank] = v;
-        a.rech[rank] = v;
     }
     __syncthreads();
-    const uint32_t M = *M_p;
-    for (uint32_t i = tid; i < n; i += 256) {
+    const uint32_t M = *M_in;
+    for (uint32_t i = tid; i < n; i += RR_THREADS) {
         const uint32_t g = s_rech[i];
         uint32_t lo, ub;
-        cns_span(cns_pos, M, lq_start[g], lq_end[g], lo, ub);
+        cns_span_near(cns_pos, M, lq_start[g], lq_end[g], lo, ub);
         s_lo[i] = lo, s_ub[i] = ub;
-        a.pos_lo[i] = lo, a.pos_ub[i] = ub;
     }
     __syncthreads();
     RechGroup *const groups = (RechGroup *)a.groups, *const tmp_groups = (RechGroup *)a.tmp_groups;
@@ -1180,31 +1211,31 @@
         hs += head[k], js += jobs[k], bsum += bytes[k];
     }
     uint32_t nh, nj, nb;
-    uint32_t lh = block_excl_scan<OpAdd, 4>(hs, sh, nh);
-    uint32_t lj = block_excl_scan<OpAdd, 4>(js, sh, nj);
-    uint32_t lbt = block_excl_scan<OpAdd, 4>(bsum, sh, nb);
+    uint32_t lh = block_excl_scan<OpAdd, RR_WAVES>(hs, sh, nh);
+    uint32_t lj = block_excl_scan<OpAdd, RR_WAVES>(js, sh, nj);
+    uint32_t lbt = block_excl_scan<OpAdd, RR_WAVES>(bsum, sh, nb);
     if (nj > min(a.cap_jobs, RL_CAP_JOBS) || nb > min(a.cap_blob, RL_CAP_BLOB)) {
-        if (tid == 0) rl_round_off(a, 1u, err);
+        if (tid == 0) rl_round_off(a, 1u, M_in, n_ap, M_out, err);
         return;
     }
 #pragma unroll
     for (uint32_t k = 0; k < RL_ITEMS; ++k) {
         if (!head[k]) continue;
         groups[lh] = tmp_groups[tid * RL_ITEMS + k];
-        a.job_off[lh] = lj;
+        s_joff[lh] = lj;
         a.blob_off[lh] = lbt;
         a.glen[lh] = glen[k];
         ++lh, lj += jobs[k], lbt += bytes[k];
     }
     if (tid == 0) {
-        a.job_off[nh] = nj;
+        s_joff[nh] = nj;
         a.st[RL_N] = n, a.st[RL_NGROUPS] = nh, a.st[RL_NJOBS] = nj, a.st[RL_OFF] = 0;
     }
     __threadfence_block();
     __syncthreads();
-    const RechCtx cx = rl_ctx(a, s_rech, cand_off, keep_list, seq_off, seq, cns_base, nh);
-    for (uint32_t j = tid >> 4; j < nj; j += 16) {
-        const uint32_t gi = job_group(cx, j), rem = j - a.job_off[gi];
+    const RechCtx cx = RechCtx{groups, s_joff, s_rech, cand_off, keep_list, seq_off, seq, cns_base, nh};
+    for (uint32_t j = tid >> 4; j < nj; j += RR_THREADS / 16) {
+        const uint32_t gi = job_group(cx, j), rem = j - s_joff[gi];
         const uint32_t off = a.blob_off[gi] + rem * a.glen[gi];
         uint32_t len = rech_group_string<false>(cx, gi, rem, nullptr);
         if (len <= a.glen[gi]) {
@@ -1215,31 +1246,22 @@
         }
         if ((tid & 15u) == 0) a.job_ol[j] = make_uint2(off, len);
     }
-}
-
-__device__ __forceinline__ void k_rech_finish(const uint32_t np2_bid, const uint32_t np2_nb, RechList a,
-                                              const uint16_t *__restrict__ score, uint16_t *__restrict__ keep_ks,
-                                              const uint32_t *__restrict__ cand_off, const uint32_t *__restrict__ keep_n,
-                                              const uint32_t *__restrict__ keep_list, const uint32_t *__restrict__ order,
-                                              uint32_t first_yak, uint32_t last_round, uint8_t *__restrict__ reg_lable,
-                                              uint32_t *__restrict__ seed_cand, const uint32_t *__restrict__ cns_pos,
-                                              const uint32_t *__restrict__ M_in, const uint32_t *__restrict__ lq_start,
-                                              const uint32_t *__restrict__ seq_off,
-                                              uint32_t *__restrict__ ap_g, uint32_t *__restrict__ ap_s,
-                                              uint32_t *__restrict__ ap_e, int32_t *__restrict__ ap_delta,
-                                              int32_t *__restrict__ ap_shift_incl, uint32_t *__restrict__ n_ap,
-                                              uint32_t *__restrict__ M_out, uint32_t out_cap, uint32_t *__restrict__ err) {
-    __shared__ uint32_t sh[8], s_hdr[4], s_stuck;
-    const uint32_t tid = threadIdx.x;
-    if (tid == 0) s_hdr[0] = *err, s_hdr[1] = a.st[RL_N], s_hdr[2] = a.st[RL_NGROUPS], s_hdr[3] = a.st[RL_OFF], s_stuck = 0;
+    __threadfence_block();
     __syncthreads();
-    if (s_hdr[0] != 0 || s_hdr[3] != 0) {
+    if (tid == 0) s_hdr[0] = atomicOr(err, 0u);
+    __syncthreads();
+    if (s_hdr[0] != 0) {
         if (tid == 0) *n_ap = 0, *M_out = *M_in, *a.cnt_in = 0, *a.cnt_out = 0;
         return;
     }
-    const uint32_t n = s_hdr[1], n_groups = s_hdr[2], M = *M_in;
-    const RechCtx cx = rl_ctx(a, a.rech, cand_off, keep_list, seq_off, nullptr, nullptr, n_groups);
-    for (uint32_t gi = tid; gi < n_groups; gi += 256) rech_apply_group(cx, gi, score, keep_ks);
+    for (uint32_t j = (uint32_t)__builtin_amdgcn_readfirstlane((int)(tid >> 6)); j < nj; j += RR_WAVES) {
+        const uint2 ol = a.job_ol[j];
+        const uint16_t sc = wave_score_string(y, a.blob + ol.x, ol.y, (uint16_t)min_count);
+        if ((tid & 63u) == 0) score[j] = sc;
+    }
+    __threadfence_block();
+    __syncthreads();
+    for (uint32_t gi = tid; gi < nh; gi += RR_THREADS) rech_apply_group(cx, gi, score, keep_ks);
     __threadfence_block();
     __syncthreads();
     uint32_t g[RL_ITEMS], s[RL_ITEMS], e[RL_ITEMS];
@@ -1248,9 +1270,9 @@
         const uint32_t x = tid * RL_ITEMS + k;
         g[k] = 0, s[k] = 0, e[k] = 0;
         if (x >= n) continue;
-        g[k] = a.rech[x];
+        g[k] = s_rech[x];
         rech_select_region(g[k], cand_off, keep_n, keep_list, keep_ks, order, first_yak, reg_lable, seed_cand);
-        if (!splice_range(cns_pos, M, lq_start[g[k]], a.pos_lo[x], a.pos_ub[x], s[k], e[k])) atomicMax(&s_stuck, g[k] + 1);
+        if (!splice_range(cns_pos, M, lq_start[g[k]], s_lo[x], s_ub[x], s[k], e[k])) atomicMax(&s_stuck, g[k] + 1);
     }
     __syncthreads();
     const uint32_t stuck = s_stuck;
@@ -1267,8 +1289,8 @@
         fsum += flag[k], dsum_t += delta[k];
     }
     uint32_t cnt, dsum;
-    uint32_t lo = block_excl_scan<OpAdd, 4>(fsum, sh, cnt);
-    uint32_t ld = block_excl_scan<OpAdd, 4>((uint32_t)dsum_t, sh, dsum);
+    uint32_t lo = block_excl_scan<OpAdd, RR_WAVES>(fsum, sh, cnt);
+    uint32_t ld = block_excl_scan<OpAdd, RR_WAVES>((uint32_t)dsum_t, sh, dsum);
 #pragma unroll
     for (uint32_t k = 0; k < RL_ITEMS; ++k) {
         if (flag[k]) {
@@ -1294,7 +1316,7 @@
         ksum += keep[k];
     }
     uint32_t n_keep;
-    uint32_t lk = block_excl_scan<OpAdd, 4>(ksum, sh, n_keep);
+    uint32_t lk = block_excl_scan<OpAdd, RR_WAVES>(ksum, sh, n_keep);
 #pragma unroll
     for (uint32_t k = 0; k < RL_ITEMS; ++k) {
         if (keep[k]) a.list_out[lk] = g[k];
@@ -1395,9 +1417,8 @@
                          const int32_t *ap_shift_incl, const uint32_t *n_ap, uint32_t max_ap, const uint32_t *lq_start,
                          const uint32_t *seed_cand, const uint32_t *seq_off, const uint8_t *seq, uint32_t *out_pos,
                          uint8_t *out_base) {
-    NP2_LAUNCH(k_splice_bases, dim3((M_cap + SPLICE_SPAN - 1) / SPLICE_SPAN), 256, s, in_pos, in_base, M_p, ap_s, ap_e, ap_shift_incl, n_ap, out_pos, out_base);
-    if (max_ap)
-        NP2_LAUNCH(k_splice_seeds, g1((uint64_t)max_ap * 8, 256), 256, s, ap_g, ap_s, ap_delta, ap_shift_incl, n_ap, lq_start, seed_cand, seq_off, seq, out_pos, out_base);
+    const uint32_t nb_bases = (M_cap + SPLICE_SPAN - 1) / SPLICE_SPAN, nb_seeds = g1((uint64_t)max_ap * 8, 256).x;
+    NP2_LAUNCH(k_splice_write, dim3(nb_bases + nb_seeds), 256, s, nb_bases, in_pos, in_base, M_p, ap_g, ap_s, ap_e, ap_delta, ap_shift_incl, n_ap, lq_start, seed_cand, seq_off, seq, out_pos, out_base);
 }
 void launch_shard_bounds(hipStream_t s, const uint32_t *cns_pos, const uint32_t *M_p, const uint32_t *t, uint32_t *out) {
     NP2_LAUNCH(k_shard_bounds, dim3(1), 64, s, cns_pos, M_p, t[0], t[1], t[2], t[3], t[4], t[5], out);
@@ -1443,19 +1464,15 @@
 void launch_rech_relabel(hipStream_t s, uint8_t *reg_lable, uint32_t n_reg) {
     NP2_LAUNCH(k_rech_relabel, g1(n_reg), 256, s, reg_lable, n_reg);
 }
-void launch_rech_prepare(hipStream_t s, const RechList &a, const uint32_t *cns_pos, const uint8_t *cns_base, const uint32_t *M_p,
-                         const uint32_t *lq_start, const uint32_t *lq_end, const uint32_t *keep_n, uint32_t ksize,
-                         const uint32_t *reg_maxlen, const uint32_t *cand_off, const uint32_t *keep_list,
-                         const uint32_t *seq_off, const uint8_t *seq, uint32_t *err) {
-    NP2_LAUNCH(k_rech_prepare, dim3(1), 256, s, a, cns_pos, cns_base, M_p, lq_start, lq_end, keep_n, ksize, reg_maxlen, cand_off, keep_list, seq_off, seq, err);
-}
-void launch_rech_finish(hipStream_t s, const RechList &a, const uint16_t *score, uint16_t *keep_ks, const uint32_t *cand_off,
-                        const uint32_t *keep_n, const uint32_t *keep_list, const uint32_t *order, bool first_yak,
-                        bool last_round, uint8_t *reg_lable, uint32_t *seed_cand, const uint32_t *cns_pos,
-                        const uint32_t *M_in, const uint32_t *lq_start, const uint32_t *seq_off,
-                        uint32_t *ap_g, uint32_t *ap_s, uint32_t *ap_e, int32_t *ap_delta, int32_t *ap_shift_incl,
-                        uint32_t *n_ap, uint32_t *M_out, uint32_t out_cap, uint32_t *err) {
-    NP2_LAUNCH(k_rech_finish, dim3(1), 256, s, a, score, keep_ks, cand_off, keep_n, keep_list, order, first_yak ? 1u : 0u, last_round ? 1u : 0u, reg_lable, seed_cand, cns_pos, M_in, lq_start, seq_off, ap_g, ap_s, ap_e, ap_delta, ap_shift_incl, n_ap, M_out, out_cap, err);
-}
-
-}
+void launch_rech_round(hipStream_t s, const RechList &a, const YakDev &y, uint16_t min_count, uint16_t *score,
+                       const uint32_t *cns_pos, const uint8_t *cns_base, const uint32_t *M_in, const uint32_t *lq_start,
+                       const uint32_t *lq_end, const uint32_t *keep_n, uint32_t ksize, const uint32_t *reg_maxlen,
+                       const uint32_t *cand_off, const uint32_t *keep_list, const uint32_t *seq_off, const uint8_t *seq,
+                       uint16_t *keep_ks, const uint32_t *order, bool first_yak, bool last_round, uint8_t *reg_lable,
+                       uint32_t *seed_cand, uint32_t *ap_g, uint32_t *ap_s, uint32_t *ap_e, int32_t *ap_delta,
+                       int32_t *ap_shift_incl, uint32_t *n_ap, uint32_t *M_out, uint32_t out_cap, uint32_t *err) {
+    static_assert(Sig<decltype(&k_rech_round)>::N >= 5, "a recheck round's arguments outgrew the merged launch of a group");
+    NP2_LAUNCH(k_rech_round, dim3(1), RR_THREADS, s, a, y, (uint32_t)min_count, score, cns_pos, cns_base, M_in, lq_start, lq_end, keep_n, ksize, reg_maxlen, cand_off, keep_list, seq_off, seq, keep_ks, order, first_yak ? 1u : 0u, last_round ? 1u : 0u, reg_lable, seed_cand, ap_g, ap_s, ap_e, ap_delta, ap_shift_incl, n_ap, M_out, out_cap, err);
+}
+
+}
```

Result: faster. 4548, median of 6 (+1.3%).
